# vdorie/stan4bart

Hardware: AMD Instinct MI355X
Metric: gibbs_iters_per_sec (higher is better)
Workload: dtype f64

## Files before the change

### include/stan4bart_amd.h

```cpp
#ifndef STAN4BART_AMD_H
#define STAN4BART_AMD_H

#include <stdint.h>
#include <stddef.h>

#ifndef S4B_PREFIX
#define S4B_PREFIX s4b_
#endif
#define S4B_CAT_(a, b) a##b
#define S4B_CAT(a, b) S4B_CAT_(a, b)
#define S4B_FN(name) S4B_CAT(S4B_PREFIX, name)

#ifdef __cplusplus
extern "C" {
#endif

#define S4B_INTERFACE_VERSION 6

typedef struct s4b_sampler s4b_sampler;

typedef struct {
  int32_t n_trees;
  int32_t n_thin;
  int32_t keep_trees;
// ... 338 lines not shown
  int64_t info[8];
} s4b_curves_out;
int S4B_FN(predict_curves)(s4b_sampler* s, const s4b_curves_in* in, s4b_curves_out* out);

typedef struct {
  s4b_summary_in rows;
  const double* y;
  const double* sigma;
  const double* row_scale;
  int32_t tail_len;
  int32_t n_peers;
  s4b_sampler* const* peers;
  const double* const* peer_dense_coef;
  const double* const* peer_ell_coef;
  const double* const* peer_sigma;
  int64_t scratch_bytes;
} s4b_loo_in;
typedef struct {
  double* elpd_loo;
  double* pareto_k;
  double* lpd;
  double* ess;
  int64_t num_samples;
  int32_t tail_len;
  int64_t info[8];
} s4b_loo_out;
int S4B_FN(predict_loo)(s4b_sampler* s, const s4b_loo_in* in, s4b_loo_out* out);

typedef struct {
  s4b_summary_in rows;
  int32_t quantity;
  int32_t split;
  const double* y;
  const double* sigma;
  const double* row_scale;
  int32_t n_peers;
  s4b_sampler* const* peers;
  const double* const* peer_dense_coef;
  const double* const* peer_ell_coef;
  const double* const* peer_sigma;
  int64_t scratch_bytes;
} s4b_conv_in;
typedef struct {
  double* rhat;
  double* ess;
  double* mean;
  double* mcse;
  int32_t* n_pairs;
  int64_t num_samples;
  int32_t n_chains;
  int32_t chain_len;
  int64_t info[8];
} s4b_conv_out;
int S4B_FN(predict_convergence)(s4b_sampler* s, const s4b_conv_in* in, s4b_conv_out* out);

#define S4B_STATE_MAGIC 0x53423453u
typedef struct {
  uint32_t magic, version;
  int64_t n;
  int32_t n_trees, num_unconstrained, is_binary, p;
  int64_t reserved[2];
} s4b_state_header;
int S4B_FN(get_state)(s4b_sampler* s, void* buf, int64_t cap, int64_t* size);
int S4B_FN(set_state)(s4b_sampler* s, const void* buf, int64_t size);

int S4B_FN(set_trace)(s4b_sampler* s, int32_t enable);
int S4B_FN(get_trace)(s4b_sampler* s, int64_t cap_records, int32_t* out, int64_t* num_records);
int S4B_FN(get_leaf_assignment)(s4b_sampler* s, int32_t tree, int32_t* out);
int S4B_FN(set_device_sharing)(s4b_sampler* s, int32_t chains);
int S4B_FN(set_tree_path)(s4b_sampler* s, int32_t path);
int S4B_FN(get_tree_path)(s4b_sampler* s, int32_t out[2]);
int S4B_FN(get_counters)(s4b_sampler* s, int64_t out[3]);
int S4B_FN(get_fused_stats)(s4b_sampler* s, int64_t out[2]);
int S4B_FN(get_sweep_stats)(s4b_sampler* s, int64_t out[2]);
int S4B_FN(get_sweep_spec)(s4b_sampler* s, int64_t out[4]);
int S4B_FN(get_sweep_busy)(s4b_sampler* s, int64_t* out);
int S4B_FN(set_hmc_mode)(s4b_sampler* s, int32_t mode);
int S4B_FN(get_hmc_mode)(s4b_sampler* s, int32_t* mode);
int S4B_FN(set_latent_mode)(s4b_sampler* s, int32_t mode);
int S4B_FN(get_latent_mode)(s4b_sampler* s, int32_t* mode);

int S4B_FN(get_nuts_stats)(s4b_sampler* s, double out[4]);

int S4B_FN(profile_sweep)(s4b_sampler* s, int32_t n_sweeps, double out[8]);
int S4B_FN(stream_probe)(int32_t device, int64_t n_doubles, int32_t reps, double out[4]);

int S4B_FN(profile_leapfrog)(s4b_sampler* s, int32_t n_evals, double out[8]);

int S4B_FN(set_test_hook)(s4b_sampler* s, int32_t hook, int64_t value);

int S4B_FN(test_draw_latents)(s4b_sampler* s);

int S4B_FN(test_hand_off)(s4b_sampler* s, const double* beta, const double* b, double sigma, int32_t update_scale);

#define S4B_STAN_SUMS_INFO 18
int S4B_FN(test_stan_sums)(s4b_sampler* s, int32_t mode, const double* beta, const double* b, const int32_t* set_exp, double* sums, int64_t* info);

void S4B_FN(free)(s4b_sampler* s);

typedef struct s4b_sweep_group s4b_sweep_group;
int S4B_FN(sweep_group_create)(int32_t device, int32_t max_members, s4b_sweep_group** out);
int S4B_FN(sweep_group_join)(s4b_sweep_group* g, s4b_sampler* s);
int S4B_FN(sweep_group_leave)(s4b_sampler* s);
int S4B_FN(sweep_group_stats)(s4b_sweep_group* g, int64_t out[4]);
int S4B_FN(sweep_group_set_timeout)(s4b_sweep_group* g, double seconds);
int S4B_FN(sweep_group_free)(s4b_sweep_group* g);

#ifdef __cplusplus
}
#endif
#endif
```

### stan4bart_amd/abi.py

```python
from __future__ import annotations

import ctypes as C
from dataclasses import dataclass, field
from typing import Callable, Optional, Sequence

import numpy as np

INTERFACE_VERSION = 6
c_double_p = C.POINTER(C.c_double)
c_int32_p = C.POINTER(C.c_int32)
c_uint32_p = C.POINTER(C.c_uint32)


class BartControl(C.Structure):
    _fields_ = [("n_trees", C.c_int32), ("n_thin", C.c_int32), ("keep_trees", C.c_int32),
                ("node_capacity", C.c_int32),
                ("base", C.c_double), ("power", C.c_double), ("k", C.c_double), ("node_scale", C.c_double),
                ("birth_or_death_prob", C.c_double), ("swap_prob", C.c_double),
                ("change_prob", C.c_double), ("birth_prob", C.c_double),
                ("split_probs", c_double_p), ("use_quantiles", C.c_int32), ("interface_version", C.c_int32),
                ("k_hyper_df", C.c_double), ("k_hyper_scale", C.c_double)]


class BartData(C.Structure):
# ... 158 lines not shown


class LooIn(C.Structure):
    _fields_ = [("rows", SummaryIn), ("y", c_double_p), ("sigma", c_double_p), ("row_scale", c_double_p), ("tail_len", C.c_int32),
                ("n_peers", C.c_int32), ("peers", C.POINTER(C.c_void_p)), ("peer_dense_coef", C.POINTER(c_double_p)),
                ("peer_ell_coef", C.POINTER(c_double_p)), ("peer_sigma", C.POINTER(c_double_p)), ("scratch_bytes", C.c_int64)]


class LooOut(C.Structure):
    _fields_ = [("elpd_loo", c_double_p), ("pareto_k", c_double_p), ("lpd", c_double_p), ("ess", c_double_p), ("num_samples", C.c_int64),
                ("tail_len", C.c_int32), ("info", C.c_int64 * 8)]


class ConvIn(C.Structure):
    _fields_ = [("rows", SummaryIn), ("quantity", C.c_int32), ("split", C.c_int32), ("y", c_double_p), ("sigma", c_double_p), ("row_scale", c_double_p),
                ("n_peers", C.c_int32), ("peers", C.POINTER(C.c_void_p)), ("peer_dense_coef", C.POINTER(c_double_p)),
                ("peer_ell_coef", C.POINTER(c_double_p)), ("peer_sigma", C.POINTER(c_double_p)), ("scratch_bytes", C.c_int64)]


class ConvOut(C.Structure):
    _fields_ = [("rhat", c_double_p), ("ess", c_double_p), ("mean", c_double_p), ("mcse", c_double_p), ("n_pairs", C.POINTER(C.c_int32)),
                ("num_samples", C.c_int64), ("n_chains", C.c_int32), ("chain_len", C.c_int32), ("info", C.c_int64 * 8)]


SUMMARY_ROUTES = {"auto": 0, "staged": 1, "global": 2}
SUMMARY_INFO = ("route", "rows_per_tile", "workgroups", "staging_bytes", "largest_draw_nodes", "launches", "device_bytes", "staging_nodes")
PD_INFO = SUMMARY_INFO[:7] + ("largest_affected", "total_affected")
QUANTILE_INFO = ("route", "rows_per_chunk", "chunks", "rows_per_sort", "padded_draws", "largest_draw_nodes", "launches", "device_bytes", "draws")
CONTRAST_INFO = ("route", "rows_per_chunk", "chunks", "launches", "device_bytes", "draws", "differing_columns", "largest_affected", "total_affected")
GROUPS_INFO = ("route", "rows_per_chunk", "chunks", "launches", "device_bytes", "draws", "edge_levels", "nan_levels")
GROUPS_STATISTICS = {"sum": 0, "mean": 1}
GROUPS_LEVEL_BYTES_MAX = 1 << 30
PROJECTION_INFO = ("route", "rows_per_chunk", "chunks", "launches", "device_bytes", "draws", "deficient", "columns")
PROJECTION_COLUMNS_MAX = 32
PROJECTION_SLAB = 128
SPREAD_INFO = ("route", "rows_per_chunk", "chunks", "launches", "device_bytes", "draws", "thresholds", "zero_slabs")
SPREAD_THRESHOLDS_MAX = 64
SPREAD_SLAB = 128
SPREAD_BIN_INDEX = {"auto": 0, "compare": 1, "search": 2}
CHECK_INFO = SPREAD_INFO
CURVES_INFO = QUANTILE_INFO[:7] + ("device_bytes", "largest_affected", "total_affected")
CURVES_OUTPUTS = ("mean", "m2", "quantiles", "p_max", "p_min", "range_mean", "range_m2", "range_quantiles")
CURVES_SCRATCH_MAX = 1 << 30
PPD_INFO = QUANTILE_INFO
LOO_INFO = QUANTILE_INFO
LOO_OUTPUTS = ("elpd_loo", "pareto_k", "lpd", "ess")
CONV_INFO = QUANTILE_INFO
CONV_OUTPUTS = ("rhat", "ess", "mean", "mcse", "n_pairs")
CONV_QUANTITIES = {"ev": 0, "lik": 1}
PD_GRID_MAX = 64


def _peer_tables(peers, draws, given, cols, what):
    if not cols or not peers or given is None:
        return None, []
    if len(given) != len(peers):
        raise ValueError(f"{what} must hold one table per peer ({len(peers)})")
    held = []
    for x, (t, smp) in enumerate(zip(given, peers)):
        t = np.asarray(t)
        if t.shape != (draws(smp), cols):
            raise ValueError(f"{what}[{x}] must be [{draws(smp)} x {cols}], not shape {t.shape}")
        held.append(_f64(t, "C"))
    return (c_double_p * len(held))(*[_dp(t) for t in held]), held


def _dp(a: Optional[np.ndarray]):
    return None if a is None else a.ctypes.data_as(c_double_p)


def _ip(a: Optional[np.ndarray]):
    return None if a is None else a.ctypes.data_as(c_int32_p)


def _f64(a, order="F") -> np.ndarray:
    return np.require(np.asarray(a, dtype=np.float64), requirements=["A", "O"] + (["F"] if order == "F" else ["C"]))


def _i32(a) -> np.ndarray:
    return np.ascontiguousarray(np.asarray(a, dtype=np.int32))


LATENT_MODES = {"exact": 0, "parallel": 1}

@dataclass
class SamplerArgs:
    x_bart: np.ndarray
    n_trees: int = 75
    n_cuts: int | Sequence[int] = 100
    n_thin: int = 1
    x_test: Optional[np.ndarray] = None
    base: float = 0.95
    power: float = 2.0
    k: float = 2.0
    node_scale: Optional[float] = None
    keep_trees: bool = False
    node_capacity: int = 0
    proposal_probs: Sequence[float] = (0.5, 0.1, 0.4, 0.5)
    split_probs: Optional[Sequence[float]] = None
    use_quantiles: bool = False
    k_hyper: Optional[tuple] = None
    latents: str = "exact"
    X: Optional[np.ndarray] = None
    y: Optional[np.ndarray] = None
    weights: Optional[np.ndarray] = None
    is_binary: bool = False
    prior_dist: int = 1
    prior_dist_for_aux: int = 3
    prior_scale: Optional[np.ndarray] = None
    prior_mean: Optional[np.ndarray] = None
    prior_df: Optional[np.ndarray] = None
    prior_scale_for_aux: float = 1.0
    prior_mean_for_aux: float = 0.0
    prior_df_for_aux: float = 1.0
    global_prior_df: float = 1.0
    global_prior_scale: float = 0.01
    slab_df: float = 4.0
    slab_scale: float = 2.5
    num_normals: Optional[Sequence[int]] = None
    p: Sequence[int] = ()
    l: Sequence[int] = ()
    shape: Sequence[float] = ()
    scale: Sequence[float] = ()
    concentration: Sequence[float] = ()
    regularization: Sequence[float] = ()
    w: Optional[np.ndarray] = None
    v: Optional[np.ndarray] = None
    u: Optional[np.ndarray] = None
    seed: int = 0
    skip: int = 1
    init_r: float = 2.0
    adapt_gamma: float = 0.05
    adapt_delta: float = 0.8
    adapt_kappa: float = 0.75
    adapt_t0: float = 10.0
    adapt_init_buffer: int = 75
    adapt_term_buffer: int = 50
    adapt_window: int = 25
    stepsize: float = 1.0
    stepsize_jitter: float = 0.0
    max_treedepth: int = 10
    hmc_mode: int = 0
    warmup: int = 1000
    iter: int = 2000
    verbose: int = 0
    refresh: int = 0
    offset: Optional[np.ndarray] = None
    offset_type: int = 0
    bart_offset_init: Optional[np.ndarray] = None
    sigma_init: float = 1.0
    keep_fits: bool = True
    callback: Optional[Callable] = None
    device: int = 0
    extras: dict = field(default_factory=dict)


class Sampler:

    def __init__(self, lib: C.CDLL, prefix: str, args: SamplerArgs, r_rng_state: np.ndarray):
        self._lib, self._pfx = lib, prefix
        self._bind()
        a = args
        self._keep = []

        def keep(x):
            self._keep.append(x)
# ... 27 lines not shown
        y = keep(_f64(a.y))
        t = len(a.p)
        q = int(sum(int(pi) * int(li) for pi, li in zip(a.p, a.l)))
        len_theta_L = int(sum(pi * (pi - 1) // 2 + pi for pi in a.p))
        ps = keep(_f64(a.prior_scale if a.prior_scale is not None else np.ones(K)))
        pm = keep(_f64(a.prior_mean if a.prior_mean is not None else np.zeros(K)))
        pdf = keep(_f64(a.prior_df if a.prior_df is not None else np.ones(K)))
        wts = keep(_f64(a.weights)) if a.weights is not None and len(a.weights) else None
        p_arr, l_arr = keep(_i32(a.p)), keep(_i32(a.l))
        shape, scale = keep(_f64(a.shape)), keep(_f64(a.scale))
        conc, reg = keep(_f64(a.concentration)), keep(_f64(a.regularization))
        w = keep(_f64(a.w if a.w is not None else np.zeros(0)))
        v = keep(_i32(a.v if a.v is not None else np.zeros(0)))
        u = keep(_i32(a.u if a.u is not None else np.zeros(n + 1)))
        sd = StanData(N=n, K=K, is_binary=int(a.is_binary), has_intercept=0, has_weights=int(wts is not None),
                      prior_dist=a.prior_dist, prior_dist_for_aux=a.prior_dist_for_aux,
                      X=_dp(X), y=_dp(y), weights=_dp(wts), prior_scale=_dp(ps), prior_mean=_dp(pm), prior_df=_dp(pdf),
                      prior_scale_for_aux=a.prior_scale_for_aux, prior_mean_for_aux=a.prior_mean_for_aux,
                      prior_df_for_aux=a.prior_df_for_aux, t=t, q=q, len_theta_L=len_theta_L,
                      len_concentration=len(conc), len_regularization=len(reg), reserved=0,
                      p=_ip(p_arr), l=_ip(l_arr), shape=_dp(shape), scale=_dp(scale),
                      concentration=_dp(conc), regularization=_dp(reg), num_non_zero=len(w),
                      w=_dp(w), v=_ip(v), u=_ip(u),
                      global_prior_df=a.global_prior_df, global_prior_scale=a.global_prior_scale, slab_df=a.slab_df,
                      slab_scale=a.slab_scale,
                      num_normals=_ip(keep(_i32(a.num_normals))) if a.num_normals is not None else None)
        sc = StanControl(seed=a.seed & 0xFFFFFFFF, skip=a.skip, init_r=a.init_r, adapt_gamma=a.adapt_gamma,
                         adapt_delta=a.adapt_delta, adapt_kappa=a.adapt_kappa, adapt_t0=a.adapt_t0,
                         adapt_init_buffer=a.adapt_init_buffer, adapt_term_buffer=a.adapt_term_buffer,
                         adapt_window=a.adapt_window, reserved=0, stepsize=a.stepsize,
                         stepsize_jitter=a.stepsize_jitter, max_treedepth=a.max_treedepth, hmc_mode=a.hmc_mode)
        off = keep(_f64(a.offset)) if a.offset is not None and len(a.offset) else None
        boi = keep(_f64(a.bart_offset_init)) if a.bart_offset_init is not None else None
        self._py_callback = a.callback
        self._cb = CALLBACK(self._trampoline) if a.callback is not None else CALLBACK()
        cc = CommonControl(warmup=a.warmup, iter=a.iter, verbose=a.verbose, refresh=a.refresh,
                           is_binary=int(a.is_binary), offset_type=a.offset_type, keep_fits=int(a.keep_fits),
                           device=a.device, offset=_dp(off), bart_offset_init=_dp(boi), sigma_init=a.sigma_init,
                           callback=self._cb, callback_user=None)
        st = np.ascontiguousarray(r_rng_state, dtype=np.uint32)
        assert st.shape == (625,)
        self._h = C.c_void_p()
        rc = self._f("create")(C.byref(bc), C.byref(bd), C.byref(sd), C.byref(sc), C.byref(cc),
                               st.ctypes.data_as(c_uint32_p), C.byref(self._h))
        self._check(rc)
        self._keep.clear()
        if a.latents not in LATENT_MODES:
            self.free()
            raise ValueError(f"latents must be one of {sorted(LATENT_MODES)}, not {a.latents!r}")
        if a.latents != "exact":
            try:
                self.set_latent_mode(LATENT_MODES[a.latents])
            except Exception:
                self.free()
                raise
        dims = (C.c_int64 * 5)()
        self._check(self._f("get_dims")(self._h, dims))
        self.num_pars, self.n, self.n_test, self.p, self.n_trees = (int(d) for d in dims)
        self.keep_fits = bool(a.keep_fits)
        self.K, self.q = int(K), int(q)
        self.callback_results: list = []
        self._pending_exc = None

    def _bind(self):
        vp, i32, i64, dp, ip, up = C.c_void_p, C.c_int32, C.c_int64, c_double_p, c_int32_p, c_uint32_p
        sig = {
            "create": [C.POINTER(BartControl), C.POINTER(BartData), C.POINTER(StanData), C.POINTER(StanControl),
                       C.POINTER(CommonControl), up, C.POINTER(vp)],
            "run": [vp, i32, i32, i32, C.POINTER(Results)],
            "disengage_adaptation": [vp], "print_initial_summary": [vp],
            "get_parametric_mean": [vp, dp], "get_bart_data_range": [vp, dp],
            "get_r_rng_state": [vp, up], "set_r_rng_state": [vp, up],
            "get_dims": [vp, C.POINTER(i64)], "get_stan_par_names": [vp, C.c_char_p, C.c_size_t],
            "get_trees": [vp, i64, ip, ip, ip, ip, dp, C.POINTER(i64)],
            "get_kept_trees": [vp, i64, i64, ip, ip, ip, ip, ip, dp, C.POINTER(i64)],
            "get_kept_trees_indexed": [vp, ip, i64, ip, i64, i64, ip, ip, ip, ip, ip, dp, C.POINTER(i64)],
            "export_bart_state": [vp, vp, i64, C.POINTER(i64)],
            "create_stored_bart_sampler": [vp, i64, i32, C.POINTER(vp)],
            "predict_bart": [vp, dp, i64, dp, C.POINTER(i64)],
            "predict_bart_offset": [vp, dp, i64, dp, dp, C.POINTER(i64)], "print_trees": [vp, ip, i64, ip, i64],
            "get_state": [vp, vp, i64, C.POINTER(i64)], "set_state": [vp, vp, i64],
            "set_trace": [vp, i32], "get_trace": [vp, i64, ip, C.POINTER(i64)],
            "get_leaf_assignment": [vp, i32, ip], "get_counters": [vp, C.POINTER(i64)], "get_nuts_stats": [vp, dp],
            "profile_sweep": [vp, i32, dp], "profile_leapfrog": [vp, i32, dp],
            "set_progress": [vp, PROGRESS, vp], "set_device_sharing": [vp, i32],
            "set_tree_path": [vp, i32], "get_tree_path": [vp, ip], "get_fused_stats": [vp, C.POINTER(i64)], "get_sweep_stats": [vp, C.POINTER(i64)], "get_sweep_busy": [vp, C.POINTER(i64)], "get_sweep_spec": [vp, C.POINTER(i64)], "set_test_hook": [vp, i32, i64], "set_hmc_mode": [vp, i32], "get_hmc_mode": [vp, ip],
            "predict_summary": [vp, C.POINTER(SummaryIn), C.POINTER(SummaryOut)],
            "partial_dependence": [vp, C.POINTER(PdIn), C.POINTER(PdOut)],
            "predict_quantiles": [vp, C.POINTER(QuantileIn), C.POINTER(QuantileOut)],
            "predict_contrast": [vp, C.POINTER(ContrastIn), C.POINTER(ContrastOut)],
            "predict_groups": [vp, C.POINTER(GroupsIn), C.POINTER(GroupsOut)],
            "predict_projection": [vp, C.POINTER(ProjectionIn), C.POINTER(ProjectionOut)],
            "predict_spread": [vp, C.POINTER(SpreadIn), C.POINTER(SpreadOut)],
            "predict_check": [vp, C.POINTER(CheckIn), C.POINTER(CheckOut)],
            "predict_curves": [vp, C.POINTER(CurvesIn), C.POINTER(CurvesOut)],
            "predict_ppd": [vp, C.POINTER(PpdIn), C.POINTER(PpdOut)],
            "predict_loo": [vp, C.POINTER(LooIn), C.POINTER(LooOut)],
            "predict_convergence": [vp, C.POINTER(ConvIn), C.POINTER(ConvOut)],
            "set_latent_mode": [vp, i32], "get_latent_mode": [vp, ip], "test_draw_latents": [vp], "test_hand_off": [vp, dp, dp, C.c_double, i32],
            "test_stan_sums": [vp, i32, dp, dp, ip, dp, C.POINTER(i64)],
        }
        for name, argtypes in sig.items():
            fn = getattr(self._lib, self._pfx + name, None)
            if fn is None:
                continue
            fn.restype = C.c_int
            fn.argtypes = argtypes
        getattr(self._lib, self._pfx + "last_error").restype = C.c_char_p
        getattr(self._lib, self._pfx + "last_error").argtypes = []
        getattr(self._lib, self._pfx + "free").restype = None
        getattr(self._lib, self._pfx + "free").argtypes = [vp]

    def _f(self, name):
        return getattr(self._lib, self._pfx + name)

    def _check(self, rc):
        if rc != 0:
            raise RuntimeError(self._f("last_error")().decode())

    def _trampoline(self, user, yhat_train, yhat_test, stan_pars, num_pars):
        tr = np.ctypeslib.as_array(yhat_train, shape=(self.n,)).copy()
        te = np.ctypeslib.as_array(yhat_test, shape=(self.n_test,)).copy() if self.n_test else None
        sp = np.ctypeslib.as_array(stan_pars, shape=(num_pars,)).copy()
        try:
            self.callback_results.append(self._py_callback(tr, te, sp))
        except BaseException as e:
            if self._pending_exc is None:
                self._pending_exc = e
            return 1
        return 0

    def run(self, num_iter: int, is_warmup: bool, results_type: int = 0) -> dict:
        S = num_iter if self.keep_fits else 1
        stan = np.zeros((self.num_pars, S), order="F")
        sigma = np.zeros(S)
        train = np.zeros((self.n, S), order="F")
        test = np.zeros((self.n_test, S), order="F")
        varcount = np.zeros((self.p, S), dtype=np.int32, order="F")
        kdraws = np.zeros(S)
        res = Results(stan=_dp(stan), bart_sigma=_dp(sigma), bart_train=_dp(train),
                      bart_test=_dp(test) if self.n_test else None, bart_varcount=_ip(varcount),
                      bart_k=_dp(kdraws) if getattr(self, "k_modeled", False) else None)
        self.callback_results = []
        self._pending_exc = None
        rc = self._f("run")(self._h, num_iter, int(is_warmup), results_type, C.byref(res))
        if self._pending_exc is not None:
            e, self._pending_exc = self._pending_exc, None
            raise e
        self._check(rc)
        out = {}
        if results_type in (0, 2):
            out["stan"] = stan
        if results_type in (0, 1):
            out["bart"] = dict(sigma=sigma, train=train, test=test, varcount=varcount)
            if getattr(self, "k_modeled", False):
                out["bart"]["k"] = kdraws
        if self._py_callback is not None:
            out["callback"] = list(self.callback_results)
        return out

    def disengage_adaptation(self):
        self._check(self._f("disengage_adaptation")(self._h))

    def print_initial_summary(self):
        self._check(self._f("print_initial_summary")(self._h))

# ... 125 lines not shown

    def get_fused_stats(self):
        out = (C.c_int64 * 2)()
        fn = getattr(self._lib, self._pfx + "get_fused_stats", None)
        if fn is not None:
            self._check(fn(self._h, out))
        return int(out[0]), int(out[1])

    def get_sweep_stats(self):
        fn = getattr(self._lib, self._pfx + "get_sweep_stats", None)
        if fn is None:
            return (0, 0)
        out = (C.c_int64 * 2)()
        self._check(fn(self._h, out))
        return (int(out[0]), int(out[1]))

    def get_sweep_spec(self):
        fn = getattr(self._lib, self._pfx + "get_sweep_spec", None)
        if fn is None:
            return (0, 0, 0, 0)
        out = (C.c_int64 * 4)()
        self._check(fn(self._h, out))
        return tuple(int(v) for v in out)

    def set_test_hook(self, hook: int, value: int):
        self._check(self._f("set_test_hook")(self._h, int(hook), int(value)))

    def test_draw_latents(self):
        self._check(self._f("test_draw_latents")(self._h))

    def test_hand_off(self, beta, b, sigma: float, update_scale: bool):
        beta, b = _f64(np.atleast_1d(beta)), _f64(np.atleast_1d(b))
        self._check(self._f("test_hand_off")(self._h, _dp(beta) if beta.size else None, _dp(b) if b.size else None, float(sigma), int(bool(update_scale))))

    STAN_SUMS_INFO = 18

    def test_stan_sums(self, mode: int, beta=None, b=None, set_exp=None):
        K, q = self.K, self.q
        beta = _f64(np.zeros(K) if beta is None else np.atleast_1d(beta))
        b = _f64(np.zeros(q) if b is None else np.atleast_1d(b))
        if beta.size != K or b.size != q:
            raise ValueError(f"test_stan_sums: beta needs {K} entries and b {q}")
        ex = None if set_exp is None else np.ascontiguousarray(set_exp, dtype=np.int32)
        if ex is not None and ex.shape != (3,):
            raise ValueError("test_stan_sums: set_exp holds three exponents")
        sums = np.zeros(1 + K + q)
        info = (C.c_int64 * Sampler.STAN_SUMS_INFO)()
        self._check(self._f("test_stan_sums")(self._h, int(mode), _dp(beta) if K else None, _dp(b) if q else None, _ip(ex) if ex is not None else None, _dp(sums), info))
        v = [int(x) for x in info]
        return sums, dict(accepted=bool(v[0]), reject=v[1], exp_used=tuple(v[2:5]), exp_after=tuple(v[5:8]), mag=tuple(v[8:11]), exw=tuple(v[11:14]),
                          grid=v[14], fused=bool(v[15]), evals=v[16], fallbacks=v[17])

    def get_sweep_busy(self) -> int:
        fn = getattr(self._lib, self._pfx + "get_sweep_busy", None)
        if fn is None:
            return 0
        out = C.c_int64(0)
        self._check(fn(self._h, C.byref(out)))
        return int(out.value)

    def set_trace(self, enable: bool):
        self._check(self._f("set_trace")(self._h, int(enable)))

    def get_trace(self, cap: int = 1 << 20) -> np.ndarray:
        nn = C.c_int64()
        out = np.zeros((cap, 5), dtype=np.int32)
        self._check(self._f("get_trace")(self._h, cap, _ip(out), C.byref(nn)))
        return out[: nn.value].copy()

    def get_leaf_assignment(self, tree: int) -> np.ndarray:
        out = np.zeros(self.n, dtype=np.int32)
        self._check(self._f("get_leaf_assignment")(self._h, tree, _ip(out)))
        return out

    def get_counters(self) -> np.ndarray:
        out = (C.c_int64 * 3)()
        self._check(self._f("get_counters")(self._h, out))
        return np.array(list(out), dtype=np.int64)

    def get_nuts_stats(self) -> dict:
        out = (C.c_double * 4)()
        self._check(self._f("get_nuts_stats")(self._h, out))
        return dict(transitions=int(out[0]), sum_treedepth=int(out[1]), sum_n_leapfrog=int(out[2]), divergent=int(out[3]))

    def predict_bart(self, x_test: np.ndarray, offset_test: Optional[np.ndarray] = None) -> np.ndarray:
        xt = _f64(x_test)
        ns = C.c_int64()
        self._check(self._f("predict_bart")(self._h, _dp(xt), xt.shape[0], None, C.byref(ns)))
        out = np.zeros((xt.shape[0], ns.value), order="F")
        if ns.value:
            if offset_test is not None:
                off = _f64(offset_test)
                if off.shape != (xt.shape[0],):
                    raise ValueError("length of offset_test must equal number of rows in x_test")
                self._check(self._f("predict_bart_offset")(self._h, _dp(xt), xt.shape[0], _dp(off), _dp(out), C.byref(ns)))
            else:
                self._check(self._f("predict_bart")(self._h, _dp(xt), xt.shape[0], _dp(out), C.byref(ns)))
        return out

    def predict_summary(self, x_test: np.ndarray, offset=None, dense=None, dense_coef=None, ell_index=None, ell_value=None, ell_coef=None,
                        link: int = 0, weights=None, route="auto", stage_nodes: int = 0, max_workgroups: int = 0) -> dict:
        fn = getattr(self._lib, self._pfx + "predict_summary", None)
        if fn is None:
            raise RuntimeError(f"this library ({self._pfx}*) has no predict_summary")
        probe = SummaryOut()
        self._check(fn(self._h, None, C.byref(probe)))
        S = int(probe.num_samples)
        arg, keep, rows, G = self._summary_in(S, x_test, offset, dense, dense_coef, ell_index, ell_value, ell_coef, link, weights, route, stage_nodes,
                                              max_workgroups)
        mean, m2, avg = np.zeros(rows), np.zeros(rows), np.zeros((S, G))
        out = SummaryOut(mean=_dp(mean), m2=_dp(m2), average=_dp(avg) if avg.size else None)
        self.summary_info = dict(zip(SUMMARY_INFO, [0] * 8))
        rc = fn(self._h, C.byref(arg), C.byref(out))
        self.summary_info = dict(zip(SUMMARY_INFO, (int(v) for v in out.info)))
        self._check(rc)
        return dict(mean=mean, m2=m2, average=avg, draws=int(out.num_samples), info=dict(self.summary_info))

    @staticmethod
    def _summary_in(S, x_test, offset, dense, dense_coef, ell_index, ell_value, ell_coef, link, weights, route, stage_nodes, max_workgroups):
        xt = _f64(x_test)
        if xt.ndim != 2:
            raise ValueError("x_test must be a matrix [rows x predictors]")
        rows = xt.shape[0]

        def table(a, first, what):
            if a is None:
                return None, 0
            a = np.asarray(a)
            if a.ndim != 2 or a.shape[0] != first:
                raise ValueError(f"{what} must have {first} rows, not shape {a.shape}")
            return a, a.shape[1]
        dense, M = table(dense, rows, "dense")
        dense_coef, Mc = table(dense_coef, S, "dense_coef")
        ell_index, E = table(ell_index, rows, "ell_index")
        ell_value, Ev = table(ell_value, rows, "ell_value")
        ell_coef, q = table(ell_coef, S, "ell_coef")
        if M != Mc:
            raise ValueError(f"dense has {M} columns, dense_coef {Mc}")
        if E != Ev:
            raise ValueError(f"ell_index has {E} columns, ell_value {Ev}")
        if weights is not None:
            weights = np.asarray(weights, dtype=np.float64)
            if weights.ndim != 2 or weights.shape[1] != rows:
                raise ValueError(f"weights must be [G x {rows}], not shape {weights.shape}")
        G = 0 if weights is None else weights.shape[0]
        off = None
        if offset is not None:
            off = _f64(offset)
            if off.shape != (rows,):
                raise ValueError("length of offset must equal number of rows in x_test")
        keep = dict(dense=None if not M else _f64(dense), dense_coef=None if not M else _f64(dense_coef, "C"),
                    ell_index=None if not E else np.asfortranarray(np.asarray(ell_index, dtype=np.int32)),
                    ell_value=None if not E else _f64(ell_value), ell_coef=None if not E else _f64(ell_coef, "C"),
                    weights=None if not G else _f64(weights, "C"))
        keep.update(x_test=xt, offset=off)
        arg = SummaryIn(x_test=_dp(xt), n_test=rows, offset=_dp(off), n_dense=M, n_ell=E, n_ell_coef=q if E else 0, link=int(link), n_weights=G,
                        route=int(SUMMARY_ROUTES.get(route, route)), stage_nodes=int(stage_nodes), max_workgroups=int(max_workgroups),
                        dense=_dp(keep["dense"]), dense_coef=_dp(keep["dense_coef"]), ell_index=_ip(keep["ell_index"]),
                        ell_value=_dp(keep["ell_value"]), ell_coef=_dp(keep["ell_coef"]), weights=_dp(keep["weights"]))
        return arg, keep, rows, G

    def partial_dependence(self, x_test: np.ndarray, vars, grid, offset=None, dense=None, dense_coef=None, ell_index=None, ell_value=None,
                           ell_coef=None, link: int = 0, weights=None, route="auto", stage_nodes: int = 0, max_workgroups: int = 0) -> dict:
        fn = getattr(self._lib, self._pfx + "partial_dependence", None)
        if fn is None:
            raise RuntimeError(f"this library ({self._pfx}*) has no partial_dependence")
# ... 732 lines not shown
```

### stan4bart_amd/csrc/c_api.inc

```
#include <memory>
#include <string>

struct s4b_sampler { s4b::SamplerCore<S4B_DEV> core; template <class... A> explicit s4b_sampler(A... a) : core(a...) {} };
struct s4b_sweep_group { std::unique_ptr<s4b::SweepGroup> g; };

namespace { thread_local std::string g_last_error; }

#define S4B_TRY try {
#define S4B_CATCH } catch (const std::exception& e) { g_last_error = e.what(); return 1; } catch (...) { g_last_error = "unknown error"; return 1; } return 0;
#define S4B_NEED(s, what) if (!(s)) { g_last_error = what " called on NULL sampler"; return 1; }

extern "C" {

const char* S4B_FN(last_error)(void) { return g_last_error.c_str(); }

int S4B_FN(create)(const s4b_bart_control* bc, const s4b_bart_data* bd, const s4b_stan_data* sd, const s4b_stan_control* sc,
                   const s4b_common_control* cc, const uint32_t* rstate, s4b_sampler** out) {
  S4B_TRY
  if (!out) throw std::invalid_argument("create: NULL output pointer");
  *out = new s4b_sampler(bc, bd, sd, sc, cc, rstate);
  S4B_CATCH
}
int S4B_FN(run)(s4b_sampler* s, int32_t num_iter, int32_t is_warmup, int32_t results_type, s4b_results* out) {
  S4B_NEED(s, "run") S4B_TRY s->core.dev().bind(); s4b::SamplerCore<S4B_DEV>::GroupRun inRun(s->core); s->core.run(num_iter, is_warmup != 0, results_type, out); S4B_CATCH
// ... 77 lines not shown
  s->core.dev().bind();
  std::vector<const s4b::SamplerCore<S4B_DEV>*> peers;
  if (in && out && in->arms.n_peers > 0 && in->arms.peers) for (int x = 0; x < in->arms.n_peers; ++x) peers.push_back(in->arms.peers[x] ? &in->arms.peers[x]->core : nullptr);
  s->core.predict_spread(in, out, peers.empty() ? nullptr : peers.data());
  S4B_CATCH
}
int S4B_FN(predict_check)(s4b_sampler* s, const s4b_check_in* in, s4b_check_out* out) {
  S4B_NEED(s, "predict_check") S4B_TRY
  s->core.dev().bind();
  std::vector<const s4b::SamplerCore<S4B_DEV>*> peers;
  if (in && out && in->n_peers > 0 && in->peers) for (int x = 0; x < in->n_peers; ++x) peers.push_back(in->peers[x] ? &in->peers[x]->core : nullptr);
  s->core.predict_check(in, out, peers.empty() ? nullptr : peers.data());
  S4B_CATCH
}
int S4B_FN(predict_curves)(s4b_sampler* s, const s4b_curves_in* in, s4b_curves_out* out) {
  S4B_NEED(s, "predict_curves") S4B_TRY
  s->core.dev().bind();
  std::vector<const s4b::SamplerCore<S4B_DEV>*> peers;
  if (in && out && in->n_peers > 0 && in->peers) for (int x = 0; x < in->n_peers; ++x) peers.push_back(in->peers[x] ? &in->peers[x]->core : nullptr);
  s->core.predict_curves(in, out, peers.empty() ? nullptr : peers.data());
  S4B_CATCH
}
int S4B_FN(predict_ppd)(s4b_sampler* s, const s4b_ppd_in* in, s4b_ppd_out* out) {
  S4B_NEED(s, "predict_ppd") S4B_TRY
  s->core.dev().bind();
  std::vector<const s4b::SamplerCore<S4B_DEV>*> peers;
  if (in && out && in->n_peers > 0 && in->peers) for (int x = 0; x < in->n_peers; ++x) peers.push_back(in->peers[x] ? &in->peers[x]->core : nullptr);
  s->core.predict_ppd(in, out, peers.empty() ? nullptr : peers.data());
  S4B_CATCH
}
int S4B_FN(predict_loo)(s4b_sampler* s, const s4b_loo_in* in, s4b_loo_out* out) {
  S4B_NEED(s, "predict_loo") S4B_TRY
  s->core.dev().bind();
  std::vector<const s4b::SamplerCore<S4B_DEV>*> peers;
  if (in && out && in->n_peers > 0 && in->peers) for (int x = 0; x < in->n_peers; ++x) peers.push_back(in->peers[x] ? &in->peers[x]->core : nullptr);
  s->core.predict_loo(in, out, peers.empty() ? nullptr : peers.data());
  S4B_CATCH
}
int S4B_FN(predict_convergence)(s4b_sampler* s, const s4b_conv_in* in, s4b_conv_out* out) {
  S4B_NEED(s, "predict_convergence") S4B_TRY
  s->core.dev().bind();
  std::vector<const s4b::SamplerCore<S4B_DEV>*> peers;
  if (in && out && in->n_peers > 0 && in->peers) for (int x = 0; x < in->n_peers; ++x) peers.push_back(in->peers[x] ? &in->peers[x]->core : nullptr);
  s->core.predict_convergence(in, out, peers.empty() ? nullptr : peers.data());
  S4B_CATCH
}
int S4B_FN(export_bart_state)(s4b_sampler* s, void* buf, int64_t cap, int64_t* size) {
  S4B_NEED(s, "exportBARTState") S4B_TRY s->core.dev().bind(); if (!size) throw std::invalid_argument("exportBARTState: NULL size pointer"); *size = s->core.export_state(buf, cap); S4B_CATCH
}
int S4B_FN(create_stored_bart_sampler)(const void* state, int64_t size, int32_t device, s4b_sampler** out) {
  S4B_TRY
  if (!out) throw std::invalid_argument("createStoredBARTSampler: NULL output pointer");
  *out = new s4b_sampler(state, size, (int)device);
  S4B_CATCH
}
int S4B_FN(get_state)(s4b_sampler* s, void* buf, int64_t cap, int64_t* size) {
  S4B_NEED(s, "get_state") S4B_TRY s->core.dev().bind(); if (!size) throw std::invalid_argument("get_state: NULL size pointer"); *size = s->core.get_state(buf, cap); S4B_CATCH
}
int S4B_FN(set_state)(s4b_sampler* s, const void* buf, int64_t size) { S4B_NEED(s, "set_state") S4B_TRY s->core.dev().bind(); s->core.set_state(buf, size); S4B_CATCH }
int S4B_FN(set_trace)(s4b_sampler* s, int32_t enable) { S4B_NEED(s, "set_trace") S4B_TRY s->core.dev().bind(); s->core.set_trace(enable != 0); S4B_CATCH }
int S4B_FN(get_trace)(s4b_sampler* s, int64_t cap, int32_t* out, int64_t* num) { S4B_NEED(s, "get_trace") S4B_TRY s->core.dev().bind(); *num = s->core.get_trace(cap, out); S4B_CATCH }
int S4B_FN(get_leaf_assignment)(s4b_sampler* s, int32_t t, int32_t* out) { S4B_NEED(s, "get_leaf_assignment") S4B_TRY s->core.dev().bind(); s->core.leaf_assignment(t, out); S4B_CATCH }
int S4B_FN(set_device_sharing)(s4b_sampler* s, int32_t chains) { S4B_NEED(s, "set_device_sharing") S4B_TRY s->core.dev().bind(); s->core.set_device_sharing(chains); S4B_CATCH }
int S4B_FN(set_tree_path)(s4b_sampler* s, int32_t path) { S4B_NEED(s, "set_tree_path") S4B_TRY s->core.dev().bind(); s->core.dev().set_tree_path(path); S4B_CATCH }
int S4B_FN(get_tree_path)(s4b_sampler* s, int32_t out[2]) { S4B_NEED(s, "get_tree_path") S4B_TRY if (!out) throw std::invalid_argument("get_tree_path: NULL output pointer"); s->core.dev().get_tree_path(out); S4B_CATCH }
int S4B_FN(set_hmc_mode)(s4b_sampler* s, int32_t mode) { S4B_NEED(s, "set_hmc_mode") S4B_TRY s->core.set_hmc_mode(mode); S4B_CATCH }
int S4B_FN(get_hmc_mode)(s4b_sampler* s, int32_t* mode) { S4B_NEED(s, "get_hmc_mode") S4B_TRY if (!mode) throw std::invalid_argument("get_hmc_mode: NULL output pointer"); *mode = s->core.hmc_mode(); S4B_CATCH }
int S4B_FN(set_latent_mode)(s4b_sampler* s, int32_t mode) { S4B_NEED(s, "set_latent_mode") S4B_TRY s->core.dev().bind(); s->core.set_latent_mode(mode); S4B_CATCH }
int S4B_FN(get_latent_mode)(s4b_sampler* s, int32_t* mode) { S4B_NEED(s, "get_latent_mode") S4B_TRY if (!mode) throw std::invalid_argument("get_latent_mode: NULL output pointer"); *mode = s->core.latent_mode(); S4B_CATCH }
int S4B_FN(get_fused_stats)(s4b_sampler* s, int64_t out[2]) { S4B_NEED(s, "get_fused_stats") S4B_TRY if (!out) throw std::invalid_argument("get_fused_stats: NULL output pointer"); s->core.dev().fused_stats(out); S4B_CATCH }
int S4B_FN(get_sweep_stats)(s4b_sampler* s, int64_t out[2]) { S4B_NEED(s, "get_sweep_stats") S4B_TRY if (!out) throw std::invalid_argument("get_sweep_stats: NULL output pointer"); s->core.dev().sweep_stats(out); S4B_CATCH }
int S4B_FN(get_sweep_spec)(s4b_sampler* s, int64_t out[4]) { S4B_NEED(s, "get_sweep_spec") S4B_TRY if (!out) throw std::invalid_argument("get_sweep_spec: NULL output pointer"); s->core.dev().sweep_spec(out); S4B_CATCH }
int S4B_FN(set_test_hook)(s4b_sampler* s, int32_t hook, int64_t value) { S4B_NEED(s, "set_test_hook") S4B_TRY s->core.dev().set_test_hook(hook, value); S4B_CATCH }
int S4B_FN(test_draw_latents)(s4b_sampler* s) { S4B_NEED(s, "test_draw_latents") S4B_TRY s->core.dev().bind(); s->core.test_draw_latents(); S4B_CATCH }
int S4B_FN(test_hand_off)(s4b_sampler* s, const double* beta, const double* b, double sigma, int32_t update_scale) {
  S4B_NEED(s, "test_hand_off") S4B_TRY s->core.dev().bind(); s->core.test_hand_off(beta, b, sigma, update_scale != 0); S4B_CATCH
}
int S4B_FN(test_stan_sums)(s4b_sampler* s, int32_t mode, const double* beta, const double* b, const int32_t* set_exp, double* sums, int64_t* info) {
  S4B_NEED(s, "test_stan_sums") S4B_TRY s->core.dev().bind(); s->core.test_stan_sums(mode, beta, b, set_exp, sums, info); S4B_CATCH
}
int S4B_FN(get_sweep_busy)(s4b_sampler* s, int64_t* out) { S4B_NEED(s, "get_sweep_busy") S4B_TRY if (!out) throw std::invalid_argument("get_sweep_busy: NULL output pointer"); *out = s->core.dev().sweep_busy(); S4B_CATCH }
int S4B_FN(get_counters)(s4b_sampler* s, int64_t out[3]) { S4B_NEED(s, "get_counters") S4B_TRY s->core.dev().bind(); s->core.counters(out); S4B_CATCH }
int S4B_FN(get_nuts_stats)(s4b_sampler* s, double out[4]) { S4B_NEED(s, "get_nuts_stats") S4B_TRY s->core.dev().bind(); s->core.nuts_stats(out); S4B_CATCH }
int S4B_FN(profile_sweep)(s4b_sampler* s, int32_t n_sweeps, double out[8]) { S4B_NEED(s, "profile_sweep") S4B_TRY s->core.dev().bind(); s->core.profile_sweep(n_sweeps, out); S4B_CATCH }
int S4B_FN(profile_leapfrog)(s4b_sampler* s, int32_t n_evals, double out[8]) { S4B_NEED(s, "profile_leapfrog") S4B_TRY s->core.dev().bind(); s->core.profile_leapfrog(n_evals, out); S4B_CATCH }
int S4B_FN(stream_probe)(int32_t device, int64_t n_doubles, int32_t reps, double out[4]) { S4B_TRY S4B_DEV::probe_stream(device, n_doubles, reps, out); S4B_CATCH }
void S4B_FN(free)(s4b_sampler* s) { if (s) { try { s->core.leave_group(); } catch (...) {} } delete s; }

int S4B_FN(sweep_group_create)(int32_t device, int32_t max_members, s4b_sweep_group** out) {
  S4B_TRY
  if (!out) throw std::invalid_argument("sweep_group_create: NULL output pointer");
  *out = new s4b_sweep_group{std::unique_ptr<s4b::SweepGroup>(s4b::SamplerCore<S4B_DEV>::make_group((int)device, (int)max_members))};
  S4B_CATCH
}
int S4B_FN(sweep_group_join)(s4b_sweep_group* g, s4b_sampler* s) {
  S4B_NEED(s, "sweep_group_join") S4B_TRY if (!g) throw std::invalid_argument("sweep_group_join: NULL group"); s->core.join_group(g->g.get()); S4B_CATCH
}
int S4B_FN(sweep_group_leave)(s4b_sampler* s) { S4B_NEED(s, "sweep_group_leave") S4B_TRY s->core.leave_group(); S4B_CATCH }
int S4B_FN(sweep_group_stats)(s4b_sweep_group* g, int64_t out[4]) {
  S4B_TRY if (!g || !out) throw std::invalid_argument("sweep_group_stats: NULL argument"); g->g->stats(out); S4B_CATCH
}
int S4B_FN(sweep_group_set_timeout)(s4b_sweep_group* g, double seconds) {
  S4B_TRY if (!g) throw std::invalid_argument("sweep_group_set_timeout: NULL group"); g->g->set_timeout(seconds); S4B_CATCH
}
int S4B_FN(sweep_group_free)(s4b_sweep_group* g) {
  S4B_TRY
  if (!g) return 0;
  if (g->g->members() != 0) throw std::invalid_argument("sweep_group_free: samplers are still joined (s4b_sweep_group_leave / s4b_free them first)");
  delete g;
  S4B_CATCH
}

}
```

### stan4bart_amd/csrc/sampler_core.hpp

```cpp
#ifndef S4B_SAMPLER_CORE_HPP
#define S4B_SAMPLER_CORE_HPP

#include <algorithm>
#include <chrono>
#include <cstdio>
#include <cstdlib>
#include <cstring>
#include <memory>
#include <stdexcept>
#include <string>
#include <thread>
#include <type_traits>
#include <unordered_map>
#include <vector>

#include "../../include/stan4bart_amd.h"
#include "sweep_group.hpp"
#include "dev_common.hpp"
#include "stan_host.hpp"

namespace s4b {

enum { OFFSET_DEFAULT = 0, OFFSET_FIXEF, OFFSET_RANEF, OFFSET_BART, OFFSET_PARAMETRIC };
enum { OBS_R = 0, OBS_OFF, OBS_LAT, OBS_Y };
// ... 231 lines not shown
    if ((sd->prior_dist == 3 || sd->prior_dist == 4) && cc->is_binary) throw std::invalid_argument("hs priors scale with the residual sd: not available for binary responses");
    if (sd->prior_dist == 7 && !sd->num_normals) throw std::invalid_argument("product_normal needs num_normals");
    n_ = (size_t)bd->n; P_ = bd->p; T_ = bc->n_trees; nTest_ = (size_t)bd->n_test;
    warmup_ = cc->warmup; verbose_ = cc->verbose; refresh_ = cc->refresh; keepFits_ = cc->keep_fits != 0; offsetType_ = cc->offset_type;
    callback_ = cc->callback; callbackUser_ = cc->callback_user;
    thin_ = bc->n_thin > 0 ? bc->n_thin : 1;
    keepTrees_ = bc->keep_trees != 0;
    nc_ = bc->node_capacity > 0 ? bc->node_capacity : 256;
    if (nc_ < 3 || nc_ > 32000) throw std::invalid_argument("node_capacity must be in [3, 32000]");
    if (cc->offset) { userOffset_.assign(cc->offset, cc->offset + n_); hasUserOffset_ = true; }
    rng_.mti = (int32_t)rstate[0]; rng_.pad = 0;
    std::memcpy(rng_.mt, rstate + 1, 624 * sizeof(uint32_t));
    latKey_ = latent_key(rstate, sc->seed);

    StanSpec sp;
    sp.N = sd->N; sp.K = sd->K; sp.q = sd->q; sp.t = sd->t; sp.len_theta_L = sd->len_theta_L;
    sp.is_binary = binary_ ? 1 : 0; sp.prior_dist = sd->prior_dist; sp.prior_dist_for_aux = sd->prior_dist_for_aux;
    if (sd->K) { sp.prior_scale.assign(sd->prior_scale, sd->prior_scale + sd->K); sp.prior_mean.assign(sd->prior_mean, sd->prior_mean + sd->K);
                 sp.prior_df.assign(sd->prior_df, sd->prior_df + sd->K); }
    sp.prior_scale_for_aux = sd->prior_scale_for_aux; sp.prior_mean_for_aux = sd->prior_mean_for_aux; sp.prior_df_for_aux = sd->prior_df_for_aux;
    sp.global_prior_df = sd->global_prior_df; sp.global_prior_scale = sd->global_prior_scale; sp.slab_df = sd->slab_df; sp.slab_scale = sd->slab_scale;
    if (sd->prior_dist == 7) sp.num_normals.assign(sd->num_normals, sd->num_normals + sd->K);
    if (sd->t) { sp.p.assign(sd->p, sd->p + sd->t); sp.l.assign(sd->l, sd->l + sd->t); sp.shape.assign(sd->shape, sd->shape + sd->t);
                 sp.scale.assign(sd->scale, sd->scale + sd->t); }
    if (sd->len_concentration) sp.concentration.assign(sd->concentration, sd->concentration + sd->len_concentration);
    if (sd->len_regularization) sp.regularization.assign(sd->regularization, sd->regularization + sd->len_regularization);
    {
      int qq = 0; for (int i = 0; i < sd->t; ++i) qq += sd->p[i] * sd->l[i];
      if (qq != sd->q) throw std::invalid_argument("q != sum(p * l)");
      for (int64_t e = 0; e < sd->num_non_zero; ++e) if (sd->v[e] < 0 || sd->v[e] >= sd->q) throw std::invalid_argument("CSR column index out of range");
    }
    model_.reset(new HostModel(sp));
    if (const char* e = std::getenv("S4B_GRADIENT_CHECK")) model_->gradientCheck = std::atoi(e);
    K_ = sd->K; q_ = sd->q; hmcMode_ = sc->hmc_mode;
    cX_.assign((size_t)K_, 0.0); cZ_.assign((size_t)q_, 0.0);

    numCuts_.assign(bd->n_cuts, bd->n_cuts + P_);
    for (int j = 0; j < P_; ++j) if (numCuts_[(size_t)j] < 0 || numCuts_[(size_t)j] > 65534) throw std::invalid_argument("n_cuts must be in [0, 65534]");
    make_cuts(bd->x, bc->use_quantiles != 0);
    std::vector<uint16_t> xbin((size_t)P_ * n_), xbinTest((size_t)P_ * nTest_);
    bin_matrix(bd->x, n_, xbin);
    if (nTest_) bin_matrix(bd->x_test, nTest_, xbinTest);

    DevInit di;
    di.n = (int64_t)n_; di.nTest = (int64_t)nTest_; di.P = P_; di.T = T_; di.nc = nc_; di.device = cc->device; groupDevice_ = cc->device;
    di.xbin = xbin.data(); di.xbinTest = nTest_ ? xbinTest.data() : nullptr; di.numCuts = numCuts_.data();
    di.y = sd->y; di.userOffset = hasUserOffset_ ? userOffset_.data() : nullptr; di.weights = weights_.empty() ? nullptr : weights_.data();
    di.model.P = P_; di.model.Pvalid = 0;
    for (int j = 0; j < P_; ++j) if (numCuts_[(size_t)j] > 0) ++di.model.Pvalid;
    if (di.model.Pvalid == 0) throw std::invalid_argument("no predictor has a cut point");
    di.model.numCuts = nullptr; di.model.scratch = nullptr; di.model.splitProbs = nullptr;
    if (bc->split_probs) {
      splitProbs_.assign(bc->split_probs, bc->split_probs + P_);
      for (double w : splitProbs_) if (!(w > 0.0) || !std::isfinite(w)) throw std::invalid_argument("split_probs must be positive and finite");
      di.model.splitProbs = splitProbs_.data();
    }
    di.model.base = bc->base; di.model.power = bc->power;
    di.model.pBD = bc->birth_or_death_prob; di.model.pSwap = bc->swap_prob; di.model.pChange = bc->change_prob; di.model.pBirth = bc->birth_prob;
    if (!(bc->k > 0.0) || !std::isfinite(bc->k)) throw std::invalid_argument("k must be positive and finite");
    kModeled_ = bc->k_hyper_df > 0.0; kFixed_ = bc->k;
    if (kModeled_ && !(bc->k_hyper_scale > 0.0)) throw std::invalid_argument("k_hyper_scale must be positive (or +Inf)");
    if (kModeled_ && !std::isfinite(bc->k_hyper_df)) throw std::invalid_argument("k_hyper_df must be finite");
    di.model.leafPrec = leaf_precision(bc->k, T_, bc->node_scale);
    {
      pgDepth_.resize(S4B_MAX_DEPTH); logPg_.resize(S4B_MAX_DEPTH); log1mPg_.resize(S4B_MAX_DEPTH);
      for (int d = 0; d < S4B_MAX_DEPTH; ++d) {
        pgDepth_[(size_t)d] = bc->base / std::pow(1.0 + (double)d, bc->power);
        logPg_[(size_t)d] = std::log(pgDepth_[(size_t)d]); log1mPg_[(size_t)d] = std::log(1.0 - pgDepth_[(size_t)d]);
      }
      int maxCuts = 1; for (int j = 0; j < P_; ++j) maxCuts = std::max(maxCuts, numCuts_[(size_t)j]);
      logInt_.resize((size_t)std::max(P_, maxCuts) + 2);
      for (size_t k = 0; k < logInt_.size(); ++k) logInt_[k] = std::log((double)k);
      di.model.pgDepth = pgDepth_.data(); di.model.logPg = logPg_.data(); di.model.log1mPg = log1mPg_.data();
      di.model.logInt = logInt_.data(); di.model.logIntLen = (int32_t)logInt_.size();
    }
    di.K = K_; di.q = q_; di.binary = binary_ ? 1 : 0; di.X = sd->X; di.w = sd->w; di.v = sd->v; di.u = sd->u; di.nnz = sd->num_non_zero; nnz_ = sd->num_non_zero;
    di.traceCap = 1 << 16;
    hostModelView_ = di.model; hostModelView_.numCuts = numCuts_.data();
    dev_.init(di);
    if (kModeled_) dev_.set_k_hyper(bc->k_hyper_df, bc->k_hyper_scale, bc->node_scale, bc->k);

    if (hmcMode_ == 0) { build_gram(sd); haveGram_ = true; }
    dev_.stan_inputs( 0, false, cX_.data(), cZ_.data(), &s0_, nullptr);
    model_->lik = [this](const double* beta, const double* b, double* gX, double* gZ) { return likelihood(beta, b, gX, gZ); };
    NutsControl nc;
    nc.seed = sc->seed; nc.init_r = sc->init_r; nc.skip = sc->skip;
    if (nc.skip <= 0) { nc.skip = (2000 - warmup_) / 1000; if (nc.skip < 1) nc.skip = 1; }
    nc.gamma = sc->adapt_gamma; nc.delta = sc->adapt_delta; nc.kappa = sc->adapt_kappa; nc.t0 = sc->adapt_t0;
    nc.init_buffer = sc->adapt_init_buffer; nc.term_buffer = sc->adapt_term_buffer; nc.window = sc->adapt_window;
    nc.stepsize = sc->stepsize; nc.jitter = sc->stepsize_jitter; nc.max_depth = sc->max_treedepth;
    nuts_.reset(new Nuts(*model_, nc, 1, warmup_));
    row_.assign((size_t)(7 + model_->sp.n_constrained), 0.0);

    std::vector<double> bartOffset(n_, 0.0);
    const double* boi = cc->bart_offset_init;
    if (hasUserOffset_) {
      if (offsetType_ != OFFSET_BART) {
        bartOffset = userOffset_;
        if (boi && offsetType_ == OFFSET_DEFAULT) for (size_t i = 0; i < n_; ++i) bartOffset[i] += boi[i];
      } else if (boi) bartOffset.assign(boi, boi + n_);
    } else if (boi) bartOffset.assign(boi, boi + n_);
    dev_.offset_from_host(bartOffset.data());
    dev_.rescale(true);
    if (!binary_) { dev_.set_sigma(cc->sigma_init); sigma_ = cc->sigma_init; } else sigma_ = 1.0;
    sample_trees_from_prior();
    dev_.sweep(thin_);
    treeUpdates_ += (long)T_ * thin_;
    dev_.stan_inputs(stan_mode(), false, cX_.data(), cZ_.data(), &s0_, nullptr);
    check_device();
  }

  void run(int numIter, bool isWarmup, int resultsType, s4b_results* out) {
    live();
    if (numIter < 1) throw std::invalid_argument("num_iter must be >= 1");
    ran_ = true;
    dev_.reset_fused_scales();
    const bool doStan = resultsType == 0 || resultsType == 2, doBart = resultsType == 0 || resultsType == 1;
    const int numPars = (int)row_.size();
    size_t slot = 0;
    std::vector<double> train, test;
    const bool wantTrain = (out && out->bart_train) || callback_;
    const bool lastOnly = !keepFits_ && !callback_;
    if (wantTrain) train.resize(n_);
    if (nTest_) test.resize(nTest_);
    if (verbose_ > 0 && !progress_)
      std::printf("starting %s, %d draws, %s\n", isWarmup ? "warmup" : "sampling", numIter,
                  resultsType == 0 ? "both BART and Stan" : (resultsType == 1 ? "BART only" : "Stan only"));
    std::fflush(stdout);
    const bool timing = std::getenv("S4B_HOST_TIMING") != nullptr;
    double tph[4] = {0, 0, 0, 0};
    auto now = [] { return std::chrono::duration<double>(std::chrono::steady_clock::now().time_since_epoch()).count(); };
    for (int iter = 0; iter < numIter; ++iter) {
      if (progress_) {
        if (refresh_ <= 0 || (iter + 1) % refresh_ == 0 || iter == 0)
          if (progress_(progressUser_, iter + 1, numIter, isWarmup ? 1 : 0) != 0) throw std::runtime_error("interrupted by the progress callback");
      } else if (refresh_ > 0 && verbose_ > 1 && (iter + 1) % refresh_ == 0) { std::printf("  iter %.3d / %.3d\n", iter + 1, numIter); std::fflush(stdout); }
      double t0 = timing ? now() : 0;
      if (doStan) {
        nuts_->run(row_.data());
        if (timing) { tph[0] += now() - t0; t0 = now(); }
        const double* cons = row_.data() + 7;
        const double* beta = cons + model_->sp.beta_pos();
        const double* b = cons + model_->sp.b_pos();
        offset_by_type(beta, b);
        if (!binary_) { sigma_ = cons[model_->sp.aux_pos()]; dev_.set_sigma(sigma_); }
        if (out && out->stan) std::memcpy(out->stan + slot * (size_t)numPars, row_.data(), (size_t)numPars * sizeof(double));
        int update_scale_mod = 1 << (8 * iter / numIter);
        dev_.rescale(isWarmup && iter % update_scale_mod == 0);
        if (timing) { tph[1] += now() - t0; t0 = now(); }
      }
      if (doBart) {
        treeUpdates_ += (long)T_ * thin_;
        const bool emit = !lastOnly || iter == numIter - 1;
        if (nTest_ && emit && ((out && out->bart_test) || callback_)) dev_.request_test_fits();
        if (out && emit && out->bart_varcount) dev_.request_var_counts();
        sweep_and_stan_inputs(wantTrain && emit, (wantTrain && emit) ? train.data() : nullptr);
        if (timing) { tph[2] += now() - t0; t0 = now(); }
        if (nTest_ && emit && ((out && out->bart_test) || callback_)) dev_.test_fits(test.data());
        if (out && emit) {
          if (out->bart_sigma) out->bart_sigma[slot] = sigma_;
          if (out->bart_k) out->bart_k[slot] = kModeled_ ? dev_.k_current() : kFixed_;
          if (out->bart_train) std::memcpy(out->bart_train + slot * n_, train.data(), n_ * sizeof(double));
          if (out->bart_test && nTest_) std::memcpy(out->bart_test + slot * nTest_, test.data(), nTest_ * sizeof(double));
          if (out->bart_varcount) dev_.var_counts(out->bart_varcount + slot * (size_t)P_);
        }
        if (keepTrees_ && !isWarmup) keep_current_trees();
        if (callback_ && callback_(callbackUser_, train.data(), nTest_ ? test.data() : nullptr, row_.data(), numPars) != 0)
          throw std::runtime_error("stopped by the per-iteration callback");
        if (timing) tph[3] += now() - t0;
      }
      if (keepFits_) ++slot;
    }
    if (timing) std::fprintf(stderr, "S4B host ms/iter: nuts %.3f  offset+rescale issue %.3f  sweep + stan inputs (wait) %.3f  results %.3f\n",
                             1e3 * tph[0] / numIter, 1e3 * tph[1] / numIter, 1e3 * tph[2] / numIter, 1e3 * tph[3] / numIter);
// ... 807 lines not shown
    for (int i = 0; i < 7; ++i) ns.window[i] = win[i];
    ns.adapting = (int32_t)win[7];
    uint32_t rr[626]; r.get(rr, sizeof(rr));
    if (rr[0] > 624u) throw std::invalid_argument("sampler state: generator position out of range");
    double sc4[4]; r.get(sc4, sizeof(sc4));
    if (!(sc4[2] > 0.0) || !(sc4[3] > 0.0)) throw std::invalid_argument("sampler state: response range and sigma must be positive");
    std::vector<double> off(n_), fits(n_), lat;
    r.get(off.data(), n_ * 8); r.get(fits.data(), n_ * 8);
    if (binary_) { lat.resize(n_); r.get(lat.data(), n_ * 8); }
    HostTrees h; h.alloc(T_, nc_);
    for (int t = 0; t < T_; ++t) {
      int32_t cnt[2]; r.get(cnt, sizeof(cnt));
      if (cnt[0] < 1 || cnt[0] > nc_ || cnt[1] < 1 || 2 * cnt[1] - 1 != cnt[0]) throw std::invalid_argument("sampler state: tree does not fit node_capacity");
      std::vector<int32_t> nd((size_t)cnt[0] * 2); std::vector<double> mu((size_t)cnt[1]);
      r.get(nd.data(), nd.size() * 4); r.get(mu.data(), mu.size() * 8);
      const size_t o = (size_t)t * nc_;
      int leaf = 0; std::vector<int> open;
      for (int i = 0; i < cnt[0]; ++i) {
        int par = -1;
        if (i > 0) {
          if (open.empty()) throw std::invalid_argument("sampler state: malformed tree");
          par = open.back();
          if (h.left[o + (size_t)par] < 0) h.left[o + (size_t)par] = (int16_t)i; else { h.right[o + (size_t)par] = (int16_t)i; open.pop_back(); }
        }
        h.parent[o + (size_t)i] = (int16_t)par;
        const int32_t v = nd[(size_t)2 * i], s2 = nd[(size_t)2 * i + 1];
        if (v >= 0) {
          if (v >= P_ || s2 < 0 || s2 >= numCuts_[(size_t)v]) throw std::invalid_argument("sampler state: rule out of range");
          h.var[o + (size_t)i] = (int16_t)v; h.cut[o + (size_t)i] = (uint16_t)s2; open.push_back(i);
        } else {
          if (leaf >= cnt[1]) throw std::invalid_argument("sampler state: malformed tree");
          h.var[o + (size_t)i] = NODE_LEAF; h.mu[o + (size_t)i] = mu[(size_t)leaf++]; h.cnt[o + (size_t)i] = s2;
        }
      }
      if (!open.empty() || leaf != cnt[1]) throw std::invalid_argument("sampler state: malformed tree");
      h.hwm[(size_t)t] = cnt[0];
    }
    uint64_t ls[2] = {0, 0};
    if (latMode_) { ls[0] = r.u64(); ls[1] = r.u64(); }
    {
      auto finite = [](const double* x, size_t k) { for (size_t i = 0; i < k; ++i) if (!std::isfinite(x[i])) return false; return true; };
      bool ok = finite(ns.q.data(), (size_t)D) && finite(ns.inv_metric.data(), (size_t)D) && finite(ns.wm.data(), (size_t)D) && finite(ns.wm2.data(), (size_t)D) &&
                finite(sc6, 6) && finite(sc4, 4) && finite(off.data(), n_) && finite(fits.data(), n_) && (!binary_ || finite(lat.data(), n_)) &&
                finite(h.mu.data(), h.mu.size());
      for (int i = 0; i < 7 && ok; ++i) ok = !std::isnan(ns.last[i]);
      for (int i = 0; i < D && ok; ++i) ok = ns.inv_metric[(size_t)i] > 0.0;
      if (!ok || !(sc6[0] > 0.0)) throw std::invalid_argument("sampler state: non-finite value, non-positive step size or inverse metric");
    }
    double kState = 0.0;
    std::memcpy(&kState, &hd.reserved[0], 8);
    if (kModeled_) {
      if (!(kState > 0.0) || !std::isfinite(kState)) throw std::invalid_argument("sampler state: k must be positive and finite (the state of a sampler with a fixed k carries none)");
    } else if (kState != 0.0) throw std::invalid_argument("sampler state: it carries the value of a modeled k, this sampler's k is fixed");
    if (kModeled_) dev_.set_k(kState);
    if (latMode_) dev_set_latent_state(ls);
    nuts_->set_state(ns);
    dev_.reset_fused_scales();
    nuts_->current_row(row_.data());
    set_rng(rr);
    sigma_ = sc4[3];
    dev_.set_scale(sc4[0], sc4[1], sc4[2], sc4[3]);
    dev_.upload_obs(OBS_OFF, off.data());
    if (binary_) { dev_.upload_obs(OBS_LAT, lat.data()); for (size_t i = 0; i < n_; ++i) fits[i] = lat[i] - fits[i]; }
    else {
      std::vector<double> y(n_); dev_.download_obs(OBS_Y, y.data());
      for (size_t i = 0; i < n_; ++i) fits[i] = ((y[i] - off[i] - sc4[0]) / sc4[2] - 0.5) - fits[i];
    }
    dev_.upload_obs(OBS_R, fits.data());
    dev_.upload_trees(h.var.data(), h.cut.data(), h.left.data(), h.right.data(), h.parent.data(), h.mu.data(), h.hwm.data());
    dev_.upload_counts(h.cnt.data());
    dev_.assign_leaves_only();
    dev_.stan_inputs(stan_mode(), false, cX_.data(), cZ_.data(), &s0_, nullptr);
    check_device();
  }

  void set_trace(bool on) { live(); dev_.set_trace(on); }
  void set_device_sharing(int chains) { live(); dev_.set_device_sharing(chains); }
  int hmc_mode() const { live(); return hmcMode_; }
  void set_hmc_mode(int mode) {
    live();
    if (mode != 0 && mode != 1) throw std::invalid_argument("hmc_mode must be 0 (sufficient statistics) or 1 (one device evaluation per leapfrog)");
    if (mode == 0 && !haveGram_) throw std::invalid_argument("this sampler was created with hmc_mode 1: it has no Gram matrix to evaluate from sufficient statistics");
    hmcMode_ = mode;
  }
  static constexpr bool kLatentMode = has_latent_mode<Dev>::value;
  int latent_mode() const { live(); return latMode_; }
  void set_latent_mode(int mode) {
    live();
    if (mode != 0 && mode != 1) throw std::invalid_argument("latent mode must be 0 (exact: R's stream, the reference's draw) or 1 (parallel: counter-based, one thread per observation)");
    if (mode == latMode_) return;
    if (mode == 1 && !binary_) throw std::invalid_argument("latent mode 1 (parallel) draws probit latents: this sampler's response is continuous");
    if (ran_) throw std::invalid_argument("the latent mode is set before the first run");
    if constexpr (kLatentMode) { dev_.set_latent_mode(mode, latKey_); latMode_ = mode; }
    else throw std::invalid_argument("this device layer has no parallel latent draw: latent mode 1 needs the HIP device layer");
  }
  void test_draw_latents() {
    live();
    if (!binary_) throw std::invalid_argument("test_draw_latents: this sampler's response is continuous (no probit latents)");
    if constexpr (has_test_draw_latents<Dev>::value) { dev_.test_draw_latents(); check_device(); }
    else throw std::invalid_argument("test_draw_latents: this device layer has no latent draw on its own");
  }
  int64_t get_trace(int64_t cap, int32_t* out) { live(); return dev_.get_trace(cap, out); }
  void leaf_assignment(int t, int32_t* out) {
    live();
    if (t < 0 || t >= T_) throw std::invalid_argument("tree index out of range");
    HostTrees h; download_trees(h);
    TreeView tv = h.view(t, nc_);
    std::vector<int16_t> list((size_t)nc_); std::vector<int32_t> rank((size_t)nc_, -1);
    PtrArr<int16_t> la(list.data());
    int nl = tv_list_leaves(tv, 0, la);
    for (int i = 0; i < nl; ++i) rank[(size_t)list[(size_t)i]] = i;
    std::vector<uint16_t> leaf(n_);
    dev_.download_leaf_plane(t, leaf.data());
    for (size_t i = 0; i < n_; ++i) out[i] = rank[leaf[i]];
  }
  void profile_sweep(int nSweeps, double out[8]) { live(); if (nSweeps < 1) throw std::invalid_argument("n_sweeps must be >= 1"); dev_.profile_sweep(nSweeps, thin_, out); out[7] = (double)n_; check_device(); }
  void profile_leapfrog(int nEvals, double out[8]) {
    live();
    if (nEvals < 1) throw std::invalid_argument("n_evals must be >= 1");
    const double* cons = row_.data() + 7;
    for (int i = 0; i < 8; ++i) out[i] = 0.0;
    dev_.profile_leapfrog(nEvals, cons + model_->sp.beta_pos(), cons + model_->sp.b_pos(), out);
    const double z = n_ ? (double)nnz_ / (double)n_ : 0.0;
    out[3] = (double)n_; out[4] = (double)n_ * (8.0 * K_ + 12.0 * z + 20.0);
    check_device();
  }
  void nuts_stats(double out[4]) { live(); nuts_->totals(out); }
  void counters(int64_t out[3]) { live(); out[0] = model_->gradEvals; out[1] = treeUpdates_; out[2] = dev_.launches(); }
  Dev& dev() { return dev_; }

  static constexpr bool kNativeGroup = has_native_sweep_group<Dev>::value;
  ~SamplerCore() { try { leave_group(); } catch (...) {} }
  static SweepGroup* make_group(int device, int maxMembers) {
    if constexpr (kNativeGroup) return Dev::group_create(device, maxMembers);
    else return new HostSweepGroup(device, maxMembers);
  }
  void join_group(SweepGroup* g) {
    if constexpr (kNativeGroup) dev_.join_group(g);
    else {
      if (group_) throw std::invalid_argument("sweep_group_join: the sampler is already in a sweep group");
      if (g->device() != groupDevice_) throw std::invalid_argument("sweep_group_join: the sampler runs on device " + std::to_string(groupDevice_) + ", the group on device " + std::to_string(g->device()));
      g->join(this); group_ = g;
    }
  }
  void leave_group() {
    if constexpr (kNativeGroup) dev_.leave_group();
    else if (group_) { group_->leave(this); group_ = nullptr; }
  }
  struct GroupRun {
    SamplerCore& c;
    explicit GroupRun(SamplerCore& cc) : c(cc) { if (SweepGroup* g = c.group()) g->enter_run(c.group_member(), c.group_eligible()); }
    ~GroupRun() { if (SweepGroup* g = c.group()) g->exit_run(c.group_member()); }
    GroupRun(const GroupRun&) = delete;
    GroupRun& operator=(const GroupRun&) = delete;
  };

 private:
  SweepGroup* group_ = nullptr;
  int groupDevice_ = 0;
  SweepGroup* group() { if constexpr (kNativeGroup) return dev_.group_; else return group_; }
  void* group_member() { if constexpr (kNativeGroup) return &dev_; else return this; }
  bool group_eligible() {
    if constexpr (kNativeGroup) return dev_.group_eligible();
    else { int32_t path[2]; dev_.get_tree_path(path); return n_ <= 4096 && (path[0] == 0 || path[0] == 4); }
  }
  void sweep_and_stan_inputs(bool wantTrain, double* train) {
    if constexpr (!kNativeGroup) {
// ... 285 lines not shown
    tv_fill_info_node(tv, hostModelView_, node);
    double pg = tv_growth(tv, hostModelView_, node);
    if (pg <= 0.0) return;
    if (!(r_unif(&rng_) < pg)) return;
    int v = tv_draw_var(tv, hostModelView_, node, &rng_);
    int lo, hi; tv_interval(tv, hostModelView_, node, v, lo, hi);
    int s = r_unif_int(&rng_, lo, hi + 1);
    int L = tv_alloc(tv, hwm); if (L < 0) throw std::runtime_error("node capacity exceeded while sampling trees from the prior");
    tv.var.set(L, NODE_LEAF);
    int R = tv_alloc(tv, hwm); if (R < 0) throw std::runtime_error("node capacity exceeded while sampling trees from the prior");
    tv.var.set(node, (int16_t)v); tv.cut.set(node, (uint16_t)s); tv.left.set(node, (int16_t)L); tv.right.set(node, (int16_t)R);
    tv.var.set(L, NODE_LEAF); tv.parent.set(L, (int16_t)node); tv.left.set(L, -1); tv.right.set(L, -1);
    tv.var.set(R, NODE_LEAF); tv.parent.set(R, (int16_t)node); tv.left.set(R, -1); tv.right.set(R, -1);
    grow(tv, hwm, L); grow(tv, hwm, R);
  }
  void sample_trees_from_prior() {
    HostTrees h; h.alloc(T_, nc_);
    std::vector<int16_t> list((size_t)nc_);
    for (int t = 0; t < T_; ++t) {
      TreeView tv = h.view(t, nc_);
      tv.var.set(0, NODE_LEAF); tv.parent.set(0, -1);
      int hwm = 1;
      grow(tv, hwm, 0);
      PtrArr<int16_t> la(list.data());
      int nl = tv_list_leaves(tv, 0, la);
      for (int i = 0; i < nl; ++i) h.mu[(size_t)t * nc_ + list[(size_t)i]] = r_norm(&rng_) / std::sqrt(hostModelView_.leafPrec);
      h.hwm[(size_t)t] = hwm;
    }
    dev_.upload_trees(h.var.data(), h.cut.data(), h.left.data(), h.right.data(), h.parent.data(), h.mu.data(), h.hwm.data());
    dev_.upload_rng(rng_);
    dev_.assign_leaves_and_residual();
  }

  void var_counts(int32_t* out) {
    HostTrees h; download_trees(h);
    for (int j = 0; j < P_; ++j) out[j] = 0;
    for (int t = 0; t < T_; ++t) { TreeView tv = h.view(t, nc_); int nd, k; Walker<TreeView> w(tv, 0); while (w.next(nd, k)) if (k == 1) ++out[tv.var.get(nd)]; }
  }

  void build_gram(const s4b_stan_data* sd) {
    const int M = K_ + q_;
    std::vector<int> idx; std::vector<double> val;
    auto row_of = [&](int64_t i) {
      idx.clear(); val.clear();
      for (int k = 0; k < K_; ++k) { idx.push_back(k); val.push_back(sd->X[(size_t)k * sd->N + i]); }
      if (q_) for (int e = sd->u[i]; e < sd->u[i + 1]; ++e) { idx.push_back(K_ + sd->v[e]); val.push_back(sd->w[e]); }
      return weights_.empty() ? 1.0 : weights_[(size_t)i];
    };
    gramPtr_.assign((size_t)M + 1, 0); gramCol_.clear(); gram_.clear();
    if ((size_t)M * (size_t)M <= ((size_t)1 << 22)) {
      std::vector<double> dense((size_t)M * M, 0.0);
      for (int64_t i = 0; i < sd->N; ++i) {
        const double wi = row_of(i);
        for (size_t a = 0; a < idx.size(); ++a) for (size_t b = 0; b < idx.size(); ++b) dense[(size_t)idx[a] * M + idx[b]] += wi * val[a] * val[b];
      }
      for (int a = 0; a < M; ++a) {
        for (int b = 0; b < M; ++b) if (dense[(size_t)a * M + b] != 0.0) { gramCol_.push_back(b); gram_.push_back(dense[(size_t)a * M + b]); }
        gramPtr_[(size_t)a + 1] = (int)gramCol_.size();
      }
      gramDense_.clear(); gramLd_ = 0;
      if (M <= 64 && gramCol_.size() * 3 >= (size_t)M * M) {
        gramLd_ = (M + 3) & ~3;
        gramDense_.assign((size_t)M * gramLd_, 0.0);
        for (int a = 0; a < M; ++a) for (int b = 0; b < M; ++b) gramDense_[(size_t)a * gramLd_ + b] = dense[(size_t)a * M + b];
      }
      return;
    }
    std::unordered_map<uint64_t, double> acc;
    acc.reserve((size_t)sd->N < ((size_t)1 << 22) ? (size_t)sd->N * 4 : ((size_t)1 << 24));
    for (int64_t i = 0; i < sd->N; ++i) {
      const double wi = row_of(i);
      for (size_t a = 0; a < idx.size(); ++a) for (size_t b = 0; b < idx.size(); ++b) acc[(uint64_t)idx[a] * (uint64_t)M + (uint64_t)idx[b]] += wi * val[a] * val[b];
    }
    std::vector<std::pair<uint64_t, double>> ent(acc.begin(), acc.end());
    std::sort(ent.begin(), ent.end(), [](const std::pair<uint64_t, double>& x, const std::pair<uint64_t, double>& y) { return x.first < y.first; });
    for (const auto& e : ent) {
      if (e.second == 0.0) continue;
      const int a = (int)(e.first / (uint64_t)M);
      gramCol_.push_back((int)(e.first % (uint64_t)M)); gram_.push_back(e.second);
      gramPtr_[(size_t)a + 1] = (int)gramCol_.size();
    }
    for (int a = 0; a < M; ++a) if (gramPtr_[(size_t)a + 1] < gramPtr_[(size_t)a]) gramPtr_[(size_t)a + 1] = gramPtr_[(size_t)a];
  }
  double likelihood(const double* beta, const double* b, double* gX, double* gZ) {
    if (hmcMode_ != 0) return dev_.leapfrog_sums(beta, b, gX, gZ);
    const int M = K_ + q_;
    if (thetaBuf_.size() < (size_t)M + 4) thetaBuf_.assign((size_t)M + 4, 0.0);
    double* const th = thetaBuf_.data();
    for (int k = 0; k < K_; ++k) th[k] = beta[k];
    for (int j = 0; j < q_; ++j) th[K_ + j] = b[j];
    if (gramLd_) {
      const double* const G = gramDense_.data(); const int ld = gramLd_;
      double ss = s0_;
      for (int a = 0; a < M; ++a) {
        const double* const r = G + (size_t)a * ld;
        double p0 = 0.0, p1 = 0.0, p2 = 0.0, p3 = 0.0;
        for (int c = 0; c < ld; c += 4) { p0 += r[c] * th[c]; p1 += r[c + 1] * th[c + 1]; p2 += r[c + 2] * th[c + 2]; p3 += r[c + 3] * th[c + 3]; }
        const double ga = (p0 + p2) + (p1 + p3);
        const double ca = a < K_ ? cX_[(size_t)a] : cZ_[(size_t)(a - K_)];
        ss += th[a] * (ga - 2.0 * ca);
        if (a < K_) gX[a] = ca - ga; else gZ[a - K_] = ca - ga;
      }
      return ss;
    }
    const int* const ptr = gramPtr_.data(); const int* const col = gramCol_.data(); const double* const g = gram_.data();
    double ss = s0_;
    for (int a = 0; a < M; ++a) {
      double ga = 0.0;
      for (int e = ptr[a]; e < ptr[a + 1]; ++e) ga += g[e] * th[col[e]];
      const double ca = a < K_ ? cX_[(size_t)a] : cZ_[(size_t)(a - K_)];
      ss += th[a] * (ga - 2.0 * ca);
      if (a < K_) gX[a] = ca - ga; else gZ[a - K_] = ca - ga;
    }
    return ss;
  }
  void check_device() {
    int32_t e = dev_.error_flags();
    if (e & S4B_ERR_NODE_CAPACITY) throw std::runtime_error("a tree outgrew node_capacity; re-create the sampler with a larger bart_control.node_capacity");
    if (e & S4B_ERR_I_LATENT) throw std::runtime_error("parallel latents: no proposal was accepted for an observation (a mean that is not finite or whose square overflows, |mean| above about 1.3e154; device error word " + std::to_string(e) + ")");
    if (e & S4B_ERR_INTERNAL) throw std::runtime_error("internal error: a hand-shake of the control kernel timed out, or one probit latent needed more than 256 positions of R's stream (device error word " + std::to_string(e) + ")");
    if (e & S4B_ERR_TRACE_OVERFLOW) throw std::runtime_error("trace buffer overflow: call get_trace more often");
  }

  Dev dev_;
  size_t n_ = 0, nTest_ = 0; int P_ = 0, T_ = 0, nc_ = 256, thin_ = 1, K_ = 0, q_ = 0, hmcMode_ = 0; bool haveGram_ = false;
  std::vector<double> thetaBuf_;
  int warmup_ = 0, verbose_ = 0, refresh_ = 0, offsetType_ = 0; s4b_progress_fn progress_ = nullptr; void* progressUser_ = nullptr; bool keepFits_ = true, hasUserOffset_ = false, binary_ = false;
  std::vector<double> userOffset_;
  s4b_callback_fn callback_ = nullptr; void* callbackUser_ = nullptr;
  MTState rng_;
  std::vector<int32_t> numCuts_; std::vector<std::vector<double>> cuts_; std::vector<double> splitProbs_;
  std::vector<double> pgDepth_, logPg_, log1mPg_, logInt_;
  ModelView hostModelView_;
  std::unique_ptr<HostModel> model_; std::unique_ptr<Nuts> nuts_;
  bool keepTrees_ = false, kModeled_ = false; double kFixed_ = 2.0;
  int latMode_ = 0; uint64_t latKey_ = 0; bool ran_ = false;
  std::vector<PackedNode> keptNodes_; std::vector<int64_t> keptTreeStart_; std::vector<double> keptScale_;
  std::vector<double> row_, cX_, cZ_, gram_, gramDense_; int gramLd_ = 0; std::vector<int> gramPtr_, gramCol_; double s0_ = 0, sigma_ = 1;
  long treeUpdates_ = 0;
};

}
#endif
```

### stan4bart_amd/csrc/stan_host.hpp

```cpp
#ifndef S4B_STAN_HOST_HPP
#define S4B_STAN_HOST_HPP

#include <algorithm>
#include <cmath>
#include <cstdint>
#include <functional>
#include <chrono>
#include <cstdio>
#include <limits>
#include <stdexcept>
#include <string>
#include <vector>

namespace s4b {

enum TapeCode : int { T_CONST = 0, T_INPUT, T_ADD, T_SUB, T_MUL, T_DIV, T_ADDC, T_SUBC, T_MULC, T_DIVC, T_CSUB, T_CDIV, T_SQRT, T_EXP, T_LOG,
                      T_SQUARE, T_LOG1M, T_STDNORMAL, T_INVLOGIT, T_INVLOGIT_LOGJAC };
class Tape {
 public:
  struct Op { double val; int a, b; double da, db; double c; int code; int k; };
  struct Ops {
    std::vector<Op> buf; size_t n = 0;
    size_t size() const { return n; }
    void clear() { n = 0; }
    void reserve(size_t k) { if (buf.size() < k) buf.resize(k); }
    Op& operator[](size_t i) { return buf[i]; }
    const Op& operator[](size_t i) const { return buf[i]; }
    int push(const Op& o) { if (n == buf.size()) buf.resize(buf.empty() ? 1024 : 2 * buf.size()); buf[n] = o; return (int)n++; }
  } ops;
  std::vector<double> adj;
  void clear() { ops.clear(); }
  static inline void eval(Op& o, const Op* all) {
    const double x = o.a >= 0 ? all[o.a].val : 0.0, y = o.b >= 0 ? all[o.b].val : 0.0, c = o.c;
    switch (o.code) {
      case T_CONST: case T_INPUT: break;
      case T_ADD: o.val = x + y; o.da = 1; o.db = 1; break;
      case T_SUB: o.val = x - y; o.da = 1; o.db = -1; break;
      case T_MUL: o.val = x * y; o.da = y; o.db = x; break;
      case T_DIV: { const double r = x / y; o.val = r; o.da = 1.0 / y; o.db = -r / y; break; }
      case T_ADDC: o.val = x + c; o.da = 1; break;
      case T_SUBC: o.val = x - c; o.da = 1; break;
      case T_MULC: o.val = x * c; o.da = c; break;
      case T_DIVC: o.val = x / c; o.da = 1.0 / c; break;
      case T_CSUB: o.val = c - x; o.da = -1; break;
      case T_CDIV: { const double r = c / x; o.val = r; o.da = -r / x; break; }
      case T_SQRT: { const double r = std::sqrt(x); o.val = r; o.da = 0.5 / r; break; }
      case T_EXP: { const double e = std::exp(x); o.val = e; o.da = e; break; }
      case T_LOG: o.val = std::log(x); o.da = 1.0 / x; break;
      case T_SQUARE: o.val = x * x; o.da = 2 * x; break;
      case T_LOG1M: o.val = std::log1p(-x); o.da = -1.0 / (1.0 - x); break;
      case T_STDNORMAL: o.val = -0.5 * x * x - 0.91893853320467274178; o.da = -x; break;
      case T_INVLOGIT: { const double il = 1.0 / (1.0 + std::exp(-x)); o.val = il; o.da = il * (1.0 - il); break; }
      case T_INVLOGIT_LOGJAC: {
        const double ax = std::fabs(x), sg = x >= 0 ? 1.0 : -1.0, e = std::exp(-ax);
        o.val = -ax - 2.0 * std::log1p(e); o.da = -sg + 2.0 * sg * e / (1.0 + e); break;
      }
    }
  }
  int node(int code, int a, int b, double c) {
    Op o; o.val = 0; o.a = a; o.b = b; o.da = 0; o.db = 0; o.c = c; o.code = code; o.k = -1;
    const int i = ops.push(o);
    eval(ops[(size_t)i], ops.buf.data());
    return i;
  }
  int leaf(double v) { Op o; o.val = v; o.a = -1; o.b = -1; o.da = 0; o.db = 0; o.c = 0; o.code = T_CONST; o.k = -1; return ops.push(o); }
  int input(int k, double v) { Op o; o.val = v; o.a = -1; o.b = -1; o.da = 0; o.db = 0; o.c = 0; o.code = T_INPUT; o.k = k; return ops.push(o); }
  double val(int i) const { return ops[(size_t)i].val; }
  void replay() {
    Op* const all = ops.buf.data();
    const size_t n = ops.size();
    for (size_t i = 0; i < n; ++i) if (all[i].code > T_INPUT) eval(all[i], all);
  }
  void backward() {
    for (int i = (int)ops.size() - 1; i >= 0; --i) {
      const Op& o = ops[(size_t)i];
      double g = adj[(size_t)i];
      if (g == 0.0) continue;
      if (o.a >= 0) adj[(size_t)o.a] += g * o.da;
      if (o.b >= 0) adj[(size_t)o.b] += g * o.db;
    }
  }
};

struct TV {
  Tape* t; int i;
  double v() const { return t->val(i); }
};
inline TV operator+(TV a, TV b) { return {a.t, a.t->node(T_ADD, a.i, b.i, 0)}; }
inline TV operator-(TV a, TV b) { return {a.t, a.t->node(T_SUB, a.i, b.i, 0)}; }
inline TV operator*(TV a, TV b) { return {a.t, a.t->node(T_MUL, a.i, b.i, 0)}; }
inline TV operator/(TV a, TV b) { return {a.t, a.t->node(T_DIV, a.i, b.i, 0)}; }
inline TV operator+(TV a, double c) { return {a.t, a.t->node(T_ADDC, a.i, -1, c)}; }
inline TV operator-(TV a, double c) { return {a.t, a.t->node(T_SUBC, a.i, -1, c)}; }
inline TV operator*(TV a, double c) { return {a.t, a.t->node(T_MULC, a.i, -1, c)}; }
inline TV operator*(double c, TV a) { return a * c; }
inline TV operator/(TV a, double c) { return {a.t, a.t->node(T_DIVC, a.i, -1, c)}; }
inline TV operator-(double c, TV a) { return {a.t, a.t->node(T_CSUB, a.i, -1, c)}; }
inline TV operator/(double c, TV a) { return {a.t, a.t->node(T_CDIV, a.i, -1, c)}; }
inline TV tsqrt(TV a) { return {a.t, a.t->node(T_SQRT, a.i, -1, 0)}; }
inline TV texp(TV a) { return {a.t, a.t->node(T_EXP, a.i, -1, 0)}; }
inline TV tlog(TV a) { return {a.t, a.t->node(T_LOG, a.i, -1, 0)}; }
inline TV tsquare(TV a) { return {a.t, a.t->node(T_SQUARE, a.i, -1, 0)}; }
inline TV tlog1m(TV a) { return {a.t, a.t->node(T_LOG1M, a.i, -1, 0)}; }
inline TV tstd_normal_lpdf(TV z) { return {z.t, z.t->node(T_STDNORMAL, z.i, -1, 0)}; }

struct StanSpec {
  int64_t N = 0; int K = 0, q = 0, t = 0, len_theta_L = 0;
  int is_binary = 0, prior_dist = 1, prior_dist_for_aux = 3;
  std::vector<double> prior_scale, prior_mean, prior_df;
  double prior_scale_for_aux = 1, prior_mean_for_aux = 0, prior_df_for_aux = 1;
  double global_prior_df = 1, global_prior_scale = 1, slab_df = 1, slab_scale = 1;
  std::vector<int> num_normals;
  std::vector<int> p, l;
  std::vector<double> shape, scale, concentration, regularization;
  int len_z_T = 0, len_rho = 0, len_conc = 0, D = 0, n_constrained = 0;
  int hs = 0, n_z_beta = 0, n_mix = 0, n_lambda = 0;
  std::vector<double> delta;
  void finish() {
    int sum_p = 0; len_z_T = 0; delta.clear();
    for (int i = 0; i < t; ++i) {
      sum_p += p[i];
      if (p[i] > 1) for (int j = 0; j < p[i]; ++j) delta.push_back(concentration[(size_t)j]);
      for (int j = 3; j <= p[i]; ++j) len_z_T += p[i] - 1;
    }
    len_rho = sum_p - t; len_conc = (int)delta.size();
    hs = prior_dist == 3 ? 2 : (prior_dist == 4 ? 4 : 0);
    n_z_beta = K;
    if (prior_dist == 7) { n_z_beta = 0; for (int k = 0; k < K; ++k) n_z_beta += num_normals[(size_t)k]; }
    n_mix = (prior_dist == 5 || prior_dist == 6) ? K : 0; n_lambda = prior_dist == 6 ? 1 : 0;
    D = n_z_beta + hs + hs * K + (hs > 0 ? 1 : 0) + n_mix + n_lambda + q + len_z_T + len_rho + len_conc + t + (is_binary ? 0 : 1);
    n_constrained = D + (is_binary ? 0 : 1) + K + q + len_theta_L;
  }
  int aux_pos() const { return D; }
  int beta_pos() const { return D + (is_binary ? 0 : 1); }
  int b_pos() const { return beta_pos() + K; }
};

typedef std::function<double(const double* beta, const double* b, double* gX, double* gZ)> Likelihood;

class HostModel {
 public:
  StanSpec sp;
  Likelihood lik;
  long gradEvals = 0;
  explicit HostModel(const StanSpec& s) : sp(s) { sp.finish(); plan_closed_form(); }
  int gradientCheck = 0;

  struct Fwd { TV sigma; std::vector<TV> beta, b, theta_L, constrained; TV lp; bool wantConstrained = true; };

  void forward(Tape& tp, const std::vector<double>& qv, Fwd& F, std::vector<int>& qidx, bool jacobian) const {
    tp.clear();
    tp.ops.reserve(4096);
    qidx.resize((size_t)sp.D);
    for (int i = 0; i < sp.D; ++i) qidx[(size_t)i] = tp.input(i, qv[(size_t)i]);
    auto Q = [&](int i) { return TV{&tp, qidx[(size_t)i]}; };
    TV lp{&tp, tp.leaf(0.0)};
    int pos = 0;
    std::vector<TV>& z_beta = w_[0]; std::vector<TV>& z_b = w_[1]; std::vector<TV>& z_T = w_[2];
    std::vector<TV>& rho = w_[3]; std::vector<TV>& zeta = w_[4]; std::vector<TV>& tau = w_[5];
    for (auto& v : w_) v.clear();
    for (int k = 0; k < sp.n_z_beta; ++k) z_beta.push_back(Q(pos++));
    auto lb0e = [&](int idx) { TV x = Q(idx); if (jacobian) lp = lp + x; return texp(x); };
    std::vector<TV>& global = sGlobal_; std::vector<TV>& caux = sCaux_; std::vector<TV>& lambda1 = sLambda_; std::vector<TV>& mix = sMix_;
    std::vector<std::vector<TV>>& local = sLocal_;
    global.clear(); caux.clear(); lambda1.clear(); mix.clear(); local.resize((size_t)sp.hs); for (auto& v : local) v.clear();
    for (int j = 0; j < sp.hs; ++j) global.push_back(lb0e(pos++));
    for (int j = 0; j < sp.hs; ++j) for (int k = 0; k < sp.K; ++k) local[(size_t)j].push_back(lb0e(pos++));
    if (sp.hs > 0) caux.push_back(lb0e(pos++));
    for (int k = 0; k < sp.n_mix; ++k) mix.push_back(lb0e(pos++));
    if (sp.n_lambda) lambda1.push_back(lb0e(pos++));
    for (int j = 0; j < sp.q; ++j) z_b.push_back(Q(pos++));
    for (int j = 0; j < sp.len_z_T; ++j) z_T.push_back(Q(pos++));
    for (int j = 0; j < sp.len_rho; ++j) {
      TV x = Q(pos++);
      rho.push_back(TV{&tp, tp.node(T_INVLOGIT, x.i, -1, 0)});
      if (jacobian) lp = lp + TV{&tp, tp.node(T_INVLOGIT_LOGJAC, x.i, -1, 0)};
    }
    auto lb0 = [&](int idx) { TV x = Q(idx); if (jacobian) lp = lp + x; return texp(x); };
    for (int j = 0; j < sp.len_conc; ++j) zeta.push_back(lb0(pos++));
    for (int j = 0; j < sp.t; ++j) tau.push_back(lb0(pos++));
    TV aux_unscaled{&tp, -1};
    if (!sp.is_binary) aux_unscaled = lb0(pos++);

    TV aux{&tp, tp.leaf(1.0)};
    if (!sp.is_binary) {
      if (sp.prior_dist_for_aux == 0) aux = aux_unscaled;
      else { aux = aux_unscaled * sp.prior_scale_for_aux; if (sp.prior_dist_for_aux <= 2) aux = aux + sp.prior_mean_for_aux; }
    }
    F.sigma = aux;
    F.beta.clear();
    if (sp.prior_dist <= 2) for (int k = 0; k < sp.K; ++k) {
      if (sp.prior_dist == 0) F.beta.push_back(z_beta[(size_t)k]);
      else if (sp.prior_dist == 1) F.beta.push_back(z_beta[(size_t)k] * sp.prior_scale[(size_t)k] + sp.prior_mean[(size_t)k]);
      else F.beta.push_back(cornish_fisher(z_beta[(size_t)k], sp.prior_df[(size_t)k]) * sp.prior_scale[(size_t)k] + sp.prior_mean[(size_t)k]);
    } else if (sp.hs > 0) {
      TV c2 = caux[0] * (sp.slab_scale * sp.slab_scale);
      TV tauG = global[0] * tsqrt(global[1]) * sp.global_prior_scale * aux;
      for (int k = 0; k < sp.K; ++k) {
        TV lam = local[0][(size_t)k] * tsqrt(local[1][(size_t)k]);
        if (sp.hs == 4) lam = lam * (local[2][(size_t)k] * tsqrt(local[3][(size_t)k]));
        TV lam2 = tsquare(lam);
        TV tilde = tsqrt(c2 * lam2 / (c2 + tsquare(tauG) * lam2));
        F.beta.push_back(z_beta[(size_t)k] * tilde * tauG);
      }
    } else if (sp.prior_dist == 5) {
      for (int k = 0; k < sp.K; ++k) F.beta.push_back(tsqrt(mix[(size_t)k] * 2.0) * sp.prior_scale[(size_t)k] * z_beta[(size_t)k] + sp.prior_mean[(size_t)k]);
    } else if (sp.prior_dist == 6) {
      for (int k = 0; k < sp.K; ++k)
        F.beta.push_back(lambda1[0] * sp.prior_scale[(size_t)k] * tsqrt(mix[(size_t)k] * 2.0) * z_beta[(size_t)k] + sp.prior_mean[(size_t)k]);
    } else {
      int zp = 0;
      for (int k = 0; k < sp.K; ++k) {
        TV bk = z_beta[(size_t)zp++];
        for (int n2 = 2; n2 <= sp.num_normals[(size_t)k]; ++n2) bk = bk * z_beta[(size_t)zp++];
        F.beta.push_back(bk * std::pow(sp.prior_scale[(size_t)k], (double)sp.num_normals[(size_t)k]) + sp.prior_mean[(size_t)k]);
      }
    }
    theta_L(tp, aux, tau, zeta, rho, z_T, F.theta_L);
    make_b(tp, z_b, F.theta_L, F.b);
    F.constrained.clear();
    if (F.wantConstrained) {
    for (auto& x : z_beta) F.constrained.push_back(x);
    for (auto& x : global) F.constrained.push_back(x);
    for (int k = 0; k < (sp.hs ? sp.K : 0); ++k) for (int j = 0; j < sp.hs; ++j) F.constrained.push_back(local[(size_t)j][(size_t)k]);
    for (auto& x : caux) F.constrained.push_back(x);
    for (auto& x : mix) F.constrained.push_back(x);
    for (auto& x : lambda1) F.constrained.push_back(x);
    for (auto& x : z_b) F.constrained.push_back(x);
    for (auto& x : z_T) F.constrained.push_back(x);
    for (auto& x : rho) F.constrained.push_back(x);
    for (auto& x : zeta) F.constrained.push_back(x);
    for (auto& x : tau) F.constrained.push_back(x);
    if (!sp.is_binary) F.constrained.push_back(aux_unscaled);
    }

    const double HALF_LOG_2PI = 0.91893853320467274178;
    if (!sp.is_binary && sp.prior_dist_for_aux > 0 && sp.prior_scale_for_aux > 0) {
      const double log_half = -0.693147180559945286;
      if (sp.prior_dist_for_aux == 1) lp = lp + (tsquare(aux_unscaled) * -0.5 - HALF_LOG_2PI) - log_half;
      else if (sp.prior_dist_for_aux == 2) {
        double nu = sp.prior_df_for_aux;
        TV tt = tlog(tsquare(aux_unscaled) / nu + 1.0) * (-(nu + 1.0) / 2.0);
        lp = lp + (tt + (lg((nu + 1.0) / 2.0) - lg(nu / 2.0) - 0.5 * std::log(nu * M_PI))) - log_half;
      } else lp = lp - aux_unscaled;
    }
    if (sp.prior_dist >= 1) for (auto& z : z_beta) lp = lp + tstd_normal_lpdf(z);
    {
      const double log_half = -0.693147180559945286;
      auto half_normal = [&](const std::vector<TV>& v) { for (auto& x : v) lp = lp + tstd_normal_lpdf(x); lp = lp - log_half; };
      auto inv_gamma = [&](TV x, double al, double be) { lp = lp + (tlog(x) * (-(al + 1.0)) - (1.0 / x) * be + (al * std::log(be) - lg(al))); };
      if (sp.hs > 0) {
        half_normal(local[0]);
        for (int k = 0; k < sp.K; ++k) inv_gamma(local[1][(size_t)k], 0.5 * sp.prior_df[(size_t)k], 0.5 * sp.prior_df[(size_t)k]);
        if (sp.hs == 4) {
          half_normal(local[2]);
          for (int k = 0; k < sp.K; ++k) inv_gamma(local[3][(size_t)k], 0.5 * sp.prior_scale[(size_t)k], 0.5 * sp.prior_scale[(size_t)k]);
        }
        lp = lp + tstd_normal_lpdf(global[0]) - log_half;
        inv_gamma(global[1], 0.5 * sp.global_prior_df, 0.5 * sp.global_prior_df);
        inv_gamma(caux[0], 0.5 * sp.slab_df, 0.5 * sp.slab_df);
      }
      for (auto& x : mix) lp = lp - x;
      if (sp.n_lambda) {
        double nu = sp.prior_df[0];
        lp = lp + (tlog(lambda1[0]) * (0.5 * nu - 1.0) - lambda1[0] * 0.5 - (0.5 * nu * std::log(2.0) + lg(0.5 * nu)));
      }
    }
    for (auto& z : z_b) lp = lp + tstd_normal_lpdf(z);
    for (auto& z : z_T) lp = lp + tstd_normal_lpdf(z);
    int pos_reg = 0, pos_rho = 0;
    for (int i = 0; i < sp.t; ++i) if (sp.p[(size_t)i] > 1) {
      int m = sp.p[(size_t)i] - 1;
      std::vector<double>& s1 = sS1_; std::vector<double>& s2 = sS2_; s1.assign((size_t)m, 0.0); s2.assign((size_t)m, 0.0);
      double nu = sp.regularization[(size_t)pos_reg++] + 0.5 * (sp.p[(size_t)i] - 2);
      s1[0] = nu; s2[0] = nu;
      for (int j = 2; j <= m; ++j) { nu -= 0.5; s1[(size_t)j - 1] = 0.5 * j; s2[(size_t)j - 1] = nu; }
      for (int j = 0; j < m; ++j) {
        TV r = rho[(size_t)(pos_rho + j)];
        double lbeta = lg(s1[(size_t)j]) + lg(s2[(size_t)j]) - lg(s1[(size_t)j] + s2[(size_t)j]);
        lp = lp + (tlog(r) * (s1[(size_t)j] - 1.0) + tlog1m(r) * (s2[(size_t)j] - 1.0) - lbeta);
      }
      pos_rho += m;
    }
    for (int j = 0; j < sp.len_conc; ++j) lp = lp + (tlog(zeta[(size_t)j]) * (sp.delta[(size_t)j] - 1.0) - zeta[(size_t)j] - lg(sp.delta[(size_t)j]));
    for (int j = 0; j < sp.t; ++j) lp = lp + (tlog(tau[(size_t)j]) * (sp.shape[(size_t)j] - 1.0) - tau[(size_t)j] - lg(sp.shape[(size_t)j]));
    F.lp = lp;
  }

  double log_prob_grad(const std::vector<double>& qv, std::vector<double>& grad) {
    if (closedForm_ && gradientCheck != 1) {
      ++gradEvals;
      grad.resize((size_t)sp.D);
      const double lp = closed_form_grad(qv.data(), grad.data());
      if (gradientCheck == 2) {
        std::vector<double> g2; const double lp2 = tape_grad(qv, g2); --gradEvals;
        double gmax = 0.0; for (double x : g2) if (std::isfinite(x)) gmax = std::max(gmax, std::fabs(x));
        auto off = [gmax](double a, double b) { return std::fabs(a - b) > 1e-9 * (std::fabs(a) + std::fabs(b)) + 1e-11 * gmax + 1e-300 && !(std::isnan(a) && std::isnan(b)) && !(std::isinf(a) && a == b); };
        bool bad = off(lp, lp2);
        for (int i = 0; i < sp.D; ++i) bad = bad || off(grad[(size_t)i], g2[(size_t)i]);
        if (bad) {
          std::string m = "closed-form gradient differs from the tape: lp " + std::to_string(lp) + " vs " + std::to_string(lp2);
          char buf[96];
          for (int i = 0; i < sp.D; ++i) if (off(grad[(size_t)i], g2[(size_t)i])) { std::snprintf(buf, sizeof buf, "; g[%d] %.17g vs %.17g (q %.6g)", i, grad[(size_t)i], g2[(size_t)i], qv[(size_t)i]); m += buf; }
          throw std::logic_error(m);
        }
      }
      return lp;
    }
    return tape_grad(qv, grad);
  }
  double tape_grad(const std::vector<double>& qv, std::vector<double>& grad) {
    ++gradEvals;
    Fwd& F = fwd_; std::vector<int>& qidx = qidx_;
    F.wantConstrained = false;
#ifdef S4B_NUTS_TIMING
    const auto t0 = std::chrono::steady_clock::now();
#endif
    if (tapeHoldsGradient_) {
      for (int i = 0; i < sp.D; ++i) tape_.ops[(size_t)qidx[(size_t)i]].val = qv[(size_t)i];
      tape_.replay();
    } else { forward(tape_, qv, F, qidx, true); tapeHoldsGradient_ = true; }
#ifdef S4B_NUTS_TIMING
    const auto t1 = std::chrono::steady_clock::now();
#endif
    std::vector<double>& beta = bufBeta_; std::vector<double>& b = bufB_; std::vector<double>& gX = bufGX_; std::vector<double>& gZ = bufGZ_;
    beta.resize((size_t)sp.K); b.resize((size_t)sp.q); gX.assign((size_t)sp.K, 0.0); gZ.assign((size_t)sp.q, 0.0);
    for (int k = 0; k < sp.K; ++k) beta[(size_t)k] = F.beta[(size_t)k].v();
    for (int j = 0; j < sp.q; ++j) b[(size_t)j] = F.b[(size_t)j].v();
    double sigma = F.sigma.v();
    double ss = lik(beta.data(), b.data(), gX.data(), gZ.data());
    double s2 = sigma * sigma, N = (double)sp.N;
    double ll = -0.5 * ss / s2 - N * std::log(sigma) - N * 0.91893853320467274178;
    tape_.adj.assign(tape_.ops.size(), 0.0);
    tape_.adj[(size_t)F.lp.i] = 1.0;
    tape_.adj[(size_t)F.sigma.i] += ss / (s2 * sigma) - N / sigma;
    for (int k = 0; k < sp.K; ++k) tape_.adj[(size_t)F.beta[(size_t)k].i] += gX[(size_t)k] / s2;
    for (int j = 0; j < sp.q; ++j) tape_.adj[(size_t)F.b[(size_t)j].i] += gZ[(size_t)j] / s2;
#ifdef S4B_NUTS_TIMING
    const auto t2 = std::chrono::steady_clock::now();
#endif
    tape_.backward();
    grad.resize((size_t)sp.D);
    for (int i = 0; i < sp.D; ++i) grad[(size_t)i] = tape_.adj[(size_t)qidx[(size_t)i]];
#ifdef S4B_NUTS_TIMING
    { const auto t3 = std::chrono::steady_clock::now(); auto us = [](auto a, auto b) { return std::chrono::duration<double, std::micro>(b - a).count(); };
      tFwd_ += us(t0, t1); tLik_ += us(t1, t2); tBwd_ += us(t2, t3);
      if (gradEvals % 5000 == 0) std::fprintf(stderr, "S4B gradient us: forward %.2f lik %.2f backward %.2f (tape %zu nodes)\n", tFwd_ / gradEvals, tLik_ / gradEvals, tBwd_ / gradEvals, tape_.ops.size()); }
#endif
    return F.lp.v() + ll;
  }

  void write_array(const std::vector<double>& qv, double* out) {
    Fwd F; std::vector<int> qidx;
    F.wantConstrained = true;
    tapeHoldsGradient_ = false;
    forward(tape_, qv, F, qidx, false);
    int o = 0;
    for (auto& x : F.constrained) out[o++] = x.v();
    if (!sp.is_binary) out[o++] = F.sigma.v();
    for (auto& x : F.beta) out[o++] = x.v();
    for (auto& x : F.b) out[o++] = x.v();
    for (auto& x : F.theta_L) out[o++] = x.v();
  }

  bool has_closed_form() const { return closedForm_; }

 private:
  struct CfTerm { int p, l, zb0, rho, zeta, tau; double scale, betaA, lbeta, delta0, delta1, lgDelta0, lgDelta1, shape, lgShape; };
  struct CfWork { double tau, A, rho, e, z0, z1, S, pi0, pi1, trace, sd1, T21, sq; };
  std::vector<CfWork> cfWork_;
  bool closedForm_ = false;
  std::vector<CfTerm> cfTerms_;
  int cfRho0_ = 0, cfZeta0_ = 0, cfTau0_ = 0, cfAux_ = 0;
  double cfAuxConst_ = 0;
  std::vector<double> cfBeta_, cfB_, cfGX_, cfGZ_, cfTh_;
  void plan_closed_form() {
    closedForm_ = false;
    if (sp.prior_dist > 1 || sp.hs || sp.n_mix || sp.n_lambda || sp.len_z_T) return;
    for (int i = 0; i < sp.t; ++i) if (sp.p[(size_t)i] > 2 || sp.p[(size_t)i] < 1) return;
    cfRho0_ = sp.K + sp.q; cfZeta0_ = cfRho0_ + sp.len_rho; cfTau0_ = cfZeta0_ + sp.len_conc; cfAux_ = cfTau0_ + sp.t;
    cfTerms_.clear();
    int zb = sp.K, rho = cfRho0_, zeta = cfZeta0_, reg = 0, dl = 0;
    for (int i = 0; i < sp.t; ++i) {
      CfTerm c{}; c.p = sp.p[(size_t)i]; c.l = sp.l[(size_t)i]; c.zb0 = zb; c.tau = cfTau0_ + i; c.scale = sp.scale[(size_t)i];
      c.shape = sp.shape[(size_t)i]; c.lgShape = lg(c.shape);
      c.rho = -1; c.zeta = -1;
      if (c.p == 2) {
        c.rho = rho++; c.zeta = zeta; zeta += 2;
        const double nu = sp.regularization[(size_t)reg++];
        c.betaA = nu; c.lbeta = lg(nu) + lg(nu) - lg(nu + nu);
        c.delta0 = sp.delta[(size_t)dl]; c.delta1 = sp.delta[(size_t)dl + 1]; dl += 2;
        c.lgDelta0 = lg(c.delta0); c.lgDelta1 = lg(c.delta1);
      }
      zb += c.p * c.l;
      cfTerms_.push_back(c);
    }
    if (!sp.is_binary && sp.prior_dist_for_aux == 2) {
      const double nu = sp.prior_df_for_aux;
      cfAuxConst_ = lg((nu + 1.0) / 2.0) - lg(nu / 2.0) - 0.5 * std::log(nu * M_PI);
    }
    cfBeta_.assign((size_t)sp.K + 1, 0.0); cfB_.assign((size_t)sp.q + 1, 0.0); cfGX_.assign((size_t)sp.K + 1, 0.0); cfGZ_.assign((size_t)sp.q + 1, 0.0);
    cfTh_.assign((size_t)(3 * sp.t + 1), 0.0); cfWork_.assign((size_t)sp.t + 1, CfWork{});
    closedForm_ = true;
  }
  double closed_form_grad(const double* q, double* g) {
    const double HALF_LOG_2PI = 0.91893853320467274178, LOG_HALF = -0.693147180559945286;
    const int K = sp.K, nq = sp.q, t = sp.t;
    double lp = 0.0;
    double u = 1.0, aux = 1.0, dAuxDu = 0.0;
    if (!sp.is_binary) {
      u = std::exp(q[cfAux_]); lp += q[cfAux_];
      if (sp.prior_dist_for_aux == 0) { aux = u; dAuxDu = 1.0; }
      else { aux = u * sp.prior_scale_for_aux; dAuxDu = sp.prior_scale_for_aux; if (sp.prior_dist_for_aux <= 2) aux += sp.prior_mean_for_aux; }
    }
    double* const beta = cfBeta_.data(); double* const b = cfB_.data();
    if (sp.prior_dist == 0) for (int k = 0; k < K; ++k) beta[k] = q[k];
    else for (int k = 0; k < K; ++k) { beta[k] = q[k] * sp.prior_scale[(size_t)k] + sp.prior_mean[(size_t)k]; lp += -0.5 * q[k] * q[k] - HALF_LOG_2PI; }
    double* const th = cfTh_.data();
    for (int i = 0; i < t; ++i) {
      const CfTerm& c = cfTerms_[(size_t)i];
      CfWork& w = cfWork_[(size_t)i];
      const double tau = std::exp(q[c.tau]); lp += q[c.tau];
      const double A = tau * c.scale * aux;
      w.tau = tau; w.A = A;
      const double* zb = q + c.zb0;
      double* bo = b + (c.zb0 - K);
      if (c.p == 1) {
        th[3 * i] = A;
        for (int s = 0; s < c.l; ++s) { bo[s] = A * zb[s]; lp += -0.5 * zb[s] * zb[s] - HALF_LOG_2PI; }
      } else {
        const double x = q[c.rho], ax = std::fabs(x), e = std::exp(-ax);
        const double rho = x >= 0 ? 1.0 / (1.0 + e) : e / (1.0 + e);
        lp += -ax - 2.0 * std::log1p(e);
        const double z0 = std::exp(q[c.zeta]), z1 = std::exp(q[c.zeta + 1]); lp += q[c.zeta] + q[c.zeta + 1];
        const double trace = A * A * 2.0, S = z0 + z1, pi0 = z0 / S, pi1 = z1 / S;
        const double sd0 = std::sqrt(pi0 * trace), sd1 = std::sqrt(pi1 * trace), T21 = rho * 2.0 - 1.0, sq = std::sqrt(1.0 - T21 * T21);
        const double T00 = sd0, T10 = sd1 * T21, T11 = sd1 * sq;
        th[3 * i] = T00; th[3 * i + 1] = T10; th[3 * i + 2] = T11;
        w.rho = rho; w.e = e; w.z0 = z0; w.z1 = z1; w.S = S; w.pi0 = pi0; w.pi1 = pi1; w.trace = trace; w.sd1 = sd1; w.T21 = T21; w.sq = sq;
        for (int j = 0; j < c.l; ++j) {
          const double a0 = zb[2 * j], a1 = zb[2 * j + 1];
          bo[2 * j] = T00 * a0; bo[2 * j + 1] = T10 * a0 + T11 * a1;
          lp += (-0.5 * a0 * a0 - HALF_LOG_2PI) + (-0.5 * a1 * a1 - HALF_LOG_2PI);
        }
        lp += std::log(rho) * (c.betaA - 1.0) + std::log1p(-rho) * (c.betaA - 1.0) - c.lbeta;
        lp += (q[c.zeta] * (c.delta0 - 1.0) - z0 - c.lgDelta0) + (q[c.zeta + 1] * (c.delta1 - 1.0) - z1 - c.lgDelta1);
      }
      lp += q[c.tau] * (c.shape - 1.0) - tau - c.lgShape;
    }
    double dLpDu = 0.0;
    if (!sp.is_binary && sp.prior_dist_for_aux > 0 && sp.prior_scale_for_aux > 0) {
      if (sp.prior_dist_for_aux == 1) { lp += (-0.5 * u * u - HALF_LOG_2PI) - LOG_HALF; dLpDu = -u; }
      else if (sp.prior_dist_for_aux == 2) {
        const double nu = sp.prior_df_for_aux;
        lp += std::log(u * u / nu + 1.0) * (-(nu + 1.0) / 2.0) + cfAuxConst_ - LOG_HALF; dLpDu = -(nu + 1.0) * u / (nu + u * u);
      } else { lp -= u; dLpDu = -1.0; }
    }
    double* const gX = cfGX_.data(); double* const gZ = cfGZ_.data();
    for (int k = 0; k < K; ++k) gX[k] = 0.0;
    for (int j = 0; j < nq; ++j) gZ[j] = 0.0;
    const double ss = lik(beta, b, gX, gZ);
    const double s2 = aux * aux, N = (double)sp.N, is2 = 1.0 / s2;
    const double ll = -0.5 * ss / s2 - N * std::log(aux) - N * HALF_LOG_2PI;
    double dAux = ss / (s2 * aux) - N / aux;
    if (sp.prior_dist == 0) for (int k = 0; k < K; ++k) g[k] = gX[k] * is2;
    else for (int k = 0; k < K; ++k) g[k] = gX[k] * is2 * sp.prior_scale[(size_t)k] - q[k];
    for (int i = 0; i < t; ++i) {
      const CfTerm& c = cfTerms_[(size_t)i];
      const double* zb = q + c.zb0; const double* gb = gZ + (c.zb0 - K); double* gz = g + c.zb0;
      const CfWork& w = cfWork_[(size_t)i];
      const double tau = w.tau, A = w.A;
      double dA = 0.0;
      if (c.p == 1) {
        double dTh = 0.0;
        for (int s = 0; s < c.l; ++s) { const double db = gb[s] * is2; dTh += db * zb[s]; gz[s] = db * A - zb[s]; }
        dA = dTh;
      } else {
        const double T00 = th[3 * i], T10 = th[3 * i + 1], T11 = th[3 * i + 2];
        double d00 = 0.0, d10 = 0.0, d11 = 0.0;
        for (int j = 0; j < c.l; ++j) {
          const double a0 = zb[2 * j], a1 = zb[2 * j + 1], db0 = gb[2 * j] * is2, db1 = gb[2 * j + 1] * is2;
          d00 += db0 * a0; d10 += db1 * a0; d11 += db1 * a1;
          gz[2 * j] = db0 * T00 + db1 * T10 - a0; gz[2 * j + 1] = db1 * T11 - a1;
        }
        const double sg = q[c.rho] >= 0 ? 1.0 : -1.0, e = w.e, rho = w.rho, z0 = w.z0, z1 = w.z1;
        const double trace = w.trace, S = w.S, pi0 = w.pi0, pi1 = w.pi1, sd0 = T00, sd1 = w.sd1, T21 = w.T21, sq = w.sq;
        const double dsd0 = d00, dsd1 = d10 * T21 + d11 * sq, dT21 = d10 * sd1 - d11 * sd1 * (T21 / sq);
        const double dpi0 = dsd0 * trace * (0.5 / sd0), dpi1 = dsd1 * trace * (0.5 / sd1);
        const double dtrace = dsd0 * pi0 * (0.5 / sd0) + dsd1 * pi1 * (0.5 / sd1);
        const double dS = -(dpi0 * pi0 + dpi1 * pi1) / S;
        double dz0 = dpi0 / S + dS, dz1 = dpi1 / S + dS;
        dA = dtrace * 4.0 * A;
        double drho = 2.0 * dT21 + (c.betaA - 1.0) / rho - (c.betaA - 1.0) / (1.0 - rho);
        g[c.rho] = drho * rho * (1.0 - rho) + (-sg + 2.0 * sg * e / (1.0 + e));
        g[c.zeta] = dz0 * z0 + 1.0 + (c.delta0 - 1.0) - z0;
        g[c.zeta + 1] = dz1 * z1 + 1.0 + (c.delta1 - 1.0) - z1;
      }
      const double dtau = dA * c.scale * aux;
      dAux += dA * tau * c.scale;
      g[c.tau] = dtau * tau + 1.0 + (c.shape - 1.0) - tau;
    }
    if (!sp.is_binary) g[cfAux_] = (dAux * dAuxDu + dLpDu) * u + 1.0;
    return lp + ll;
  }

  mutable std::vector<std::pair<double, double>> lgMemo_;
  double lg(double x) const {
    for (const auto& e : lgMemo_) if (e.first == x) return e.second;
    const double v = std::lgamma(x);
    if (lgMemo_.size() < 64) lgMemo_.emplace_back(x, v);
    return v;
  }
  mutable std::vector<TV> sGlobal_, sCaux_, sLambda_, sMix_, sT_, sPi_; mutable std::vector<std::vector<TV>> sLocal_;
  mutable std::vector<double> sS1_, sS2_; mutable std::vector<int> sIdx_;
#ifdef S4B_NUTS_TIMING
  double tFwd_ = 0, tLik_ = 0, tBwd_ = 0;
#endif
  Tape tape_; bool tapeHoldsGradient_ = false;
  mutable std::vector<TV> w_[6];
  Fwd fwd_; std::vector<int> qidx_; std::vector<double> bufBeta_, bufB_, bufGX_, bufGZ_;
  static TV cornish_fisher(TV z, double df) {
    TV z2 = tsquare(z), z3 = z2 * z, z5 = z2 * z3, z7 = z2 * z5, z9 = z2 * z7;
    double df2 = df * df, df3 = df2 * df, df4 = df2 * df2;
    return z + (z3 + z) / (4 * df) + (z5 * 5.0 + z3 * 16.0 + z * 3.0) / (96 * df2) +
           (z7 * 3.0 + z5 * 19.0 + z3 * 17.0 - z * 15.0) / (384 * df3) +
           (z9 * 79.0 + z7 * 776.0 + z5 * 1482.0 - z3 * 1920.0 - z * 945.0) / (92160 * df4);
  }
  void theta_L(Tape& tp, TV dispersion, const std::vector<TV>& tau, const std::vector<TV>& zeta, const std::vector<TV>& rho,
               const std::vector<TV>& z_T, std::vector<TV>& out) const {
    out.clear();
    int zeta_mark = 0, rho_mark = 0, z_T_mark = 0;
    for (int i = 0; i < sp.t; ++i) {
      int nc = sp.p[(size_t)i];
      TV A = tau[(size_t)i] * sp.scale[(size_t)i] * dispersion;
      if (nc == 1) { out.push_back(A); continue; }
      TV zero{&tp, tp.leaf(0.0)};
      std::vector<TV>& T = sT_; T.assign((size_t)(nc * nc), zero);
      auto at = [&](int r, int c) -> TV& { return T[(size_t)(r * nc + c)]; };
      TV trace = tsquare(A) * (double)nc;
      TV sum_pi = zeta[(size_t)zeta_mark];
      for (int j = 1; j < nc; ++j) sum_pi = sum_pi + zeta[(size_t)(zeta_mark + j)];
      std::vector<TV>& pi = sPi_; pi.clear();
      for (int j = 0; j < nc; ++j) pi.push_back(zeta[(size_t)(zeta_mark + j)] / sum_pi);
      zeta_mark += nc;
      TV std_dev = tsqrt(pi[0] * trace);
      at(0, 0) = std_dev;
      std_dev = tsqrt(pi[1] * trace);
      TV T21 = rho[(size_t)rho_mark] * 2.0 - 1.0;
      rho_mark += 1;
      at(1, 1) = std_dev * tsqrt(1.0 - tsquare(T21));
      at(1, 0) = std_dev * T21;
      for (int r = 2; r <= nc - 1; ++r) {
        TV dot = tsquare(z_T[(size_t)z_T_mark]);
// ... 27 lines not shown
          }
          b_mark += nc;
        }
      }
    }
    (void)tp;
  }
};

class StanRng {
 public:
  void create(uint32_t seed, uint32_t chain) {
    x1_ = seed % 2147483563u; if (!x1_) x1_ = 1;
    x2_ = seed % 2147483399u; if (!x2_) x2_ = 1;
    uint64_t z = (uint64_t(1) << 50) * chain;
    x1_ = (uint32_t)(mulpow(40014, z, 2147483563ull) * x1_ % 2147483563ull);
    x2_ = (uint32_t)(mulpow(40692, z, 2147483399ull) * x2_ % 2147483399ull);
    build_tables();
  }
  uint32_t raw() {
    x1_ = (uint32_t)(40014ull * x1_ % 2147483563ull);
    x2_ = (uint32_t)(40692ull * x2_ % 2147483399ull);
    return x2_ < x1_ ? x1_ - x2_ : x1_ - x2_ + 2147483562u;
  }
  double u01() { return (double)(raw() - 1u) / 2147483562.0; }
  void get_state(uint32_t out[2]) const { out[0] = x1_; out[1] = x2_; }
  void set_state(const uint32_t in[2]) { x1_ = in[0]; x2_ = in[1]; }
  double uniform(double a, double b) { for (;;) { double r = u01() * (b - a) + a; if (r < b) return r; } }
  double normal() {
    for (;;) {
      double u; int bucket; pair8(u, bucket);
      int sign = (bucket & 1) * 2 - 1, i = bucket >> 1;
      double x = u * nx_[i];
      if (x < nx_[i + 1]) return x * sign;
      if (i == 0) {
        for (;;) { double tx = expo() / nx_[1], ty = expo(); if (2.0 * ty > tx * tx) return (tx + nx_[1]) * sign; }
      }
      double y = ny_[i] + u01() * (ny_[i + 1] - ny_[i]);
      if (y < std::exp(-0.5 * x * x)) return x * sign;
    }
  }
 private:
  uint32_t x1_ = 1, x2_ = 1;
  double nx_[129], ny_[129], ex_[257], ey_[257];
  static uint64_t mulpow(uint64_t a, uint64_t e, uint64_t m) { uint64_t r = 1; a %= m; while (e) { if (e & 1) r = r * a % m; a = a * a % m; e >>= 1; } return r; }
  uint32_t digit30() { uint32_t u; do { u = raw() - 1u; } while (u >= (1u << 30)); return u; }
  void pair8(double& r, int& bucket) {
    uint32_t a = digit30(), b = digit30(), c = digit30();
    bucket = (int)(a & 255u);
    r = std::ldexp((double)(a >> 8), -22);
    r = std::ldexp(r + (double)b, -30);
    r = 0.5 * (r + (double)(c & 1u));
  }
  double expo() {
    double shift = 0.0;
    for (;;) {
      double u; int i; pair8(u, i);
      double x = u * ex_[i];
      if (x < ex_[i + 1]) return shift + x;
      if (i == 0) { shift += ex_[1]; continue; }
      double y = ey_[i] + u01() * (ey_[i + 1] - ey_[i]);
      if (y < std::exp(-x)) return shift + x;
    }
  }
  void build_tables() {
    const double r = 3.442619855899, v = 9.91256303526217e-3;
    nx_[1] = r; ny_[1] = std::exp(-0.5 * r * r); nx_[0] = v / ny_[1]; ny_[0] = 0;
    for (int i = 2; i < 128; ++i) { ny_[i] = ny_[i - 1] + v / nx_[i - 1]; nx_[i] = std::sqrt(-2.0 * std::log(ny_[i])); }
    nx_[128] = 0; ny_[128] = 1;
    const double re = 7.69711747013104972, ve = 3.949659822581572e-3;
    ex_[1] = re; ey_[1] = std::exp(-re); ex_[0] = ve / ey_[1]; ey_[0] = 0;
    for (int i = 2; i < 256; ++i) { ey_[i] = ey_[i - 1] + ve / ex_[i - 1]; ex_[i] = -std::log(ey_[i]); }
    ex_[256] = 0; ey_[256] = 1;
  }
};

struct NutsControl {
  uint32_t seed = 0; double init_r = 2.0; int skip = 1;
  double gamma = 0.05, delta = 0.8, kappa = 0.75, t0 = 10;
  unsigned init_buffer = 75, term_buffer = 50, window = 25;
  double stepsize = 1, jitter = 0; int max_depth = 10;
};

class Nuts {
 public:
  typedef std::vector<double> V;
  struct Pt { V q, p, g; double Vv = 0; };

  Nuts(HostModel& m, const NutsControl& c, unsigned chain, int num_warmup) : model_(m), D_(m.sp.D), skip_(c.skip) {
    rng_.create(c.seed, chain);
    bool ok = false;
    for (int attempt = 0; attempt < (c.init_r == 0 ? 1 : 100) && !ok; ++attempt) {
      cont_.assign((size_t)D_, 0.0);
      if (c.init_r != 0) for (int i = 0; i < D_; ++i) cont_[(size_t)i] = rng_.uniform(-c.init_r, c.init_r);
      V g;
      double lp = model_.log_prob_grad(cont_, g);
      if (!std::isfinite(lp)) continue;
      lp = model_.log_prob_grad(cont_, g);
      double s = 0; for (double x : g) s += x;
      ok = std::isfinite(s);
    }
    if (!ok) throw std::domain_error("Initialization failed.");
    inv_metric_.assign((size_t)D_, 1.0);
    z_.q = cont_; z_.p.assign((size_t)D_, 0.0); z_.g.assign((size_t)D_, 0.0);
    wm_.assign((size_t)D_, 0.0); wm2_.assign((size_t)D_, 0.0);
    if (c.stepsize > 0) nom_eps_ = c.stepsize;
    if (c.jitter > 0 && c.jitter < 1) jitter_ = c.jitter;
    if (c.max_depth > 0) max_depth_ = c.max_depth;
    mu_ = std::log(10 * c.stepsize);
    if (c.delta > 0 && c.delta < 1) delta_ = c.delta;
    if (c.gamma > 0) gamma_ = c.gamma;
    if (c.kappa > 0) kappa_ = c.kappa;
    if (c.t0 > 0) t0_ = c.t0;
    next_window_ = init_buffer_ + window_size_ - 1;
    set_windows((unsigned)(num_warmup * c.skip), c.init_buffer, c.term_buffer, c.window);
    init_stepsize();
  }

  void run(double* row) {
    for (int s = 0; s < skip_; ++s) transition();
    row[0] = lp_; row[1] = accept_; row[2] = eps_; row[3] = depth_; row[4] = n_leapfrog_; row[5] = divergent_ ? 1 : 0; row[6] = energy_;
    model_.write_array(cont_, row + 7);
  }
  void disengage() { adapting_ = false; nom_eps_ = std::exp(x_bar_); }
  void totals(double out[4]) const { out[0] = (double)nTrans_; out[1] = (double)sumDepth_; out[2] = (double)sumLeap_; out[3] = (double)nDiv_; }

  struct State {
    V q, inv_metric, wm, wm2;
    double stepsize = 0, mu = 0, counter = 0, s_bar = 0, x_bar = 0, wn = 0;
    int32_t adapting = 1;
    uint32_t window[7] = {0, 0, 0, 0, 0, 0, 0};
    uint32_t rng[2] = {1, 1};
    double last[7] = {0, 0, 0, 0, 0, 0, 0};
  };
  void get_state(State& s) const {
    s.q = cont_; s.inv_metric = inv_metric_; s.wm = wm_; s.wm2 = wm2_;
    s.stepsize = nom_eps_; s.mu = mu_; s.counter = counter_; s.s_bar = s_bar_; s.x_bar = x_bar_; s.wn = wn_;
    s.adapting = adapting_ ? 1 : 0;
    const uint32_t w[7] = {num_warmup_, init_buffer_, term_buffer_, base_window_, window_counter_, next_window_, window_size_};
    for (int i = 0; i < 7; ++i) s.window[i] = w[i];
    rng_.get_state(s.rng);
    const double l[7] = {lp_, accept_, eps_, (double)depth_, (double)n_leapfrog_, divergent_ ? 1.0 : 0.0, energy_};
    for (int i = 0; i < 7; ++i) s.last[i] = l[i];
  }
  void set_state(const State& s) {
    if ((int)s.q.size() != D_ || (int)s.inv_metric.size() != D_ || (int)s.wm.size() != D_ || (int)s.wm2.size() != D_)
      throw std::invalid_argument("sampler state: wrong number of unconstrained parameters");
    cont_ = s.q; z_.q = s.q; inv_metric_ = s.inv_metric; wm_ = s.wm; wm2_ = s.wm2;
    nom_eps_ = s.stepsize; mu_ = s.mu; counter_ = s.counter; s_bar_ = s.s_bar; x_bar_ = s.x_bar; wn_ = s.wn;
    adapting_ = s.adapting != 0;
    num_warmup_ = s.window[0]; init_buffer_ = s.window[1]; term_buffer_ = s.window[2]; base_window_ = s.window[3];
    window_counter_ = s.window[4]; next_window_ = s.window[5]; window_size_ = s.window[6];
    rng_.set_state(s.rng);
    lp_ = s.last[0]; accept_ = s.last[1]; eps_ = s.last[2]; depth_ = (int)s.last[3]; n_leapfrog_ = (int)s.last[4];
    divergent_ = s.last[5] != 0.0; energy_ = s.last[6];
  }
  void current_row(double* row) {
    row[0] = lp_; row[1] = accept_; row[2] = eps_; row[3] = depth_; row[4] = n_leapfrog_; row[5] = divergent_ ? 1 : 0; row[6] = energy_;
    model_.write_array(cont_, row + 7);
  }

 private:
  HostModel& model_; int D_, skip_;
  StanRng rng_;
  Pt z_; V inv_metric_, cont_;
  double nom_eps_ = 0.1, eps_ = 0.1, jitter_ = 0; int max_depth_ = 10;
  double lp_ = 0, accept_ = 0, energy_ = 0; int depth_ = 0, n_leapfrog_ = 0; bool divergent_ = false, adapting_ = true;
  double mu_ = 0.5, delta_ = 0.5, gamma_ = 0.05, kappa_ = 0.75, t0_ = 10, counter_ = 0, s_bar_ = 0, x_bar_ = 0;
  unsigned num_warmup_ = 0, init_buffer_ = 0, term_buffer_ = 0, base_window_ = 0, window_counter_ = 0, next_window_ = 0, window_size_ = 0;
  double wn_ = 0; V wm_, wm2_;
  long nTrans_ = 0, sumDepth_ = 0, sumLeap_ = 0, nDiv_ = 0;

  double kinetic() const { double s = 0; for (int i = 0; i < D_; ++i) s += z_.p[(size_t)i] * (inv_metric_[(size_t)i] * z_.p[(size_t)i]); return 0.5 * s; }
  double hamiltonian() const { return kinetic() + z_.Vv; }
  void grad() { z_.Vv = -model_.log_prob_grad(z_.q, z_.g); for (double& x : z_.g) x = -x; }
  void draw_momentum() { for (int i = 0; i < D_; ++i) z_.p[(size_t)i] = rng_.normal() / std::sqrt(inv_metric_[(size_t)i]); }
  void leapfrog(double e) {
    for (int i = 0; i < D_; ++i) z_.p[(size_t)i] -= (0.5 * e) * z_.g[(size_t)i];
    for (int i = 0; i < D_; ++i) z_.q[(size_t)i] += e * (inv_metric_[(size_t)i] * z_.p[(size_t)i]);
    grad();
    for (int i = 0; i < D_; ++i) z_.p[(size_t)i] -= (0.5 * e) * z_.g[(size_t)i];
  }
  V sharp() const { V r((size_t)D_); for (int i = 0; i < D_; ++i) r[(size_t)i] = inv_metric_[(size_t)i] * z_.p[(size_t)i]; return r; }
  static double finite_or_inf(double h) { return std::isnan(h) ? std::numeric_limits<double>::infinity() : h; }

  void init_stepsize() {
    Pt z0 = z_;
    if (nom_eps_ == 0 || nom_eps_ > 1e7 || std::isnan(nom_eps_)) return;
    const double thr = std::log(0.8);
    draw_momentum(); grad();
    double H0 = hamiltonian();
    leapfrog(nom_eps_);
    double dH = H0 - finite_or_inf(hamiltonian());
    int dir = dH > thr ? 1 : -1;
    for (;;) {
      z_ = z0;
      draw_momentum(); grad();
      double H0b = hamiltonian();
      leapfrog(nom_eps_);
      double d = H0b - finite_or_inf(hamiltonian());
      if (dir == 1 && !(d > thr)) break;
      if (dir == -1 && !(d < thr)) break;
      nom_eps_ = dir == 1 ? 2 * nom_eps_ : 0.5 * nom_eps_;
      if (nom_eps_ > 1e7) throw std::runtime_error("Posterior is improper. Please check your model.");
      if (nom_eps_ == 0) throw std::runtime_error("No acceptably small step size could be found. Perhaps the posterior is not continuous?");
    }
    z_ = z0;
  }

  static double lse(double a, double b) {
    const double ninf = -std::numeric_limits<double>::infinity();
    if (a == ninf) return b;
    if (b == ninf) return a;
    return a > b ? a + std::log1p(std::exp(b - a)) : b + std::log1p(std::exp(a - b));
  }
  static bool uturn_ok(const V& sharp_minus, const V& sharp_plus, const V& rho) {
    double a = 0, b = 0;
    for (size_t i = 0; i < rho.size(); ++i) { a += sharp_plus[i] * rho[i]; b += sharp_minus[i] * rho[i]; }
    return a > 0 && b > 0;
  }
  static V vsum(const V& a, const V& b) { V r(a.size()); for (size_t i = 0; i < a.size(); ++i) r[i] = a[i] + b[i]; return r; }

  struct Acc { int n_leapfrog = 0; double sum_metro = 0; };

  struct Prop { V q; double Vv = 0, H = 0; };
  struct Level { V p_init_end, sharp_init_end, rho_init, p_final_beg, sharp_final_beg, rho_final; Prop propose_final; };
  std::vector<Level> lv_;
  void ensure_levels() {
    if ((int)lv_.size() == max_depth_ + 1) return;
    lv_.resize((size_t)max_depth_ + 1);
    for (Level& l : lv_)
      for (V* v : {&l.p_init_end, &l.sharp_init_end, &l.rho_init, &l.p_final_beg, &l.sharp_final_beg, &l.rho_final, &l.propose_final.q}) v->assign((size_t)D_, 0.0);
  }

  bool subtree(int depth, Prop& propose, V& sharp_beg, V& sharp_end, V& rho, V& p_beg, V& p_end, double H0, double sign,
               double& lsw, Acc& acc) {
    const double ninf = -std::numeric_limits<double>::infinity();
    const int D = D_;
    if (depth == 0) {
      const double e = sign * eps_, he = 0.5 * e;
      {
        double* __restrict__ const p = z_.p.data(); double* __restrict__ const q = z_.q.data();
        const double* __restrict__ const g = z_.g.data(); const double* __restrict__ const im = inv_metric_.data();
        for (int i = 0; i < D; ++i) { const double pi = p[i] - he * g[i]; p[i] = pi; q[i] += e * (im[i] * pi); }
      }
      grad();
      ++acc.n_leapfrog;
      double kin = 0.0;
      {
        double* __restrict__ const p = z_.p.data(); const double* __restrict__ const g = z_.g.data(); const double* __restrict__ const im = inv_metric_.data();
        double* __restrict__ const sb = sharp_beg.data(); double* __restrict__ const se = sharp_end.data(); double* __restrict__ const rh = rho.data();
        double* __restrict__ const pb = p_beg.data(); double* __restrict__ const pe = p_end.data();
        for (int i = 0; i < D; ++i) {
          const double pi = p[i] - he * g[i], sh = im[i] * pi;
          p[i] = pi; kin += pi * sh; sb[i] = sh; se[i] = sh; rh[i] += pi; pb[i] = pi; pe[i] = pi;
        }
      }
      const double hRaw = 0.5 * kin + z_.Vv, h = finite_or_inf(hRaw);
      if (h - H0 > 1000.0) divergent_ = true;
      lsw = lse(lsw, H0 - h);
      acc.sum_metro += (H0 - h > 0) ? 1.0 : std::exp(H0 - h);
      std::copy(z_.q.begin(), z_.q.end(), propose.q.begin()); propose.Vv = z_.Vv; propose.H = hRaw;
      return !divergent_;
    }
    Level& L = lv_[(size_t)depth];
    double lsw_init = ninf;
    std::fill(L.rho_init.begin(), L.rho_init.end(), 0.0);
    if (!subtree(depth - 1, propose, sharp_beg, L.sharp_init_end, L.rho_init, p_beg, L.p_init_end, H0, sign, lsw_init, acc)) return false;
    double lsw_final = ninf;
    std::fill(L.rho_final.begin(), L.rho_final.end(), 0.0);
    if (!subtree(depth - 1, L.propose_final, L.sharp_final_beg, sharp_end, L.rho_final, L.p_final_beg, p_end, H0, sign, lsw_final, acc)) return false;
    double lsw_sub = lse(lsw_init, lsw_final);
    lsw = lse(lsw, lsw_sub);
    if (lsw_final > lsw_sub) std::swap(propose, L.propose_final);
    else if (rng_.u01() < std::exp(lsw_final - lsw_sub)) std::swap(propose, L.propose_final);
    double a1 = 0, b1 = 0, a2 = 0, b2 = 0, a3 = 0, b3 = 0;
    {
      const double* __restrict__ const ri = L.rho_init.data(); const double* __restrict__ const rf = L.rho_final.data();
      const double* __restrict__ const pfb = L.p_final_beg.data(); const double* __restrict__ const pie = L.p_init_end.data();
      const double* __restrict__ const sb = sharp_beg.data(); const double* __restrict__ const se = sharp_end.data();
      const double* __restrict__ const sfb = L.sharp_final_beg.data(); const double* __restrict__ const sie = L.sharp_init_end.data();
      double* __restrict__ const rh = rho.data();
      for (int i = 0; i < D; ++i) {
        const double rs = ri[i] + rf[i], t2 = ri[i] + pfb[i], t3 = rf[i] + pie[i];
        rh[i] += rs;
        a1 += se[i] * rs; b1 += sb[i] * rs;
        a2 += sfb[i] * t2; b2 += sb[i] * t2;
        a3 += se[i] * t3; b3 += sie[i] * t3;
      }
    }
    return (a1 > 0 && b1 > 0) & (a2 > 0 && b2 > 0) & (a3 > 0 && b3 > 0);
  }

  void nuts_transition() {
    const double ninf = -std::numeric_limits<double>::infinity();
    eps_ = nom_eps_;
    if (jitter_) eps_ *= 1.0 + jitter_ * (2.0 * rng_.u01() - 1.0);
    ensure_levels();
    z_.q = cont_;
    draw_momentum(); grad();
    const double H0 = hamiltonian();
    Pt& fwd = tFwd_; Pt& bck = tBck_; fwd = z_; bck = z_;
    Prop& sample = tSample_; Prop& propose = tPropose_;
    sample.q = z_.q; sample.Vv = z_.Vv; sample.H = H0; propose = sample;
    V& p_ff = tV_[0]; V& s_ff = tV_[1]; V& p_fb = tV_[2]; V& s_fb = tV_[3]; V& p_bf = tV_[4]; V& s_bf = tV_[5]; V& p_bb = tV_[6]; V& s_bb = tV_[7];
    V& rho = tV_[8]; V& rho_f = tV_[9]; V& rho_b = tV_[10];
    p_ff = z_.p; s_ff = sharp(); p_fb = z_.p; s_fb = s_ff; p_bf = z_.p; s_bf = s_ff; p_bb = z_.p; s_bb = s_ff;
    rho = z_.p;
    double lsw = 0;
    Acc acc;
    depth_ = 0; divergent_ = false;
    while (depth_ < max_depth_) {
      rho_f.assign((size_t)D_, 0.0); rho_b.assign((size_t)D_, 0.0);
      bool valid; double lsw_sub = ninf;
      if (rng_.u01() > 0.5) {
        z_ = fwd; rho_b = rho; p_bf = p_ff; s_bf = s_ff;
        valid = subtree(depth_, propose, s_fb, s_ff, rho_f, p_fb, p_ff, H0, 1, lsw_sub, acc);
        fwd = z_;
      } else {
        z_ = bck; rho_f = rho; p_fb = p_bb; s_fb = s_bb;
        valid = subtree(depth_, propose, s_bf, s_bb, rho_b, p_bf, p_bb, H0, -1, lsw_sub, acc);
        bck = z_;
      }
      if (!valid) break;
      ++depth_;
      if (lsw_sub > lsw) sample = propose;
      else if (rng_.u01() < std::exp(lsw_sub - lsw)) sample = propose;
      lsw = lse(lsw, lsw_sub);
      rho = vsum(rho_b, rho_f);
      bool ok = uturn_ok(s_bb, s_ff, rho);
      ok &= uturn_ok(s_bb, s_fb, vsum(rho_b, p_fb));
      ok &= uturn_ok(s_bf, s_ff, vsum(rho_f, p_bf));
      if (!ok) break;
    }
    n_leapfrog_ = acc.n_leapfrog;
    ++nTrans_; sumDepth_ += depth_; sumLeap_ += acc.n_leapfrog; if (divergent_) ++nDiv_;
    accept_ = acc.sum_metro / (double)acc.n_leapfrog;
    z_.q = sample.q; z_.Vv = sample.Vv;
    energy_ = sample.H;
    cont_ = z_.q; lp_ = -z_.Vv;
  }
  Pt tFwd_, tBck_; Prop tSample_, tPropose_; V tV_[11];

  void transition() {
    nuts_transition();
    if (!adapting_) return;
    ++counter_;
    double a = accept_ > 1 ? 1 : accept_;
    double eta = 1.0 / (counter_ + t0_);
    s_bar_ = (1.0 - eta) * s_bar_ + eta * (delta_ - a);
    double x = mu_ - s_bar_ * std::sqrt(counter_) / gamma_;
    double x_eta = std::pow(counter_, -kappa_);
    x_bar_ = (1.0 - x_eta) * x_bar_ + x_eta * x;
    nom_eps_ = std::exp(x);
    bool in_window = window_counter_ >= init_buffer_ && window_counter_ < num_warmup_ - term_buffer_ && window_counter_ != num_warmup_;
    if (in_window) {
      ++wn_;
      for (int i = 0; i < D_; ++i) { double d = z_.q[(size_t)i] - wm_[(size_t)i]; wm_[(size_t)i] += d / wn_; wm2_[(size_t)i] += d * (z_.q[(size_t)i] - wm_[(size_t)i]); }
    }
    bool window_end = window_counter_ == next_window_ && window_counter_ != num_warmup_;
    if (window_end) {
      next_window();
      for (int i = 0; i < D_; ++i) {
        double var = wn_ > 1 ? wm2_[(size_t)i] / (wn_ - 1.0) : inv_metric_[(size_t)i];
        inv_metric_[(size_t)i] = (wn_ / (wn_ + 5.0)) * var + 1e-3 * (5.0 / (wn_ + 5.0));
      }
      wn_ = 0; wm_.assign((size_t)D_, 0.0); wm2_.assign((size_t)D_, 0.0);
      ++window_counter_;
      init_stepsize();
      mu_ = std::log(10 * nom_eps_);
      counter_ = 0; s_bar_ = 0; x_bar_ = 0;
      return;
    }
    ++window_counter_;
  }
  void set_windows(unsigned num_warmup, unsigned init_buffer, unsigned term_buffer, unsigned base_window) {
    if (num_warmup < 20) return;
    if (init_buffer + base_window + term_buffer > num_warmup) {
      num_warmup_ = num_warmup;
      init_buffer_ = (unsigned)(0.15 * num_warmup);
      term_buffer_ = (unsigned)(0.10 * num_warmup);
      base_window_ = num_warmup - (init_buffer_ + term_buffer_);
      return;
// ... 17 lines not shown
```

Before: 504.6.

## Add run-ahead helper threads precomputing NUTS leapfrog trajectories plus AVX2 host loops

Adds helper threads that speculatively integrate the leapfrog trajectory in the backward (and optionally forward) direction using the closed-form Gram likelihood, so the NUTS tree builder can take precomputed states instead of evaluating gradients serially. It also adds AVX2 versions of the dense Gram gradient, kick/drift, leaf-finish and U-turn merge loops, with FP contraction disabled to keep results bit-identical. Helpers are placed on neighbouring CPUs, enabled by default with one helper, and only used when hmc_mode is 0 with a Gram matrix. The cost is thread synchronisation, wasted speculative steps when trees terminate early, and extra memory for stored states.

```diff
diff --git a/include/stan4bart_amd.h b/include/stan4bart_amd.h
--- a/include/stan4bart_amd.h
+++ b/include/stan4bart_amd.h
@@ -444,6 +444,10 @@
 
 int S4B_FN(get_nuts_stats)(s4b_sampler* s, double out[4]);
 
+int S4B_FN(set_nuts_helpers)(s4b_sampler* s, int32_t n);
+int S4B_FN(get_nuts_runahead)(s4b_sampler* s, int64_t out[4]);
+int S4B_FN(set_host_vector)(int32_t on, int32_t* effective);
+
 int S4B_FN(profile_sweep)(s4b_sampler* s, int32_t n_sweeps, double out[8]);
 int S4B_FN(stream_probe)(int32_t device, int64_t n_doubles, int32_t reps, double out[4]);
 
diff --git a/stan4bart_amd/abi.py b/stan4bart_amd/abi.py
--- a/stan4bart_amd/abi.py
+++ b/stan4bart_amd/abi.py
@@ -264,6 +264,15 @@
 
 
 LATENT_MODES = {"exact": 0, "parallel": 1}
+
+def set_host_vector(lib, prefix: str, on: Optional[bool]) -> bool:
+    fn = getattr(lib, prefix + "set_host_vector")
+    fn.restype, fn.argtypes = C.c_int, [C.c_int32, c_int32_p]
+    eff = C.c_int32()
+    if fn(-1 if on is None else int(bool(on)), C.byref(eff)) != 0:
+        raise RuntimeError(getattr(lib, prefix + "last_error")().decode())
+    return bool(eff.value)
+
 
 @dataclass
 class SamplerArgs:
@@ -457,6 +466,7 @@
             "get_state": [vp, vp, i64, C.POINTER(i64)], "set_state": [vp, vp, i64],
             "set_trace": [vp, i32], "get_trace": [vp, i64, ip, C.POINTER(i64)],
             "get_leaf_assignment": [vp, i32, ip], "get_counters": [vp, C.POINTER(i64)], "get_nuts_stats": [vp, dp],
+            "set_nuts_helpers": [vp, i32], "get_nuts_runahead": [vp, C.POINTER(i64)],
             "profile_sweep": [vp, i32, dp], "profile_leapfrog": [vp, i32, dp],
             "set_progress": [vp, PROGRESS, vp], "set_device_sharing": [vp, i32],
             "set_tree_path": [vp, i32], "get_tree_path": [vp, ip], "get_fused_stats": [vp, C.POINTER(i64)], "get_sweep_stats": [vp, C.POINTER(i64)], "get_sweep_busy": [vp, C.POINTER(i64)], "get_sweep_spec": [vp, C.POINTER(i64)], "set_test_hook": [vp, i32, i64], "set_hmc_mode": [vp, i32], "get_hmc_mode": [vp, ip],
@@ -748,6 +758,14 @@
         out = (C.c_double * 4)()
         self._check(self._f("get_nuts_stats")(self._h, out))
         return dict(transitions=int(out[0]), sum_treedepth=int(out[1]), sum_n_leapfrog=int(out[2]), divergent=int(out[3]))
+
+    def set_nuts_helpers(self, n: int, wait: bool = False) -> None:
+        self._check(self._f("set_nuts_helpers")(self._h, int(n) | (16 if wait and n else 0)))
+
+    def get_nuts_runahead(self) -> dict:
+        out = (C.c_int64 * 4)()
+        self._check(self._f("get_nuts_runahead")(self._h, out))
+        return dict(taken=int(out[0]), not_ready=int(out[1]), unconsumed=int(out[2]), transitions_without_helper=int(out[3]))
 
     def predict_bart(self, x_test: np.ndarray, offset_test: Optional[np.ndarray] = None) -> np.ndarray:
         xt = _f64(x_test)
diff --git a/stan4bart_amd/csrc/c_api.inc b/stan4bart_amd/csrc/c_api.inc
--- a/stan4bart_amd/csrc/c_api.inc
+++ b/stan4bart_amd/csrc/c_api.inc
@@ -183,6 +183,9 @@
 int S4B_FN(get_sweep_busy)(s4b_sampler* s, int64_t* out) { S4B_NEED(s, "get_sweep_busy") S4B_TRY if (!out) throw std::invalid_argument("get_sweep_busy: NULL output pointer"); *out = s->core.dev().sweep_busy(); S4B_CATCH }
 int S4B_FN(get_counters)(s4b_sampler* s, int64_t out[3]) { S4B_NEED(s, "get_counters") S4B_TRY s->core.dev().bind(); s->core.counters(out); S4B_CATCH }
 int S4B_FN(get_nuts_stats)(s4b_sampler* s, double out[4]) { S4B_NEED(s, "get_nuts_stats") S4B_TRY s->core.dev().bind(); s->core.nuts_stats(out); S4B_CATCH }
+int S4B_FN(set_nuts_helpers)(s4b_sampler* s, int32_t n) { S4B_NEED(s, "set_nuts_helpers") S4B_TRY s->core.set_nuts_helpers(n); S4B_CATCH }
+int S4B_FN(get_nuts_runahead)(s4b_sampler* s, int64_t out[4]) { S4B_NEED(s, "get_nuts_runahead") S4B_TRY if (!out) throw std::invalid_argument("get_nuts_runahead: NULL output pointer"); s->core.nuts_runahead(out); S4B_CATCH }
+int S4B_FN(set_host_vector)(int32_t on, int32_t* effective) { S4B_TRY const int v = on < 0 ? (s4b::host_vector_on() ? 1 : 0) : s4b::set_host_vector(on); if (effective) *effective = v; S4B_CATCH }
 int S4B_FN(profile_sweep)(s4b_sampler* s, int32_t n_sweeps, double out[8]) { S4B_NEED(s, "profile_sweep") S4B_TRY s->core.dev().bind(); s->core.profile_sweep(n_sweeps, out); S4B_CATCH }
 int S4B_FN(profile_leapfrog)(s4b_sampler* s, int32_t n_evals, double out[8]) { S4B_NEED(s, "profile_leapfrog") S4B_TRY s->core.dev().bind(); s->core.profile_leapfrog(n_evals, out); S4B_CATCH }
 int S4B_FN(stream_probe)(int32_t device, int64_t n_doubles, int32_t reps, double out[4]) { S4B_TRY S4B_DEV::probe_stream(device, n_doubles, reps, out); S4B_CATCH }
diff --git a/stan4bart_amd/csrc/sampler_core.hpp b/stan4bart_amd/csrc/sampler_core.hpp
--- a/stan4bart_amd/csrc/sampler_core.hpp
+++ b/stan4bart_amd/csrc/sampler_core.hpp
@@ -337,7 +337,7 @@
 
     if (hmcMode_ == 0) { build_gram(sd); haveGram_ = true; }
     dev_.stan_inputs( 0, false, cX_.data(), cZ_.data(), &s0_, nullptr);
-    model_->lik = [this](const double* beta, const double* b, double* gX, double* gZ) { return likelihood(beta, b, gX, gZ); };
+    model_->lik = [this](const double* beta, const double* b, double* gX, double* gZ, double* th) { return likelihood(beta, b, gX, gZ, th); };
     NutsControl nc;
     nc.seed = sc->seed; nc.init_r = sc->init_r; nc.skip = sc->skip;
     if (nc.skip <= 0) { nc.skip = (2000 - warmup_) / 1000; if (nc.skip < 1) nc.skip = 1; }
@@ -345,6 +345,8 @@
     nc.init_buffer = sc->adapt_init_buffer; nc.term_buffer = sc->adapt_term_buffer; nc.window = sc->adapt_window;
     nc.stepsize = sc->stepsize; nc.jitter = sc->stepsize_jitter; nc.max_depth = sc->max_treedepth;
     nuts_.reset(new Nuts(*model_, nc, 1, warmup_));
+    { const char* e = std::getenv("S4B_NUTS_HELPERS"); const int n = e && *e ? std::atoi(e) : 1; nuts_->set_helpers(n < 0 ? 0 : (n > 2 ? 2 : n)); }
+    sync_runahead();
     row_.assign((size_t)(7 + model_->sp.n_constrained), 0.0);
 
     std::vector<double> bartOffset(n_, 0.0);
@@ -1318,7 +1320,14 @@
     if (mode != 0 && mode != 1) throw std::invalid_argument("hmc_mode must be 0 (sufficient statistics) or 1 (one device evaluation per leapfrog)");
     if (mode == 0 && !haveGram_) throw std::invalid_argument("this sampler was created with hmc_mode 1: it has no Gram matrix to evaluate from sufficient statistics");
     hmcMode_ = mode;
-  }
+    sync_runahead();
+  }
+  void set_nuts_helpers(int n) {
+    live();
+    if (n < 0 || (n & ~16) > 2) throw std::invalid_argument("nuts helpers must be 0 (none), 1 (the backward direction) or 2 (both directions), plus 16 to wait for a helper");
+    if (nuts_) nuts_->set_helpers(n & 3, (n & 16) != 0);
+  }
+  void nuts_runahead(int64_t out[4]) { live(); for (int i = 0; i < 4; ++i) out[i] = 0; if (nuts_) nuts_->runahead_counters(out); }
   static constexpr bool kLatentMode = has_latent_mode<Dev>::value;
   int latent_mode() const { live(); return latMode_; }
   void set_latent_mode(int mode) {
@@ -1770,26 +1779,14 @@
     }
     for (int a = 0; a < M; ++a) if (gramPtr_[(size_t)a + 1] < gramPtr_[(size_t)a]) gramPtr_[(size_t)a + 1] = gramPtr_[(size_t)a];
   }
-  double likelihood(const double* beta, const double* b, double* gX, double* gZ) {
+  void sync_runahead() { if (nuts_) nuts_->set_runahead_allowed(model_->has_closed_form() && hmcMode_ == 0 && haveGram_ && model_->gradientCheck == 0); }
+  double likelihood(const double* beta, const double* b, double* gX, double* gZ, double* th) {
     if (hmcMode_ != 0) return dev_.leapfrog_sums(beta, b, gX, gZ);
     const int M = K_ + q_;
-    if (thetaBuf_.size() < (size_t)M + 4) thetaBuf_.assign((size_t)M + 4, 0.0);
-    double* const th = thetaBuf_.data();
     for (int k = 0; k < K_; ++k) th[k] = beta[k];
     for (int j = 0; j < q_; ++j) th[K_ + j] = b[j];
     if (gramLd_) {
-      const double* const G = gramDense_.data(); const int ld = gramLd_;
-      double ss = s0_;
-      for (int a = 0; a < M; ++a) {
-        const double* const r = G + (size_t)a * ld;
-        double p0 = 0.0, p1 = 0.0, p2 = 0.0, p3 = 0.0;
-        for (int c = 0; c < ld; c += 4) { p0 += r[c] * th[c]; p1 += r[c + 1] * th[c + 1]; p2 += r[c + 2] * th[c + 2]; p3 += r[c + 3] * th[c + 3]; }
-        const double ga = (p0 + p2) + (p1 + p3);
-        const double ca = a < K_ ? cX_[(size_t)a] : cZ_[(size_t)(a - K_)];
-        ss += th[a] * (ga - 2.0 * ca);
-        if (a < K_) gX[a] = ca - ga; else gZ[a - K_] = ca - ga;
-      }
-      return ss;
+      return hostloop::gram_dense(host_vector_on(), gramDense_.data(), gramLd_, M, K_, th, cX_.data(), cZ_.data(), s0_, gX, gZ);
     }
     const int* const ptr = gramPtr_.data(); const int* const col = gramCol_.data(); const double* const g = gram_.data();
     double ss = s0_;
@@ -1812,7 +1809,6 @@
 
   Dev dev_;
   size_t n_ = 0, nTest_ = 0; int P_ = 0, T_ = 0, nc_ = 256, thin_ = 1, K_ = 0, q_ = 0, hmcMode_ = 0; bool haveGram_ = false;
-  std::vector<double> thetaBuf_;
   int warmup_ = 0, verbose_ = 0, refresh_ = 0, offsetType_ = 0; s4b_progress_fn progress_ = nullptr; void* progressUser_ = nullptr; bool keepFits_ = true, hasUserOffset_ = false, binary_ = false;
   std::vector<double> userOffset_;
   s4b_callback_fn callback_ = nullptr; void* callbackUser_ = nullptr;
diff --git a/stan4bart_amd/csrc/stan_host.hpp b/stan4bart_amd/csrc/stan_host.hpp
--- a/stan4bart_amd/csrc/stan_host.hpp
+++ b/stan4bart_amd/csrc/stan_host.hpp
@@ -2,17 +2,219 @@
 #define S4B_STAN_HOST_HPP
 
 #include <algorithm>
+#include <atomic>
 #include <cmath>
+#include <condition_variable>
 #include <cstdint>
+#include <cstdlib>
 #include <functional>
 #include <chrono>
 #include <cstdio>
 #include <limits>
+#include <memory>
+#include <mutex>
 #include <stdexcept>
 #include <string>
+#include <thread>
 #include <vector>
+#if defined(__linux__)
+#include <pthread.h>
+#include <sched.h>
+#endif
+#if defined(__x86_64__) && !defined(__HIP_DEVICE_COMPILE__)
+#include <immintrin.h>
+#define S4B_HOST_AVX2 1
+#define S4B_TARGET_AVX2 __attribute__((target("avx2")))
+#endif
+#if defined(__clang__)
+#define S4B_NO_CONTRACT
+#define S4B_NO_CONTRACT_BODY _Pragma("clang fp contract(off)")
+#elif defined(__GNUC__)
+#define S4B_NO_CONTRACT __attribute__((optimize("fp-contract=off")))
+#define S4B_NO_CONTRACT_BODY
+#else
+#define S4B_NO_CONTRACT
+#define S4B_NO_CONTRACT_BODY
+#endif
 
 namespace s4b {
+
+inline bool host_vector_supported() {
+#ifdef S4B_HOST_AVX2
+  return __builtin_cpu_supports("avx2") != 0;
+#else
+  return false;
+#endif
+}
+inline std::atomic<int>& host_vector_flag() {
+  static std::atomic<int> f{[] { const char* e = std::getenv("S4B_HOST_VECTOR"); return (host_vector_supported() && !(e && std::atoi(e) == 0)) ? 1 : 0; }()};
+  return f;
+}
+inline bool host_vector_on() { return host_vector_flag().load(std::memory_order_relaxed) != 0; }
+inline int set_host_vector(int on) { const int v = (on && host_vector_supported()) ? 1 : 0; host_vector_flag().store(v, std::memory_order_relaxed); return v; }
+inline void cpu_pause() {
+#ifdef S4B_HOST_AVX2
+  _mm_pause();
+#else
+  std::this_thread::yield();
+#endif
+}
+
+namespace hostloop {
+S4B_NO_CONTRACT inline double gram_dense_scalar(const double* G, int ld, int M, int K, const double* th, const double* cX, const double* cZ, double s0, double* gX, double* gZ) {
+  S4B_NO_CONTRACT_BODY
+  double ss = s0;
+  for (int a = 0; a < M; ++a) {
+    const double* const r = G + (size_t)a * ld;
+    double p0 = 0.0, p1 = 0.0, p2 = 0.0, p3 = 0.0;
+    for (int c = 0; c < ld; c += 4) { p0 += r[c] * th[c]; p1 += r[c + 1] * th[c + 1]; p2 += r[c + 2] * th[c + 2]; p3 += r[c + 3] * th[c + 3]; }
+    const double ga = (p0 + p2) + (p1 + p3);
+    const double ca = a < K ? cX[a] : cZ[a - K];
+    ss += th[a] * (ga - 2.0 * ca);
+    if (a < K) gX[a] = ca - ga; else gZ[a - K] = ca - ga;
+  }
+  return ss;
+}
+S4B_NO_CONTRACT inline void kick_drift_scalar(int D, double e, double he, double* __restrict__ p, double* __restrict__ q, const double* __restrict__ g, const double* __restrict__ im) {
+  S4B_NO_CONTRACT_BODY
+  for (int i = 0; i < D; ++i) { const double pi = p[i] - he * g[i]; p[i] = pi; q[i] += e * (im[i] * pi); }
+}
+template <bool Kick>
+S4B_NO_CONTRACT inline double leaf_finish_scalar(int D, double he, double* __restrict__ p, const double* __restrict__ g, const double* __restrict__ im, double* __restrict__ sb,
+                                 double* __restrict__ se, double* __restrict__ rh, double* __restrict__ pb, double* __restrict__ pe) {
+  S4B_NO_CONTRACT_BODY
+  double kin = 0.0;
+  for (int i = 0; i < D; ++i) {
+    const double pi = Kick ? p[i] - he * g[i] : p[i], sh = im[i] * pi;
+    p[i] = pi; kin += pi * sh; sb[i] = sh; se[i] = sh; rh[i] += pi; pb[i] = pi; pe[i] = pi;
+  }
+  return kin;
+}
+S4B_NO_CONTRACT inline void merge_scalar(int D, const double* __restrict__ ri, const double* __restrict__ rf, const double* __restrict__ pfb, const double* __restrict__ pie,
+                         const double* __restrict__ sb, const double* __restrict__ se, const double* __restrict__ sfb, const double* __restrict__ sie,
+                         double* __restrict__ rh, double out[6]) {
+  S4B_NO_CONTRACT_BODY
+  double a1 = 0, b1 = 0, a2 = 0, b2 = 0, a3 = 0, b3 = 0;
+  for (int i = 0; i < D; ++i) {
+    const double rs = ri[i] + rf[i], t2 = ri[i] + pfb[i], t3 = rf[i] + pie[i];
+    rh[i] += rs;
+    a1 += se[i] * rs; b1 += sb[i] * rs;
+    a2 += sfb[i] * t2; b2 += sb[i] * t2;
+    a3 += se[i] * t3; b3 += sie[i] * t3;
+  }
+  out[0] = a1; out[1] = b1; out[2] = a2; out[3] = b2; out[4] = a3; out[5] = b3;
+}
+#ifdef S4B_HOST_AVX2
+S4B_TARGET_AVX2 S4B_NO_CONTRACT inline double gram_dense_avx2(const double* G, int ld, int M, int K, const double* th, const double* cX, const double* cZ, double s0, double* gX, double* gZ) {
+  S4B_NO_CONTRACT_BODY
+  double ss = s0;
+  for (int a = 0; a < M; ++a) {
+    const double* const r = G + (size_t)a * ld;
+    __m256d acc = _mm256_setzero_pd();
+    for (int c = 0; c < ld; c += 4) acc = _mm256_add_pd(acc, _mm256_mul_pd(_mm256_loadu_pd(r + c), _mm256_loadu_pd(th + c)));
+    const __m128d s = _mm_add_pd(_mm256_castpd256_pd128(acc), _mm256_extractf128_pd(acc, 1));
+    const double ga = _mm_cvtsd_f64(_mm_add_sd(s, _mm_unpackhi_pd(s, s)));
+    const double ca = a < K ? cX[a] : cZ[a - K];
+    ss += th[a] * (ga - 2.0 * ca);
+    if (a < K) gX[a] = ca - ga; else gZ[a - K] = ca - ga;
+  }
+  return ss;
+}
+S4B_TARGET_AVX2 S4B_NO_CONTRACT inline void kick_drift_avx2(int D, double e, double he, double* __restrict__ p, double* __restrict__ q, const double* __restrict__ g, const double* __restrict__ im) {
+  S4B_NO_CONTRACT_BODY
+  const __m256d ve = _mm256_set1_pd(e), vhe = _mm256_set1_pd(he);
+  int i = 0;
+  for (; i + 4 <= D; i += 4) {
+    const __m256d pi = _mm256_sub_pd(_mm256_loadu_pd(p + i), _mm256_mul_pd(vhe, _mm256_loadu_pd(g + i)));
+    _mm256_storeu_pd(p + i, pi);
+    _mm256_storeu_pd(q + i, _mm256_add_pd(_mm256_loadu_pd(q + i), _mm256_mul_pd(ve, _mm256_mul_pd(_mm256_loadu_pd(im + i), pi))));
+  }
+  for (; i < D; ++i) { const double pi = p[i] - he * g[i]; p[i] = pi; q[i] += e * (im[i] * pi); }
+}
+template <bool Kick>
+S4B_TARGET_AVX2 S4B_NO_CONTRACT inline double leaf_finish_avx2(int D, double he, double* __restrict__ p, const double* __restrict__ g, const double* __restrict__ im, double* __restrict__ sb,
+                                               double* __restrict__ se, double* __restrict__ rh, double* __restrict__ pb, double* __restrict__ pe) {
+  S4B_NO_CONTRACT_BODY
+  const __m256d vhe = _mm256_set1_pd(he);
+  double kin = 0.0;
+  int i = 0;
+  for (; i + 4 <= D; i += 4) {
+    __m256d pi = _mm256_loadu_pd(p + i);
+    if (Kick) pi = _mm256_sub_pd(pi, _mm256_mul_pd(vhe, _mm256_loadu_pd(g + i)));
+    const __m256d sh = _mm256_mul_pd(_mm256_loadu_pd(im + i), pi);
+    alignas(32) double t[4];
+    _mm256_store_pd(t, _mm256_mul_pd(pi, sh));
+    kin += t[0]; kin += t[1]; kin += t[2]; kin += t[3];
+    _mm256_storeu_pd(p + i, pi); _mm256_storeu_pd(sb + i, sh); _mm256_storeu_pd(se + i, sh);
+    _mm256_storeu_pd(rh + i, _mm256_add_pd(_mm256_loadu_pd(rh + i), pi)); _mm256_storeu_pd(pb + i, pi); _mm256_storeu_pd(pe + i, pi);
+  }
+  for (; i < D; ++i) {
+    const double pi = Kick ? p[i] - he * g[i] : p[i], sh = im[i] * pi;
+    p[i] = pi; kin += pi * sh; sb[i] = sh; se[i] = sh; rh[i] += pi; pb[i] = pi; pe[i] = pi;
+  }
+  return kin;
+}
+S4B_TARGET_AVX2 S4B_NO_CONTRACT inline void merge_avx2(int D, const double* __restrict__ ri, const double* __restrict__ rf, const double* __restrict__ pfb, const double* __restrict__ pie,
+                                       const double* __restrict__ sb, const double* __restrict__ se, const double* __restrict__ sfb, const double* __restrict__ sie,
+                                       double* __restrict__ rh, double out[6]) {
+  S4B_NO_CONTRACT_BODY
+  __m256d acc4 = _mm256_setzero_pd(); __m128d acc2 = _mm_setzero_pd();
+  int i = 0;
+  for (; i + 4 <= D; i += 4) {
+    const __m256d vri = _mm256_loadu_pd(ri + i), vrf = _mm256_loadu_pd(rf + i), vsb = _mm256_loadu_pd(sb + i), vse = _mm256_loadu_pd(se + i);
+    const __m256d rs = _mm256_add_pd(vri, vrf), t2 = _mm256_add_pd(vri, _mm256_loadu_pd(pfb + i)), t3 = _mm256_add_pd(vrf, _mm256_loadu_pd(pie + i));
+    _mm256_storeu_pd(rh + i, _mm256_add_pd(_mm256_loadu_pd(rh + i), rs));
+    const __m256d pa1 = _mm256_mul_pd(vse, rs), pb1 = _mm256_mul_pd(vsb, rs), pa2 = _mm256_mul_pd(_mm256_loadu_pd(sfb + i), t2), pb2 = _mm256_mul_pd(vsb, t2);
+    const __m256d pa3 = _mm256_mul_pd(vse, t3), pb3 = _mm256_mul_pd(_mm256_loadu_pd(sie + i), t3);
+    const __m256d u0 = _mm256_unpacklo_pd(pa1, pb1), u1 = _mm256_unpackhi_pd(pa1, pb1), u2 = _mm256_unpacklo_pd(pa2, pb2), u3 = _mm256_unpackhi_pd(pa2, pb2);
+    acc4 = _mm256_add_pd(acc4, _mm256_permute2f128_pd(u0, u2, 0x20));
+    acc4 = _mm256_add_pd(acc4, _mm256_permute2f128_pd(u1, u3, 0x20));
+    acc4 = _mm256_add_pd(acc4, _mm256_permute2f128_pd(u0, u2, 0x31));
+    acc4 = _mm256_add_pd(acc4, _mm256_permute2f128_pd(u1, u3, 0x31));
+    const __m256d w0 = _mm256_unpacklo_pd(pa3, pb3), w1 = _mm256_unpackhi_pd(pa3, pb3);
+    acc2 = _mm_add_pd(acc2, _mm256_castpd256_pd128(w0)); acc2 = _mm_add_pd(acc2, _mm256_castpd256_pd128(w1));
+    acc2 = _mm_add_pd(acc2, _mm256_extractf128_pd(w0, 1)); acc2 = _mm_add_pd(acc2, _mm256_extractf128_pd(w1, 1));
+  }
+  alignas(32) double t[4]; alignas(16) double u[2];
+  _mm256_store_pd(t, acc4); _mm_store_pd(u, acc2);
+  double a1 = t[0], b1 = t[1], a2 = t[2], b2 = t[3], a3 = u[0], b3 = u[1];
+  for (; i < D; ++i) {
+    const double rs = ri[i] + rf[i], t2 = ri[i] + pfb[i], t3 = rf[i] + pie[i];
+    rh[i] += rs;
+    a1 += se[i] * rs; b1 += sb[i] * rs;
+    a2 += sfb[i] * t2; b2 += sb[i] * t2;
+    a3 += se[i] * t3; b3 += sie[i] * t3;
+  }
+  out[0] = a1; out[1] = b1; out[2] = a2; out[3] = b2; out[4] = a3; out[5] = b3;
+}
+#endif
+inline double gram_dense(bool vec, const double* G, int ld, int M, int K, const double* th, const double* cX, const double* cZ, double s0, double* gX, double* gZ) {
+#ifdef S4B_HOST_AVX2
+  if (vec) return gram_dense_avx2(G, ld, M, K, th, cX, cZ, s0, gX, gZ);
+#endif
+  (void)vec; return gram_dense_scalar(G, ld, M, K, th, cX, cZ, s0, gX, gZ);
+}
+inline void kick_drift(bool vec, int D, double e, double he, double* p, double* q, const double* g, const double* im) {
+#ifdef S4B_HOST_AVX2
+  if (vec) { kick_drift_avx2(D, e, he, p, q, g, im); return; }
+#endif
+  (void)vec; kick_drift_scalar(D, e, he, p, q, g, im);
+}
+template <bool Kick>
+inline double leaf_finish(bool vec, int D, double he, double* p, const double* g, const double* im, double* sb, double* se, double* rh, double* pb, double* pe) {
+#ifdef S4B_HOST_AVX2
+  if (vec) return leaf_finish_avx2<Kick>(D, he, p, g, im, sb, se, rh, pb, pe);
+#endif
+  (void)vec; return leaf_finish_scalar<Kick>(D, he, p, g, im, sb, se, rh, pb, pe);
+}
+inline void merge(bool vec, int D, const double* ri, const double* rf, const double* pfb, const double* pie, const double* sb, const double* se, const double* sfb,
+                  const double* sie, double* rh, double out[6]) {
+#ifdef S4B_HOST_AVX2
+  if (vec) { merge_avx2(D, ri, rf, pfb, pie, sb, se, sfb, sie, rh, out); return; }
+#endif
+  (void)vec; merge_scalar(D, ri, rf, pfb, pie, sb, se, sfb, sie, rh, out);
+}
+}
 
 enum TapeCode : int { T_CONST = 0, T_INPUT, T_ADD, T_SUB, T_MUL, T_DIV, T_ADDC, T_SUBC, T_MULC, T_DIVC, T_CSUB, T_CDIV, T_SQRT, T_EXP, T_LOG,
                       T_SQUARE, T_LOG1M, T_STDNORMAL, T_INVLOGIT, T_INVLOGIT_LOGJAC };
@@ -136,15 +338,22 @@
   int b_pos() const { return beta_pos() + K; }
 };
 
-typedef std::function<double(const double* beta, const double* b, double* gX, double* gZ)> Likelihood;
+typedef std::function<double(const double* beta, const double* b, double* gX, double* gZ, double* theta)> Likelihood;
 
 class HostModel {
  public:
   StanSpec sp;
   Likelihood lik;
-  long gradEvals = 0;
-  explicit HostModel(const StanSpec& s) : sp(s) { sp.finish(); plan_closed_form(); }
-  int gradientCheck = 0;
+  alignas(64) long gradEvals = 0;
+  explicit HostModel(const StanSpec& s) : sp(s) { sp.finish(); plan_closed_form(); size_scratch(scratch_); }
+  struct CfWork { double tau, A, rho, e, z0, z1, S, pi0, pi1, trace, sd1, T21, sq; };
+  struct Scratch { std::vector<double> beta, b, gX, gZ, th, theta; std::vector<CfWork> work; };
+  void size_scratch(Scratch& s) const {
+    s.beta.assign((size_t)sp.K + 1, 0.0); s.b.assign((size_t)sp.q + 1, 0.0); s.gX.assign((size_t)sp.K + 1, 0.0); s.gZ.assign((size_t)sp.q + 1, 0.0);
+    s.th.assign((size_t)(3 * sp.t + 1), 0.0); s.theta.assign((size_t)(sp.K + sp.q) + 4, 0.0); s.work.assign((size_t)sp.t + 1, CfWork{});
+  }
+  double closed_form_with(const double* q, double* g, Scratch& s) const { return closed_form_grad(q, g, s); }
+  alignas(64) int gradientCheck = 0;
 
   struct Fwd { TV sigma; std::vector<TV> beta, b, theta_L, constrained; TV lp; bool wantConstrained = true; };
 
@@ -291,7 +500,7 @@
     if (closedForm_ && gradientCheck != 1) {
       ++gradEvals;
       grad.resize((size_t)sp.D);
-      const double lp = closed_form_grad(qv.data(), grad.data());
+      const double lp = closed_form_grad(qv.data(), grad.data(), scratch_);
       if (gradientCheck == 2) {
         std::vector<double> g2; const double lp2 = tape_grad(qv, g2); --gradEvals;
         double gmax = 0.0; for (double x : g2) if (std::isfinite(x)) gmax = std::max(gmax, std::fabs(x));
@@ -328,7 +537,7 @@
     for (int k = 0; k < sp.K; ++k) beta[(size_t)k] = F.beta[(size_t)k].v();
     for (int j = 0; j < sp.q; ++j) b[(size_t)j] = F.b[(size_t)j].v();
     double sigma = F.sigma.v();
-    double ss = lik(beta.data(), b.data(), gX.data(), gZ.data());
+    double ss = lik(beta.data(), b.data(), gX.data(), gZ.data(), scratch_.theta.data());
     double s2 = sigma * sigma, N = (double)sp.N;
     double ll = -0.5 * ss / s2 - N * std::log(sigma) - N * 0.91893853320467274178;
     tape_.adj.assign(tape_.ops.size(), 0.0);
@@ -367,13 +576,11 @@
 
  private:
   struct CfTerm { int p, l, zb0, rho, zeta, tau; double scale, betaA, lbeta, delta0, delta1, lgDelta0, lgDelta1, shape, lgShape; };
-  struct CfWork { double tau, A, rho, e, z0, z1, S, pi0, pi1, trace, sd1, T21, sq; };
-  std::vector<CfWork> cfWork_;
+  Scratch scratch_;
   bool closedForm_ = false;
   std::vector<CfTerm> cfTerms_;
   int cfRho0_ = 0, cfZeta0_ = 0, cfTau0_ = 0, cfAux_ = 0;
   double cfAuxConst_ = 0;
-  std::vector<double> cfBeta_, cfB_, cfGX_, cfGZ_, cfTh_;
   void plan_closed_form() {
     closedForm_ = false;
     if (sp.prior_dist > 1 || sp.hs || sp.n_mix || sp.n_lambda || sp.len_z_T) return;
@@ -399,11 +606,9 @@
       const double nu = sp.prior_df_for_aux;
       cfAuxConst_ = lg((nu + 1.0) / 2.0) - lg(nu / 2.0) - 0.5 * std::log(nu * M_PI);
     }
-    cfBeta_.assign((size_t)sp.K + 1, 0.0); cfB_.assign((size_t)sp.q + 1, 0.0); cfGX_.assign((size_t)sp.K + 1, 0.0); cfGZ_.assign((size_t)sp.q + 1, 0.0);
-    cfTh_.assign((size_t)(3 * sp.t + 1), 0.0); cfWork_.assign((size_t)sp.t + 1, CfWork{});
     closedForm_ = true;
   }
-  double closed_form_grad(const double* q, double* g) {
+  __attribute__((noinline)) double closed_form_grad(const double* q, double* g, Scratch& sc) const {
     const double HALF_LOG_2PI = 0.91893853320467274178, LOG_HALF = -0.693147180559945286;
     const int K = sp.K, nq = sp.q, t = sp.t;
     double lp = 0.0;
@@ -413,13 +618,13 @@
       if (sp.prior_dist_for_aux == 0) { aux = u; dAuxDu = 1.0; }
       else { aux = u * sp.prior_scale_for_aux; dAuxDu = sp.prior_scale_for_aux; if (sp.prior_dist_for_aux <= 2) aux += sp.prior_mean_for_aux; }
     }
-    double* const beta = cfBeta_.data(); double* const b = cfB_.data();
+    double* const beta = sc.beta.data(); double* const b = sc.b.data();
     if (sp.prior_dist == 0) for (int k = 0; k < K; ++k) beta[k] = q[k];
     else for (int k = 0; k < K; ++k) { beta[k] = q[k] * sp.prior_scale[(size_t)k] + sp.prior_mean[(size_t)k]; lp += -0.5 * q[k] * q[k] - HALF_LOG_2PI; }
-    double* const th = cfTh_.data();
+    double* const th = sc.th.data();
     for (int i = 0; i < t; ++i) {
       const CfTerm& c = cfTerms_[(size_t)i];
-      CfWork& w = cfWork_[(size_t)i];
+      CfWork& w = sc.work[(size_t)i];
       const double tau = std::exp(q[c.tau]); lp += q[c.tau];
       const double A = tau * c.scale * aux;
       w.tau = tau; w.A = A;
@@ -456,10 +661,10 @@
         lp += std::log(u * u / nu + 1.0) * (-(nu + 1.0) / 2.0) + cfAuxConst_ - LOG_HALF; dLpDu = -(nu + 1.0) * u / (nu + u * u);
       } else { lp -= u; dLpDu = -1.0; }
     }
-    double* const gX = cfGX_.data(); double* const gZ = cfGZ_.data();
+    double* const gX = sc.gX.data(); double* const gZ = sc.gZ.data();
     for (int k = 0; k < K; ++k) gX[k] = 0.0;
     for (int j = 0; j < nq; ++j) gZ[j] = 0.0;
-    const double ss = lik(beta, b, gX, gZ);
+    const double ss = lik(beta, b, gX, gZ, sc.theta.data());
     const double s2 = aux * aux, N = (double)sp.N, is2 = 1.0 / s2;
     const double ll = -0.5 * ss / s2 - N * std::log(aux) - N * HALF_LOG_2PI;
     double dAux = ss / (s2 * aux) - N / aux;
@@ -468,7 +673,7 @@
     for (int i = 0; i < t; ++i) {
       const CfTerm& c = cfTerms_[(size_t)i];
       const double* zb = q + c.zb0; const double* gb = gZ + (c.zb0 - K); double* gz = g + c.zb0;
-      const CfWork& w = cfWork_[(size_t)i];
+      const CfWork& w = sc.work[(size_t)i];
       const double tau = w.tau, A = w.A;
       double dA = 0.0;
       if (c.p == 1) {
@@ -662,10 +867,171 @@
   double stepsize = 1, jitter = 0; int max_depth = 10;
 };
 
+inline std::atomic<int>& runahead_budget() { static std::atomic<int> b{8}; return b; }
+inline bool runahead_budget_take() {
+  int v = runahead_budget().load(std::memory_order_relaxed);
+  while (v > 0) if (runahead_budget().compare_exchange_weak(v, v - 1, std::memory_order_relaxed)) return true;
+  return false;
+}
+inline void runahead_budget_give() { runahead_budget().fetch_add(1, std::memory_order_relaxed); }
+
+#if defined(__linux__)
+struct CpuNeighbours {
+  static bool read_list(const char* fmt, int cpu, cpu_set_t* out) {
+    char path[128]; std::snprintf(path, sizeof path, fmt, cpu);
+    std::FILE* f = std::fopen(path, "r");
+    if (!f) return false;
+    CPU_ZERO(out);
+    int a, b; bool any = false;
+    while (std::fscanf(f, "%d", &a) == 1) {
+      b = a;
+      int ch = std::fgetc(f);
+      if (ch == '-') { if (std::fscanf(f, "%d", &b) != 1) break; ch = std::fgetc(f); }
+      for (int c = a; c <= b && c < CPU_SETSIZE; ++c) if (c >= 0) { CPU_SET(c, out); any = true; }
+      if (ch != ',') break;
+    }
+    std::fclose(f);
+    return any;
+  }
+  enum Advice { PLACE, ANYWHERE, NOWHERE };
+  static Advice helper_set(int cpu, cpu_set_t* out, cpu_set_t* domain) {
+    cpu_set_t l3, smt, allowed;
+    CPU_ZERO(domain); CPU_ZERO(out);
+    if (cpu < 0 || cpu >= CPU_SETSIZE) return ANYWHERE;
+    CPU_SET(cpu, domain);
+    if (sched_getaffinity(0, sizeof allowed, &allowed) != 0) return ANYWHERE;
+    if (!read_list("/sys/devices/system/cpu/cpu%d/topology/thread_siblings_list", cpu, &smt)) { CPU_ZERO(&smt); CPU_SET(cpu, &smt); }
+    int others = 0;
+    for (int c = 0; c < CPU_SETSIZE; ++c) if (CPU_ISSET(c, &allowed) && !CPU_ISSET(c, &smt)) ++others;
+    if (others == 0) return NOWHERE;
+    if (!read_list("/sys/devices/system/cpu/cpu%d/cache/index3/shared_cpu_list", cpu, &l3)) return ANYWHERE;
+    *domain = l3; CPU_SET(cpu, domain);
+    int n = 0;
+    for (int c = 0; c < CPU_SETSIZE; ++c) if (CPU_ISSET(c, &l3) && CPU_ISSET(c, &allowed) && !CPU_ISSET(c, &smt)) { CPU_SET(c, out); ++n; }
+    if (n > 0) return PLACE;
+    *out = allowed;
+    return PLACE;
+  }
+};
+#endif
+
 class Nuts {
  public:
   typedef std::vector<double> V;
   struct Pt { V q, p, g; double Vv = 0; };
+
+  class RunAhead {
+   public:
+    RunAhead(const HostModel& m, int D, size_t cap) : model_(m), D_(D), cap_(cap), stride_(((size_t)3 * D + 1 + 7) & ~(size_t)7) {
+      th_ = std::thread([this] { thread_main(); });
+      std::unique_lock<std::mutex> lk(m_);
+      cv_.wait(lk, [this] { return phase_ != INIT; });
+      if (phase_ == FAILED) { lk.unlock(); th_.join(); throw std::bad_alloc(); }
+    }
+    ~RunAhead() {
+      finish();
+      { std::lock_guard<std::mutex> lk(m_); phase_ = QUIT; }
+      cv_.notify_one();
+      th_.join();
+    }
+    RunAhead(const RunAhead&) = delete; RunAhead& operator=(const RunAhead&) = delete;
+#if defined(__linux__)
+    void place_on(const cpu_set_t& set) { pthread_setaffinity_np(th_.native_handle(), sizeof set, &set); }
+#endif
+    void start(const Pt& z, double e, const V& inv_metric, bool vec) {
+      {
+        std::lock_guard<std::mutex> lk(m_);
+        q_ = z.q; p_ = z.p; g_ = z.g; im_ = inv_metric; e_ = e; vec_ = vec;
+        taken_ = 0; count_.store(0, std::memory_order_relaxed); stop_.store(0, std::memory_order_relaxed); busy_.store(1, std::memory_order_relaxed);
+        phase_ = POSTED;
+      }
+      cv_.notify_one();
+    }
+    int64_t finish() {
+      {
+        std::lock_guard<std::mutex> lk(m_);
+        if (phase_ == POSTED) { phase_ = IDLE; busy_.store(0, std::memory_order_relaxed); }
+      }
+      stop_.store(1, std::memory_order_relaxed);
+      for (unsigned spins = 0; busy_.load(std::memory_order_acquire); ++spins) { if (spins < 4096) cpu_pause(); else std::this_thread::yield(); }
+      const int64_t done = count_.load(std::memory_order_relaxed), left = done > taken_ ? done - taken_ : 0;
+      count_.store(0, std::memory_order_relaxed); taken_ = 0;
+      return left;
+    }
+    const double* take(int64_t k, bool wait, bool& waited) {
+      if ((size_t)k >= cap_) throw std::logic_error("NUTS run-ahead: more leapfrogs in one direction than 2^max_depth");
+      waited = false;
+      int64_t c = count_.load(std::memory_order_acquire);
+      if (c <= k) {
+        if (!wait) return nullptr;
+        waited = true;
+        for (unsigned spins = 0; (c = count_.load(std::memory_order_acquire)) <= k; ++spins) { if (spins < 4096) cpu_pause(); else std::this_thread::yield(); }
+      }
+      if (k + 1 > taken_) taken_ = k + 1;
+      const double* const s = states_ + (size_t)k * stride_;
+      if (c > k + 1) {
+        const char* const nx = reinterpret_cast<const char*>(s + stride_);
+        for (size_t b = 0; b < ((size_t)2 * D_ + 1) * sizeof(double); b += 64) __builtin_prefetch(nx + b, 0, 3);
+      }
+      return s;
+    }
+    const double* gradient_of(int64_t k) const { return states_ + (size_t)k * stride_ + 2 * (size_t)D_ + 1; }
+   private:
+    enum { INIT = 0, FAILED, IDLE, POSTED, RUNNING, QUIT };
+    void thread_main() {
+      bool ok = true;
+      try {
+        model_.size_scratch(scratch_);
+        q_.assign((size_t)D_, 0.0); p_.assign((size_t)D_, 0.0); g_.assign((size_t)D_, 0.0); im_.assign((size_t)D_, 0.0);
+        raw_.reset(new double[cap_ * stride_ + 8]);
+        states_ = raw_.get();
+        while ((reinterpret_cast<uintptr_t>(states_) & 63u) != 0) ++states_;
+      } catch (...) { ok = false; }
+      std::unique_lock<std::mutex> lk(m_);
+      phase_ = ok ? IDLE : FAILED;
+      cv_.notify_all();
+      if (!ok) return;
+      for (;;) {
+        cv_.wait(lk, [this] { return phase_ == POSTED || phase_ == QUIT; });
+        if (phase_ == QUIT) return;
+        phase_ = RUNNING;
+        lk.unlock();
+        integrate();
+        lk.lock();
+        phase_ = IDLE;
+        busy_.store(0, std::memory_order_release);
+      }
+    }
+    S4B_NO_CONTRACT void integrate() {
+      S4B_NO_CONTRACT_BODY
+      const int D = D_; const double e = e_, he = 0.5 * e_;
+      double* const q = q_.data(); double* const p = p_.data(); double* const g = g_.data();
+      for (size_t k = 0; k < cap_; ++k) {
+        if (stop_.load(std::memory_order_relaxed)) return;
+        hostloop::kick_drift(vec_, D, e, he, p, q, g, im_.data());
+        const double Vv = -model_.closed_form_with(q, g, scratch_);
+        for (int i = 0; i < D; ++i) g[i] = -g[i];
+        for (int i = 0; i < D; ++i) p[i] -= he * g[i];
+        double* const s = states_ + k * stride_;
+        std::copy(q, q + D, s); std::copy(p, p + D, s + D); s[2 * (size_t)D] = Vv; std::copy(g, g + D, s + 2 * (size_t)D + 1);
+        count_.store((int64_t)k + 1, std::memory_order_release);
+      }
+    }
+    const HostModel& model_; const int D_; const size_t cap_, stride_;
+    HostModel::Scratch scratch_;
+    V q_, p_, g_, im_; double e_ = 0; bool vec_ = false;
+    std::unique_ptr<double[]> raw_; double* states_ = nullptr;
+    std::thread th_; std::mutex m_; std::condition_variable cv_; int phase_ = INIT;
+    alignas(64) int64_t taken_ = 0;
+    alignas(64) std::atomic<int64_t> count_{0};
+    alignas(64) std::atomic<int> stop_{0};
+    alignas(64) std::atomic<int> busy_{0};
+    alignas(64) char pad_[8] = {0};
+  };
+  void set_helpers(int n, bool wait = false) { helpersWanted_ = n < 0 ? 0 : (n > 2 ? 2 : n); helpersWait_ = wait; drop_helpers(helpersWanted_); }
+  void set_runahead_allowed(bool ok) { runaheadAllowed_ = ok; if (!ok) drop_helpers(0); }
+  void runahead_counters(int64_t out[4]) const { for (int i = 0; i < 4; ++i) out[i] = raCount_[i]; }
+  ~Nuts() { drop_helpers(0); }
 
   Nuts(HostModel& m, const NutsControl& c, unsigned chain, int num_warmup) : model_(m), D_(m.sp.D), skip_(c.skip) {
     rng_.create(c.seed, chain);
@@ -750,6 +1116,47 @@
   unsigned num_warmup_ = 0, init_buffer_ = 0, term_buffer_ = 0, base_window_ = 0, window_counter_ = 0, next_window_ = 0, window_size_ = 0;
   double wn_ = 0; V wm_, wm2_;
   long nTrans_ = 0, sumDepth_ = 0, sumLeap_ = 0, nDiv_ = 0;
+  std::unique_ptr<RunAhead> ra_[2]; RunAhead* raDir_[2] = {nullptr, nullptr};
+  int helpersWanted_ = 0; bool runaheadAllowed_ = false, vec_ = false, helpersWait_ = false;
+  int64_t raPos_[2] = {0, 0}; bool raGradStale_[2] = {false, false};
+  int64_t raCount_[4] = {0, 0, 0, 0};
+  void drop_helpers(int keep) {
+    for (int k = 1; k >= keep && k >= 0; --k) if (ra_[k]) { ra_[k].reset(); runahead_budget_give(); }
+  }
+  void ensure_helpers() {
+    const size_t cap = (size_t)1 << max_depth_;
+    if (max_depth_ > 20 || cap * ((size_t)3 * D_ + 1) * sizeof(double) > ((size_t)64 << 20)) return;
+    for (int k = 0; k < helpersWanted_; ++k) {
+      if (ra_[k]) continue;
+      if (!runahead_budget_take()) return;
+      try { ra_[k].reset(new RunAhead(model_, D_, cap)); } catch (...) { runahead_budget_give(); return; }
+      placed_ = false;
+    }
+  }
+  bool placed_ = false, noRoom_ = false;
+#if defined(__linux__)
+  cpu_set_t placedDomain_;
+#endif
+  bool place_helpers() {
+#if defined(__linux__)
+    const int cpu = sched_getcpu();
+    if (cpu < 0 || cpu >= CPU_SETSIZE) return true;
+    if (placed_ && CPU_ISSET(cpu, &placedDomain_)) return !noRoom_;
+    cpu_set_t set;
+    const CpuNeighbours::Advice advice = CpuNeighbours::helper_set(cpu, &set, &placedDomain_);
+    placed_ = true; noRoom_ = advice == CpuNeighbours::NOWHERE;
+    if (advice == CpuNeighbours::PLACE) for (int k = 0; k < 2; ++k) if (ra_[k]) ra_[k]->place_on(set);
+    return !noRoom_;
+#else
+    return true;
+#endif
+  }
+  struct RunAheadScope {
+    Nuts& n;
+    ~RunAheadScope() {
+      for (int k = 0; k < 2; ++k) if (n.raDir_[k]) { n.raCount_[2] += n.raDir_[k]->finish(); n.raDir_[k] = nullptr; }
+    }
+  };
 
   double kinetic() const { double s = 0; for (int i = 0; i < D_; ++i) s += z_.p[(size_t)i] * (inv_metric_[(size_t)i] * z_.p[(size_t)i]); return 0.5 * s; }
   double hamiltonian() const { return kinetic() + z_.Vv; }
@@ -819,22 +1226,27 @@
     const int D = D_;
     if (depth == 0) {
       const double e = sign * eps_, he = 0.5 * e;
-      {
-        double* __restrict__ const p = z_.p.data(); double* __restrict__ const q = z_.q.data();
-        const double* __restrict__ const g = z_.g.data(); const double* __restrict__ const im = inv_metric_.data();
-        for (int i = 0; i < D; ++i) { const double pi = p[i] - he * g[i]; p[i] = pi; q[i] += e * (im[i] * pi); }
-      }
-      grad();
-      ++acc.n_leapfrog;
-      double kin = 0.0;
-      {
-        double* __restrict__ const p = z_.p.data(); const double* __restrict__ const g = z_.g.data(); const double* __restrict__ const im = inv_metric_.data();
-        double* __restrict__ const sb = sharp_beg.data(); double* __restrict__ const se = sharp_end.data(); double* __restrict__ const rh = rho.data();
-        double* __restrict__ const pb = p_beg.data(); double* __restrict__ const pe = p_end.data();
-        for (int i = 0; i < D; ++i) {
-          const double pi = p[i] - he * g[i], sh = im[i] * pi;
-          p[i] = pi; kin += pi * sh; sb[i] = sh; se[i] = sh; rh[i] += pi; pb[i] = pi; pe[i] = pi;
+      double kin;
+      const int dir = sign < 0 ? 0 : 1;
+      RunAhead* const ra = raDir_[dir];
+      const int64_t k = raPos_[dir]++;
+      bool waited = false;
+      const double* const s = ra ? ra->take(k, helpersWait_, waited) : nullptr;
+      if (s) {
+        std::copy(s, s + D, z_.q.data()); std::copy(s + D, s + 2 * (size_t)D, z_.p.data()); z_.Vv = s[2 * (size_t)D];
+        raGradStale_[dir] = true;
+        ++model_.gradEvals; ++raCount_[0]; if (waited) ++raCount_[1];
+        ++acc.n_leapfrog;
+        kin = hostloop::leaf_finish<false>(vec_, D, he, z_.p.data(), z_.g.data(), inv_metric_.data(), sharp_beg.data(), sharp_end.data(), rho.data(), p_beg.data(), p_end.data());
+      } else {
+        if (ra) {
+          ++raCount_[1];
+          if (raGradStale_[dir]) { const double* const g = ra->gradient_of(k - 1); std::copy(g, g + D, z_.g.data()); raGradStale_[dir] = false; }
         }
+        hostloop::kick_drift(vec_, D, e, he, z_.p.data(), z_.q.data(), z_.g.data(), inv_metric_.data());
+        grad();
+        ++acc.n_leapfrog;
+        kin = hostloop::leaf_finish<true>(vec_, D, he, z_.p.data(), z_.g.data(), inv_metric_.data(), sharp_beg.data(), sharp_end.data(), rho.data(), p_beg.data(), p_end.data());
       }
       const double hRaw = 0.5 * kin + z_.Vv, h = finite_or_inf(hRaw);
       if (h - H0 > 1000.0) divergent_ = true;
@@ -854,22 +1266,10 @@
     lsw = lse(lsw, lsw_sub);
     if (lsw_final > lsw_sub) std::swap(propose, L.propose_final);
     else if (rng_.u01() < std::exp(lsw_final - lsw_sub)) std::swap(propose, L.propose_final);
-    double a1 = 0, b1 = 0, a2 = 0, b2 = 0, a3 = 0, b3 = 0;
-    {
-      const double* __restrict__ const ri = L.rho_init.data(); const double* __restrict__ const rf = L.rho_final.data();
-      const double* __restrict__ const pfb = L.p_final_beg.data(); const double* __restrict__ const pie = L.p_init_end.data();
-      const double* __restrict__ const sb = sharp_beg.data(); const double* __restrict__ const se = sharp_end.data();
-      const double* __restrict__ const sfb = L.sharp_final_beg.data(); const double* __restrict__ const sie = L.sharp_init_end.data();
-      double* __restrict__ const rh = rho.data();
-      for (int i = 0; i < D; ++i) {
-        const double rs = ri[i] + rf[i], t2 = ri[i] + pfb[i], t3 = rf[i] + pie[i];
-        rh[i] += rs;
-        a1 += se[i] * rs; b1 += sb[i] * rs;
-        a2 += sfb[i] * t2; b2 += sb[i] * t2;
-        a3 += se[i] * t3; b3 += sie[i] * t3;
-      }
-    }
-    return (a1 > 0 && b1 > 0) & (a2 > 0 && b2 > 0) & (a3 > 0 && b3 > 0);
+    double d[6];
+    hostloop::merge(vec_, D, L.rho_init.data(), L.rho_final.data(), L.p_final_beg.data(), L.p_init_end.data(), sharp_beg.data(), sharp_end.data(),
+                    L.sharp_final_beg.data(), L.sharp_init_end.data(), rho.data(), d);
+    return (d[0] > 0 && d[1] > 0) & (d[2] > 0 && d[3] > 0) & (d[4] > 0 && d[5] > 0);
   }
 
   void nuts_transition() {
@@ -877,8 +1277,18 @@
     eps_ = nom_eps_;
     if (jitter_) eps_ *= 1.0 + jitter_ * (2.0 * rng_.u01() - 1.0);
     ensure_levels();
+    vec_ = host_vector_on();
     z_.q = cont_;
     draw_momentum(); grad();
+    RunAheadScope scope{*this};
+    raPos_[0] = raPos_[1] = 0; raGradStale_[0] = raGradStale_[1] = false;
+    if (runaheadAllowed_ && helpersWanted_ > 0) {
+      ensure_helpers();
+      const bool room = place_helpers();
+      if (room && ra_[0]) { ra_[0]->start(z_, -eps_, inv_metric_, vec_); raDir_[0] = ra_[0].get(); }
+      if (room && ra_[1]) { ra_[1]->start(z_, eps_, inv_metric_, vec_); raDir_[1] = ra_[1].get(); }
+    }
+    if (!raDir_[0] && !raDir_[1]) ++raCount_[3];
     const double H0 = hamiltonian();
     Pt& fwd = tFwd_; Pt& bck = tBck_; fwd = z_; bck = z_;
     Prop& sample = tSample_; Prop& propose = tPropose_;
```

New measurement: 515.2 (median of 6 runs). 2.1% higher.
